# bwittmann/transoar

Hardware: AMD Instinct MI355X
Metric: training-step CT volumes/s, 160x160x256 Focused-Decoder (higher is better)
Workload: dtype bf16

## Files before the change

include/transoar_msda3d.h:

```cpp
#ifndef TRANSOAR_MSDA3D_H
#define TRANSOAR_MSDA3D_H

#include <stddef.h>
#include <stdint.h>

#ifdef __cplusplus
extern "C" {
#endif

enum {
  TRANSOAR_F32 = 0,
  TRANSOAR_F64 = 1,
  TRANSOAR_BF16 = 2,
  TRANSOAR_F16 = 3
};

enum {
  TRANSOAR_OK = 0,
  TRANSOAR_ERR_NULL = -1,
  TRANSOAR_ERR_DIM = -2,
  TRANSOAR_ERR_DTYPE = -3,
  TRANSOAR_ERR_ALIGN = -4,
  TRANSOAR_ERR_LEVELS = -5,
  TRANSOAR_ERR_WORKSPACE = -6,
  TRANSOAR_ERR_CONST = -7,
  TRANSOAR_ERR_MODE = -8
};

#define TRANSOAR_MSDA3D_MAX_LEVELS 8

#define TRANSOAR_MSDA3D_FORCE_GENERIC 1u
#define TRANSOAR_MSDA3D_NO_BRICK 4u
#define TRANSOAR_MSDA3D_FORK 8u
#define TRANSOAR_MSDA3D_NO_MMA 16u
#define TRANSOAR_MSDA3D_MMA_Q32 32u
#define TRANSOAR_MSDA3D_Q16 128u
#define TRANSOAR_MSDA3D_DETERMINISTIC 64u
#define TRANSOAR_MSDA3D_PULL_HEAD_MAJOR 2u

int transoar_msda3d_forward(const void* value, const int64_t* spatial_shapes,
                            const int64_t* level_start_index,
                            const void* sampling_loc, const void* attn_weight,
                            void* out, int N, int S, int M, int C, int L,
                            int Lq, int P, int value_dtype, int loc_dtype,
                            const int64_t* host_spatial_shapes, unsigned flags,
                            void* hip_stream);

int transoar_msda3d_forward_fused(const void* value, const void* proj,
                                  const float* ref, long ref_rows, void* out,
                                  int N, int S, int M, int C, int L, int P,
                                  int value_dtype,
                                  const int64_t* host_spatial_shapes,
                                  void* hip_stream);

int transoar_msda3d_backward(const void* value, const int64_t* spatial_shapes,
                             const int64_t* level_start_index,
                             const void* sampling_loc, const void* attn_weight,
                             const void* grad_out, void* grad_value,
                             void* grad_sampling_loc, void* grad_attn_weight,
                             void* workspace, size_t workspace_bytes,
                             int N, int S, int M, int C, int L, int Lq, int P,
                             int value_dtype, int loc_dtype,
                             const int64_t* host_spatial_shapes, unsigned flags,
                             void* hip_stream);

int transoar_msda3d_backward_proj(const void* value, const int64_t* spatial_shapes,
                                  const int64_t* level_start_index, const void* sampling_loc,
                                  const void* attn_weight, const void* grad_out,
                                  void* grad_value, void* grad_proj, void* workspace,
                                  size_t workspace_bytes, int N, int S, int M, int C, int L,
                                  int Lq, int P, int value_dtype, int loc_dtype,
                                  const int64_t* host_spatial_shapes, unsigned flags,
                                  void* hip_stream);

size_t transoar_msda3d_backward_workspace_bytes(int N, int S, int M, int C,
                                                int L, int Lq, int P,
                                                int value_dtype, int loc_dtype,
                                                unsigned flags);

enum {
  TRANSOAR_PROF_FWD = 0,
  TRANSOAR_PROF_BWD_QUERY = 1,
  TRANSOAR_PROF_CELL_COUNT = 2,
  TRANSOAR_PROF_SCAN = 3,
  TRANSOAR_PROF_CELL_FILL = 4,
  TRANSOAR_PROF_PULL = 5,
  TRANSOAR_PROF_FWD_GENERIC = 6,
  TRANSOAR_PROF_BWD_GENERIC = 7,
  TRANSOAR_PROF_VALUE_TILE = 8,
  TRANSOAR_PROF_VALUE_CELLS = 9,
  TRANSOAR_PROF_KINDS = 10
};
void transoar_msda3d_profile_enable(int on);
int transoar_msda3d_profile_read(double* total_ms, long* launches);

const char* transoar_msda3d_strerror(int code);

int transoar_msda3d_abi_version(void);

#ifdef __cplusplus
}
#endif
#endif
```

transoar_amd/backbone.py:

```python
import os

import torch
from torch import nn

from . import instnorm
from .conv3d import Conv3dK3, to_ncdhw
from .position_encoding import PositionEmbeddingLearned3D, PositionEmbeddingSine3D
from .swin_encoder import ConvPatchMerging, EncoderSwinBlock, PatchMerging
from .refine_block import DecoderDefAttnBlock
from .token_linear import token_linear


class EncoderCnnBlock(nn.Module):

    def __init__(self, in_channels, out_channels, kernel_size, stride, padding=1, bias=False,
                 affine=True, eps=1e-05):
        super().__init__()
        kernel_size, stride = tuple(kernel_size), tuple(stride)
        self._block = nn.Sequential(
            Conv3dK3(in_channels, out_channels, kernel_size, stride=stride, padding=padding, bias=bias),
            nn.InstanceNorm3d(out_channels, affine=affine, eps=eps),
            nn.ReLU(inplace=True),
            Conv3dK3(out_channels, out_channels, kernel_size, stride=1, padding=padding, bias=bias),
            nn.InstanceNorm3d(out_channels, affine=affine, eps=eps),
            nn.ReLU(inplace=True),
        )
        self._affine = affine

    fused_norm = True

    def _norm_relu(self, x, norm, part=None):
        if (EncoderCnnBlock.fused_norm and self._affine and x.dtype == torch.bfloat16
                and instnorm.supported(x, norm.num_features)):
            return instnorm.instance_norm_relu(x, norm.weight, norm.bias, norm.eps, relu=True, part=part)
        return torch.relu_(norm(x))

    def _conv_norm_relu(self, conv, norm, x):
        if (EncoderCnnBlock.fused_norm and self._affine and isinstance(conv, Conv3dK3) and norm.num_features <= 32):
            y, part = conv.forward_with_stats(x)
            if part is not None and not (y.dtype == torch.bfloat16 and instnorm.supported(y, norm.num_features)):
                part = None
            return self._norm_relu(y, norm, part)
        return self._norm_relu(conv(x), norm)

    def forward(self, x):
        if not x.is_cuda:
            return self._block(x)
        blk = self._block
        x = self._conv_norm_relu(blk[0], blk[1], x)
        return self._conv_norm_relu(blk[3], blk[4], x)


class Encoder(nn.Module):
    def __init__(self, config, debug=False):
        super().__init__()
        self._debug = debug
        self._stages = nn.ModuleList()
        cin, cout = config["in_channels"], config["start_channels"]
        swin = bool(config["use_encoder_attn"])
        depths = list(config["depths"])
        dpr = [float(v) for v in torch.linspace(0, config["drop_path_rate"], sum(depths))]
        merge = ConvPatchMerging if config["conv_merging"] else PatchMerging
        for stage_id, (kernel, stride) in enumerate(zip(config["conv_kernels"], config["strides"])):
            if swin and stage_id > 1:
                k = stage_id - 2
                stage = EncoderSwinBlock(
                    dim=cin, depth=depths[k], num_heads=config["num_heads"][k], window_size=config["window_size"],
                    mlp_ratio=config["mlp_ratio"], qkv_bias=config["qkv_bias"], qk_scale=config["qk_scale"],
                    drop=config["drop_rate"], attn_drop=config["attn_drop_rate"],
                    drop_path=dpr[sum(depths[:k]):sum(depths[:k + 1])], downsample=merge)
            else:
                stage = EncoderCnnBlock(cin, cout, kernel, stride)
            self._stages.append(stage)
            cin, cout = cout, cout * 2

    def forward(self, x):
        outputs = {}
        for i, stage in enumerate(self._stages):
            x = stage(x)
            outputs["C%d" % i] = x
        if self._debug:
            print("AttnFPN encoder shapes:", {k: list(v.shape) for k, v in outputs.items()})
            self._debug = False
        return outputs


def _gemm_conv_ok(f):
    return (f.is_cuda and f.dtype == torch.bfloat16 and f.dim() == 5 and f.shape[1] % 8 == 0
            and f.is_contiguous(memory_format=torch.channels_last_3d)
            and torch.is_autocast_enabled() and torch.get_autocast_gpu_dtype() == torch.bfloat16)


def _conv1_as_gemm(conv, f):
    n, c, d, h, w = f.shape
    tok = f.permute(0, 2, 3, 4, 1).reshape(n, d * h * w, c)
    y = token_linear(tok, conv.weight.view(conv.out_channels, c), conv.bias, force_hip=True, min_tokens=1024)
    return y.view(n, d, h, w, conv.out_channels).permute(0, 4, 1, 2, 3)


def _is_up2(up):
    return (tuple(up.kernel_size) == (2, 2, 2) and tuple(up.stride) == (2, 2, 2) and tuple(up.padding) == (0, 0, 0)
            and tuple(up.output_padding) == (0, 0, 0) and tuple(up.dilation) == (1, 1, 1) and up.groups == 1)


def _up2_as_gemm(up, f):
    n, c, d, h, w = f.shape
    co = up.out_channels
    tok = f.permute(0, 2, 3, 4, 1).reshape(n, d * h * w, c)
    w8 = up.weight.permute(2, 3, 4, 1, 0).reshape(8 * co, c)
    b8 = None if up.bias is None else up.bias.repeat(8)
    y = token_linear(tok, w8, b8, force_hip=True, min_tokens=1024)
    y = y.view(n, d, h, w, 2, 2, 2, co).permute(0, 1, 4, 2, 5, 3, 6, 7).reshape(n, 2 * d, 2 * h, 2 * w, co)
    return y.permute(0, 4, 1, 2, 3)


class Decoder(nn.Module):
    gemm_pointwise = os.environ.get("TRANSOAR_FPN_STOCK_POINTWISE") is None

    def __init__(self, config, debug=False):
        super().__init__()
        self._debug = debug
        n_stages = len(config["conv_kernels"])
        self._num_stages = n_stages
        self._refine_fmaps = config["use_decoder_attn"]
        self._refine_feature_levels = list(config["feature_levels"])
        self._seg_proxy = config["use_seg_proxy_loss"]
        fpn = int(config["fpn_channels"])
        enc_channels = [config["start_channels"] * 2 ** s for s in range(n_stages)]

        wanted = list(config["out_fmaps"]) + (list(config["feature_levels"]) if self._refine_fmaps else [])
        required = {int(name[-1]) for name in wanted}
        if self._seg_proxy:
            required.add(0)
        self._required_stages = sorted(required)
        first = 0 if self._seg_proxy else self._required_stages[0]
        self._first_stage = first

        lateral_in = enc_channels[first:]
        lateral_out = [min(c, fpn) for c in lateral_in]
        self._lateral = nn.ModuleList(nn.Conv3d(i, o, kernel_size=1) for i, o in zip(lateral_in, lateral_out))
        self._lateral_levels = len(self._lateral)

        self._out = nn.ModuleList()
        for n, stage in enumerate(self._required_stages):
            cout = enc_channels[0] if (self._seg_proxy and n == 0) else fpn
            self._out.append(Conv3dK3(lateral_out[stage - first], cout, kernel_size=3, padding=1))

        self._up = nn.ModuleList()
        coarse_to_fine = lateral_out[::-1]
        strides = [tuple(s) for s in config["strides"]][::-1]
        for lvl in range(len(coarse_to_fine) - 1):
            self._up.append(nn.ConvTranspose3d(coarse_to_fine[lvl], coarse_to_fine[lvl + 1],
                                               kernel_size=strides[lvl], stride=strides[lvl]))

        if self._refine_fmaps:
            if config["pos_encoding"] == "sine":
                self._pos_enc = PositionEmbeddingSine3D(channels=config["hidden_dim"])
            elif config["pos_encoding"] == "learned":
                self._pos_enc = PositionEmbeddingLearned3D(channels=config["hidden_dim"])
            else:
                raise ValueError("Please select a implemented pos. encoding.")
            self._refine = DecoderDefAttnBlock(
                d_model=config["hidden_dim"], nhead=config["nheads"], num_layers=config["layers"],
                dim_feedforward=config["dim_feedforward"], dropout=config["dropout"],
                feature_levels=config["feature_levels"], n_points=config["n_points"],
                use_cuda=config["use_cuda"])

    def forward(self, x):
        feats = list(x.values())[-self._lateral_levels:]
        if not Conv3dK3.ndhwc_everywhere:
            feats = [to_ncdhw(f) for f in feats]
        as_gemm = Decoder.gemm_pointwise and all(_gemm_conv_ok(f) for f in feats)
        laterals = [(_conv1_as_gemm(conv, f) if as_gemm else conv(f)) for conv, f in zip(self._lateral, feats)]
        merged = [None] * self._lateral_levels
        carry = None
        for k, lat in enumerate(reversed(laterals)):
            cur = lat if carry is None else lat + carry
            merged[self._lateral_levels - 1 - k] = cur
            if k < self._lateral_levels - 1:
                up = self._up[k]
                carry = _up2_as_gemm(up, cur) if (as_gemm and _is_up2(up)) else up(cur)
        outputs = {"P%d" % s: self._out[n](merged[s - self._first_stage])
                   for n, s in enumerate(self._required_stages)}

        if self._refine_fmaps:
            fmaps = [outputs[name] for name in self._refine_feature_levels]
            refined = self._refine(fmaps, [self._pos_enc(f) for f in fmaps])
            outputs.update(zip(self._refine_feature_levels, refined))
        if self._debug:
            print("AttnFPN decoder shapes:", {k: list(v.shape) for k, v in outputs.items()})
            self._debug = False
        return outputs


class AttnFPN(nn.Module):
    def __init__(self, fpn_config, debug=False):
        super().__init__()
        self._encoder = Encoder(fpn_config, debug)
        self._decoder = Decoder(fpn_config, debug)

    def forward(self, src):
        return self._decoder(self._encoder(src))

    def init_weights(self):
        pass
```

transoar_amd/csrc/msda3d.hip:

```cpp
#include <algorithm>
#include <cstring>

#include "../../include/transoar_msda3d.h"
#include "msda3d_common.hpp"
#include "msda3d_brick.hpp"
#include "msda3d_mma.hpp"
#include "msda3d_pcm.hpp"
#include "msda3d_q16.hpp"
#include "msda3d_tile.hpp"
#include "msda3d_cells_mma.hpp"
#include "msda3d_gather.hpp"
#include "msda3d_generic.hpp"
#include "msda3d_scatter.hpp"

#include <map>
#include <mutex>
#include <string>
#include <vector>

namespace transoar {

struct ProfPair { hipEvent_t beg, end; int kind; };
static std::mutex g_prof_mu;
static bool g_prof_on = false;
static std::vector<ProfPair> g_prof_live;
static std::vector<ProfPair> g_prof_free;

struct ProfScope {
  hipStream_t st;
  ProfPair pair;
  bool on;
  ProfScope(int kind, hipStream_t s) : st(s), on(false) {
    std::lock_guard<std::mutex> lk(g_prof_mu);
    if (!g_prof_on) return;
    if (!g_prof_free.empty()) {
      pair = g_prof_free.back();
      g_prof_free.pop_back();
    } else if (hipEventCreate(&pair.beg) != hipSuccess || hipEventCreate(&pair.end) != hipSuccess) {
      return;
    }
    pair.kind = kind;
    on = hipEventRecord(pair.beg, st) == hipSuccess;
  }
  ~ProfScope() {
    if (!on) return;
    (void)hipEventRecord(pair.end, st);
    std::lock_guard<std::mutex> lk(g_prof_mu);
    g_prof_live.push_back(pair);
  }
};

struct SideStream {
  hipStream_t stream = nullptr;
  hipEvent_t fork = nullptr, join = nullptr;
  bool ok = false;
};
static SideStream* side_stream() {
  static std::mutex mu;
  static SideStream per_device[16];
  int dev = 0;
  if (hipGetDevice(&dev) != hipSuccess || dev < 0 || dev >= 16) return nullptr;
  std::lock_guard<std::mutex> lk(mu);
  SideStream& s = per_device[dev];
  if (!s.ok && s.stream == nullptr) {
    if (hipStreamCreateWithFlags(&s.stream, hipStreamNonBlocking) == hipSuccess &&
        hipEventCreateWithFlags(&s.fork, hipEventDisableTiming) == hipSuccess &&
        hipEventCreateWithFlags(&s.join, hipEventDisableTiming) == hipSuccess)
      s.ok = true;
  }
  return s.ok ? &s : nullptr;
}

__global__ __launch_bounds__(256) void msda3d_zero16(u32x4* __restrict__ p, long n16) {
  const long i = static_cast<long>(blockIdx.x) * 256 + threadIdx.x;
  if (i < n16) p[i] = u32x4{0u, 0u, 0u, 0u};
}
static inline hipError_t zero_async(void* p, size_t bytes, hipStream_t st) {
  if (getenv("TRANSOAR_MSDA_MEMSET_NODE")) return hipMemsetAsync(p, 0, bytes, st);
  const long n16 = static_cast<long>((bytes + 15) / 16);
  hipLaunchKernelGGL(msda3d_zero16, dim3(static_cast<unsigned>((n16 + 255) / 256)), dim3(256), 0, st,
                     static_cast<u32x4*>(p), n16);
  return hipGetLastError();
}

struct Dims { int N, S, M, C, L, Lq, P; };

static inline int lpv_log2(int C, int elt) {
  const long bytes = static_cast<long>(C) * elt;
  if (bytes == 128) return 3;
  if (bytes == 256) return 4;
  if (bytes == 512) return 5;
  return -1;
}

static BrickOrder make_order(const int64_t* host_shapes, const Dims& d, int rows) {
  BrickOrder o{};
  if (!host_shapes || rows != d.S) return o;
  long start = 0, pad = 0;
  for (int l = 0; l < d.L; ++l) {
    const long D = host_shapes[3 * l], H = host_shapes[3 * l + 1], W = host_shapes[3 * l + 2];
    if (D <= 0 || H <= 0 || W <= 0) return BrickOrder{};
    o.D[l] = static_cast<int>(D); o.H[l] = static_cast<int>(H); o.W[l] = static_cast<int>(W);
    o.start[l] = static_cast<int>(start);
    o.nbh[l] = static_cast<int>((H + kBrickH - 1) / kBrickH);
    o.nbw[l] = static_cast<int>((W + kBrickW - 1) / kBrickW);
    o.pad_start[l] = static_cast<int>(pad);
    pad += ((D + kBrickD - 1) / kBrickD) * o.nbh[l] * o.nbw[l] * kBrickSlots;
    start += D * H * W;
  }
  if (start != d.S || pad * d.N * d.M >= (1L << 31)) return BrickOrder{};
  o.pad_start[d.L] = static_cast<int>(pad);
  o.L = d.L;
  o.enabled = 1;
  return o;
}
static inline long order_units(const BrickOrder& o, const Dims& d, int rows) {
  return static_cast<long>(d.N) * d.M * (o.enabled ? o.pad_start[o.L] : rows);
}

static inline size_t align16(size_t x) { return (x + 15) & ~static_cast<size_t>(15); }

static const void* device_const(const void* host, size_t bytes, hipStream_t st) {
  static std::mutex mu;
  static std::map<std::pair<int, std::string>, void*> cache;
  int dev = 0;
  if (hipGetDevice(&dev) != hipSuccess) return nullptr;
  std::pair<int, std::string> key(dev, std::string(static_cast<const char*>(host), bytes));
  std::lock_guard<std::mutex> lk(mu);
  auto it = cache.find(key);
  if (it != cache.end()) return it->second;
  hipStreamCaptureStatus cap = hipStreamCaptureStatusNone;
  if (hipStreamIsCapturing(st, &cap) != hipSuccess || cap != hipStreamCaptureStatusNone) return nullptr;
  if (cache.size() >= 256) return nullptr;
  void* p = nullptr;
  if (hipMalloc(&p, bytes) != hipSuccess) return nullptr;
  if (hipMemcpy(p, host, bytes, hipMemcpyHostToDevice) != hipSuccess) {
    (void)hipFree(p);
    return nullptr;
  }
  cache[key] = p;
  return p;
}
template <typename T> static const T* device_const(const T& v, hipStream_t st) {
  return static_cast<const T*>(device_const(&v, sizeof(T), st));
}

static inline int vec_lpv(const Dims& d, int elt, unsigned flags) {
  if (flags & TRANSOAR_MSDA3D_FORCE_GENERIC) return -1;
  const long value_bytes = static_cast<long>(d.N) * d.S * d.M * d.C * elt;
  const long n_points = static_cast<long>(d.N) * d.Lq * d.M * d.L * d.P;
  const long n_bins = static_cast<long>(d.N) * d.M * 8 * d.S;
  if (value_bytes >= 0xfffffff0L || n_points >= (1L << 31) - 1 || n_bins >= (1L << 31) - 1) return -1;
  if (static_cast<long>(d.N) * d.S >= (1L << 24) || static_cast<long>(d.M) * d.C * elt >= (1L << 24)) return -1;
  if (n_points * 32 >= 0xfffffff0L) return -1;
  if (static_cast<long>(d.N) * d.Lq * d.M >= (1L << 24) ||
      static_cast<long>(d.N) * d.Lq * d.M * d.C * elt >= 0x7ffffff0L) return -1;
  return lpv_log2(d.C, elt);
}

struct BwdWorkspace {
  size_t count, tile_sums, rank, rec_item, recs, coarse, det_keys, det_alt, det_temp, det_temp_bytes, total;
  long n_bins, n_points, n_scan, n_tiles;
};

int sort_keys64(unsigned long long* keys, unsigned long long* alt, long n, int end_bit, void* temp, size_t* temp_bytes,
                unsigned long long** sorted, hipStream_t st);

static BwdWorkspace bwd_workspace(const Dims& d, size_t acc_size, unsigned flags = 0u) {
  BwdWorkspace w;
  w.n_points = static_cast<long>(d.N) * d.Lq * d.M * d.L * d.P;
  w.n_bins = static_cast<long>(d.N) * d.M * 8 * d.S;
  w.n_scan = w.n_bins + 1;
  w.n_tiles = (w.n_scan + kScanTile - 1) / kScanTile;
  size_t off = 0;
  w.count = off;     off += align16(sizeof(int) * w.n_scan);
  w.tile_sums = off; off += align16(sizeof(int) * w.n_tiles);
  w.rank = off;      off += align16(sizeof(int) * w.n_points);
  w.rec_item = off;  off += align16(sizeof(int) * w.n_points);
  w.recs = off;      off += align16(8 * acc_size * w.n_points);
  w.coarse = off;    off += align16(sizeof(float) * static_cast<size_t>(d.N) * d.S * d.M * d.C);
  w.det_keys = w.det_alt = w.det_temp = off;
  w.det_temp_bytes = 0;
  if (flags & TRANSOAR_MSDA3D_DETERMINISTIC) {
    w.det_keys = off;  off += align16(sizeof(unsigned long long) * w.n_points);
    w.det_alt = off;   off += align16(sizeof(unsigned long long) * w.n_points);
    w.det_temp_bytes = align16((size_t(32) << 20) + static_cast<size_t>(w.n_points));
    w.det_temp = off;  off += w.det_temp_bytes;
  }
  w.total = off;
  return w;
}

static bool pcm_ok(const BrickOrder& order, const Dims& d) {
  if (!order.enabled || d.L > kPcmLevels || d.C != 64 || d.P != 4 || d.Lq != d.S) return false;
  for (int l = 0; l < d.L; ++l)
    if (order.D[l] > 1000 || order.H[l] > 1000 || order.W[l] > 1000) return false;
  const long n_pts = static_cast<long>(d.N) * d.Lq * d.M * d.L * d.P;
  const long n_wave = static_cast<long>(d.N) * (order.pad_start[order.L] >> 7) * d.M * 16;
  const long vbytes = static_cast<long>(d.N) * d.S * d.M * d.C * 2;
  return n_pts * 12 < 0xfffffff0L && n_wave < (1L << 31) - 8 && vbytes < 0xffffff00L;
}
static float host_bf16_round(float x) {
  unsigned u;
  memcpy(&u, &x, 4);
  u += 0x7fffu + ((u >> 16) & 1u);
  u &= 0xffff0000u;
  memcpy(&x, &u, 4);
  return x;
}
static PcmConst make_pcm_const(const BrickOrder& order) {
  PcmConst c;
  memset(&c, 0, sizeof(c));
  c.order = order;
  for (int l = 0; l < 4; ++l) {
    const int ls = l < order.L ? l : 0;
    c.fD[l] = static_cast<float>(order.D[ls]); c.fH[l] = static_cast<float>(order.H[ls]); c.fW[l] = static_cast<float>(order.W[ls]);
    c.dD[l] = host_bf16_round(c.fD[l]); c.dH[l] = host_bf16_round(c.fH[l]); c.dW[l] = host_bf16_round(c.fW[l]);
  }
  return c;
}

static Q16Const make_q16_const(const BrickOrder& order, int M) {
  Q16Const c;
  memset(&c, 0, sizeof(c));
  c.pc = make_pcm_const(order);
  auto mg = [](long d) -> unsigned long long { return (1ull << 40) / static_cast<unsigned long long>(d > 0 ? d : 1) + 1ull; };
  c.mg_M = mg(M);
  c.mg_bricks = mg(order.pad_start[order.L] >> 7);
  for (int l = 0; l < 4; ++l) {
    c.mg_nbw[l] = mg(l < order.L ? order.nbw[l] : 1);
    c.mg_nbh[l] = mg(l < order.L ? order.nbh[l] : 1);
  }
  return c;
}
static int env_int(const char* name, int dflt) {
  const char* v = getenv(name);
  return (v && *v) ? atoi(v) : dflt;
}

template <typename VT, typename LT>
static int launch_fwd(const void* value, const int64_t* shapes, const int64_t* lsi,
                      const void* loc, const void* attn, void* out, const Dims& d,
                      const int64_t* host_shapes, unsigned flags, hipStream_t st) {
  const long n_items = static_cast<long>(d.N) * d.Lq * d.M;
  const BrickOrder order = make_order(host_shapes, d, d.Lq);
  const long n_units = order_units(order, d, d.Lq);
  const long n_blocks = ((order.enabled ? n_units : n_items) + kWavesPerBlock - 1) / kWavesPerBlock;
  const int lg = vec_lpv(d, sizeof(VT), flags);
  const dim3 block(64 * kWavesPerBlock);
  auto v = static_cast<const VT*>(value);
  auto lo = static_cast<const LT*>(loc);
  auto at = static_cast<const LT*>(attn);
  auto o = static_cast<VT*>(out);
  if constexpr (sizeof(VT) == 2) {
    bool small = d.L <= kMmaLevels;
    for (int l = 0; small && l < d.L; ++l) small = order.D[l] <= 1000 && order.H[l] <= 1000 && order.W[l] <= 1000;
    if constexpr (sizeof(LT) == 4) {
      if (lg >= 0 && small && pcm_ok(order, d) && (flags & TRANSOAR_MSDA3D_Q16) &&
          !(flags & (TRANSOAR_MSDA3D_NO_BRICK | TRANSOAR_MSDA3D_NO_MMA | TRANSOAR_MSDA3D_MMA_Q32))) {
        ProfScope prof(TRANSOAR_PROF_FWD, st);
        static const int upw_env = env_int("TRANSOAR_MSDA3D_Q16_UPW", 4), probe = env_int("TRANSOAR_MSDA3D_Q16_PROBE", 0);
        const unsigned upw = static_cast<unsigned>(upw_env < 1 ? 1 : (upw_env > 64 ? 64 : upw_env));
        const long n_units = static_cast<long>(d.N) * (order.pad_start[order.L] >> 7) * d.M * 8;
        const long n_waves = (n_units + upw - 1) / upw;
        const unsigned vbytes = static_cast<unsigned>(static_cast<long>(d.N) * d.S * d.M * d.C * sizeof(VT));
        const long n_pts = static_cast<long>(d.N) * d.Lq * d.M * d.L * d.P;
        const Q16Const* cst = device_const(make_q16_const(order, d.M), st);
        if (cst == nullptr) return TRANSOAR_ERR_CONST;
        const dim3 grid(static_cast<unsigned>(((n_waves + 7) / 8) * 8));
#define TRANSOAR_Q16(PROBE)                                                                                             \
  hipLaunchKernelGGL((msda3d_fwd_q16<VT, PROBE>), grid, dim3(64), 0, st, v, lo, at, o, d.S, d.M, d.L, vbytes,               \
                     static_cast<unsigned>(n_pts * 12), static_cast<unsigned>(n_pts * 4), static_cast<unsigned>(n_units), upw, cst)
        if (probe == 1) TRANSOAR_Q16(1);
        else if (probe == 2) TRANSOAR_Q16(2);
        else if (probe == 3) TRANSOAR_Q16(3);
        else TRANSOAR_Q16(0);
#undef TRANSOAR_Q16
        return static_cast<int>(hipGetLastError());
      }
      if (lg >= 0 && small && pcm_ok(order, d) &&
          !(flags & (TRANSOAR_MSDA3D_NO_BRICK | TRANSOAR_MSDA3D_NO_MMA | TRANSOAR_MSDA3D_MMA_Q32))) {
        ProfScope prof(TRANSOAR_PROF_FWD, st);
        const long n_wave = static_cast<long>(d.N) * (order.pad_start[order.L] >> 7) * d.M * 16;
        const unsigned vbytes = static_cast<unsigned>(static_cast<long>(d.N) * d.S * d.M * d.C * sizeof(VT));
        const long n_pts = static_cast<long>(d.N) * d.Lq * d.M * d.L * d.P;
        const PcmConst* cst = device_const(make_pcm_const(order), st);
        if (cst == nullptr) return TRANSOAR_ERR_CONST;
        hipLaunchKernelGGL((msda3d_fwd_pcm<VT, false>), dim3(static_cast<unsigned>(((n_wave + 7) / 8) * 8)), dim3(64), 0, st,
                           v, lo, at, nullptr, nullptr, 0u, o, d.S, d.M, d.L, vbytes, static_cast<unsigned>(n_pts * 12),
                           static_cast<unsigned>(n_pts * 4), static_cast<unsigned>(n_wave), cst);
        return static_cast<int>(hipGetLastError());
      }
    }
    if (lg >= 0 && order.enabled && small && d.C == 64 && d.P == 4 &&
        !(flags & (TRANSOAR_MSDA3D_NO_BRICK | TRANSOAR_MSDA3D_NO_MMA))) {
      ProfScope prof(TRANSOAR_PROF_FWD, st);
      const long n_wave = static_cast<long>(d.N) * (order.pad_start[order.L] >> 7) * d.M * 4;
      const unsigned vbytes = static_cast<unsigned>(static_cast<long>(d.N) * d.S * d.M * d.C * sizeof(VT));
      const BrickOrder* order_d = device_const(order, st);
      if (order_d == nullptr) return TRANSOAR_ERR_CONST;
      hipLaunchKernelGGL((msda3d_fwd_mma<VT, LT>), dim3(static_cast<unsigned>(((n_wave + 7) / 8) * 8)), dim3(64), 0, st,
                         v, lo, at, o, d.S, d.M, d.L, vbytes, n_wave, order_d);
      return static_cast<int>(hipGetLastError());
    }
  }
  if (lg >= 0 && order.enabled && d.C == 64 && d.P == 4 && sizeof(VT) == 2 && !(flags & TRANSOAR_MSDA3D_NO_BRICK)) {
    ProfScope prof(TRANSOAR_PROF_FWD, st);
    const long n_wg = static_cast<long>(d.N) * (order.pad_start[order.L] >> 7) * d.M;
    const dim3 bgrid(((n_wg + 7) / 8) * 8);
    hipLaunchKernelGGL((msda3d_fwd_brick<VT, LT, 4, 64>), bgrid, dim3(kBrickThreads), kTileBytes, st, v, lo, at, o,
                       d.S, d.M, d.L, n_wg, order);
    return static_cast<int>(hipGetLastError());
  }
  if (lg < 0) {
    ProfScope prof(TRANSOAR_PROF_FWD_GENERIC, st);
    hipLaunchKernelGGL((msda3d_fwd_generic<VT, LT>), dim3((n_items + kWavesPerBlock - 1) / kWavesPerBlock),
                       block, 0, st, v, shapes, lsi, lo, at, o, d.S, d.M, d.C, d.L, d.Lq, d.P, n_items);
  } else {
    ProfScope prof(TRANSOAR_PROF_FWD, st);
    const dim3 grid(((n_blocks + 7) / 8) * 8);
    const unsigned vbytes = static_cast<unsigned>(static_cast<long>(d.N) * d.S * d.M * d.C * sizeof(VT));
#define TRANSOAR_FWD(LG)                                                                      \
  hipLaunchKernelGGL((msda3d_fwd_vec<VT, LT, LG>), grid, block, 0, st, v, shapes, lsi, lo, at, \
                     o, d.S, d.M, d.C, d.L, d.Lq, d.P, vbytes, n_units, n_blocks, order)
    if (lg == 3) TRANSOAR_FWD(3);
    else if (lg == 4) TRANSOAR_FWD(4);
    else TRANSOAR_FWD(5);
#undef TRANSOAR_FWD
  }
  return static_cast<int>(hipGetLastError());
}

template <typename VT>
static int launch_fwd_fused(const void* value, const void* proj, const float* ref, long ref_rows, void* out, const Dims& d,
                            const int64_t* host_shapes, hipStream_t st) {
  const BrickOrder order = make_order(host_shapes, d, d.Lq);
  if (vec_lpv(d, sizeof(VT), 0) < 0 || !pcm_ok(order, d)) return TRANSOAR_ERR_DIM;
  if (ref_rows != d.Lq && ref_rows != static_cast<long>(d.N) * d.Lq) return TRANSOAR_ERR_DIM;
  ProfScope prof(TRANSOAR_PROF_FWD, st);
  const long n_wave = static_cast<long>(d.N) * (order.pad_start[order.L] >> 7) * d.M * 16;
  const unsigned vbytes = static_cast<unsigned>(static_cast<long>(d.N) * d.S * d.M * d.C * sizeof(VT));
  const PcmConst* cst = device_const(make_pcm_const(order), st);
  if (cst == nullptr) return TRANSOAR_ERR_CONST;
  const unsigned ref_bstride = ref_rows == d.Lq ? 0u : static_cast<unsigned>(d.Lq) * d.L * 12u;
  const long proj_bytes = static_cast<long>(d.N) * d.S * 4 * d.M * d.L * d.P * 2;
  hipLaunchKernelGGL((msda3d_fwd_pcm<VT, true>), dim3(static_cast<unsigned>(((n_wave + 7) / 8) * 8)), dim3(64), 0, st,
                     static_cast<const VT*>(value), nullptr, nullptr, static_cast<const unsigned short*>(proj), ref, ref_bstride,
                     static_cast<VT*>(out), d.S, d.M, d.L, vbytes, static_cast<unsigned>(proj_bytes),
                     static_cast<unsigned>(ref_rows * d.L * 12), static_cast<unsigned>(n_wave), cst);
  return static_cast<int>(hipGetLastError());
}

__global__ __launch_bounds__(256) void msda3d_det_gather(const unsigned long long* __restrict__ sorted, const PointR16* __restrict__ slots,
                                                          PointR16* __restrict__ recs, long n) {
  const long j = static_cast<long>(blockIdx.x) * 256 + threadIdx.x;
  if (j >= n) return;
  const unsigned long long k = sorted[j];
  if (k == ~0ull) return;
  recs[j] = slots[static_cast<unsigned>(k)];
}

template <typename VT, typename LT>
static size_t bwd_workspace_bytes(const Dims& d, unsigned flags) {
  using A = typename Elem<VT>::acc;
  if (vec_lpv(d, sizeof(VT), flags) >= 0) return bwd_workspace(d, sizeof(A), flags).total;
  return sizeof(VT) == 2 ? align16(sizeof(float) * static_cast<size_t>(d.N) * d.S * d.M * d.C) : 0;
}

#define TRANSOAR_CHECK_HIP(expr)                         \
  do {                                                   \
    const hipError_t e_ = (expr);                        \
    if (e_ != hipSuccess) return static_cast<int>(e_);   \
  } while (0)

template <typename VT, typename LT>
static int launch_bwd(const void* value, const int64_t* shapes, const int64_t* lsi,
                      const void* loc, const void* attn, const void* grad_out, void* grad_value,
                      void* grad_loc, void* grad_attn, void* workspace, size_t workspace_bytes,
                      const Dims& d, const int64_t* host_shapes, unsigned flags, hipStream_t st, void* grad_proj = nullptr) {
  using A = typename Elem<VT>::acc;
  if (workspace_bytes < bwd_workspace_bytes<VT, LT>(d, flags)) return TRANSOAR_ERR_WORKSPACE;
  if (grad_proj != nullptr && (sizeof(VT) != 2 || sizeof(LT) != 4 || vec_lpv(d, sizeof(VT), flags) < 0)) return TRANSOAR_ERR_MODE;
  const long n_items = static_cast<long>(d.N) * d.Lq * d.M;
  const BrickOrder q_order = make_order(host_shapes, d, d.Lq);
  const long q_units = order_units(q_order, d, d.Lq);
  const long n_blocks = (q_units + kWavesPerBlock - 1) / kWavesPerBlock;
  const int lg = vec_lpv(d, sizeof(VT), flags);
  const dim3 block(64 * kWavesPerBlock);
  auto v = static_cast<const VT*>(value);
  auto lo = static_cast<const LT*>(loc);
  auto at = static_cast<const LT*>(attn);
  auto go = static_cast<const VT*>(grad_out);
  auto gl = static_cast<LT*>(grad_loc);
  auto ga = static_cast<LT*>(grad_attn);
  const size_t value_elems = static_cast<size_t>(d.N) * d.S * d.M * d.C;

  if (lg < 0) {
    ProfScope prof(TRANSOAR_PROF_BWD_GENERIC, st);
    A* gv = sizeof(VT) == 2 ? static_cast<A*>(workspace) : static_cast<A*>(grad_value);
    TRANSOAR_CHECK_HIP(hipMemsetAsync(gv, 0, sizeof(A) * value_elems, st));
    hipLaunchKernelGGL((msda3d_bwd_generic<VT, LT>), dim3((n_items + kWavesPerBlock - 1) / kWavesPerBlock),
                       block, 0, st, v, shapes, lsi, lo, at, go, gv, gl, ga, d.S, d.M, d.C, d.L, d.Lq, d.P,
                       n_items);
    if (sizeof(VT) == 2) {
      const int cast_blocks = static_cast<int>(std::min<size_t>((value_elems + 255) / 256, 1 << 16));
      hipLaunchKernelGGL((msda3d_cast_rows<VT>), dim3(cast_blocks), dim3(256), 0, st,
                         reinterpret_cast<const float*>(gv), static_cast<VT*>(grad_value),
                         static_cast<long>(value_elems));
    }
    return static_cast<int>(hipGetLastError());
  }

  const dim3 grid(((n_blocks + 7) / 8) * 8);
  const unsigned vbytes = static_cast<unsigned>(value_elems * sizeof(VT));
  const BwdWorkspace w = bwd_workspace(d, sizeof(A), flags);
  char* ws = static_cast<char*>(workspace);
  int* count = reinterpret_cast<int*>(ws + w.count);
  int* tile_sums = reinterpret_cast<int*>(ws + w.tile_sums);
  int* rank = reinterpret_cast<int*>(ws + w.rank);
  int* rec_item = reinterpret_cast<int*>(ws + w.rec_item);
  auto recs = reinterpret_cast<PointRec<A>*>(ws + w.recs);
  long cells_per_slab = 0;
  if (host_shapes)
    for (int l = 0; l < d.L; ++l)
      cells_per_slab += (host_shapes[3 * l] + 1) * (host_shapes[3 * l + 1] + 1) * (host_shapes[3 * l + 2] + 1);
  const bool fold_count = host_shapes != nullptr && cells_per_slab * d.N * d.M <= w.n_bins;
  const bool det_req = (flags & TRANSOAR_MSDA3D_DETERMINISTIC) != 0;
  const long n_scan = fold_count ? cells_per_slab * d.N * d.M + 1 + (det_req && cells_per_slab * d.N * d.M + 2 <= w.n_scan ? 1 : 0) : w.n_scan;
  const long n_tiles = (n_scan + kScanTile - 1) / kScanTile;
  TRANSOAR_CHECK_HIP(zero_async(count, sizeof(int) * n_scan, st));
  auto scan = [&]() {
    ProfScope prof(TRANSOAR_PROF_SCAN, st);
    hipLaunchKernelGGL(msda3d_scan_tiles, dim3(static_cast<unsigned>(n_tiles)), dim3(kScanThreads), 0,
                       st, count, tile_sums, static_cast<int>(n_scan));
    hipLaunchKernelGGL(msda3d_scan_tile_sums, dim3(1), dim3(kScanThreads), 0, st, tile_sums,
                       static_cast<int>(n_tiles));
    hipLaunchKernelGGL(msda3d_scan_add, dim3(static_cast<unsigned>(n_tiles)), dim3(kScanThreads), 0, st,
                       count, tile_sums, static_cast<int>(n_scan));
  };

#define TRANSOAR_BWDQ(LG)                                                                   \
  hipLaunchKernelGGL((msda3d_bwd_query_vec<VT, LT, LG>), grid, block, 0, st, v, shapes, lsi, lo, \
                     at, go, gl, ga, fold_count ? count : nullptr, rank, static_cast<int>(cells_per_slab), \
                     d.S, d.M, d.C, d.L, d.Lq, d.P, vbytes, q_units, n_blocks, q_order)
  bool brick_done = false, recs_done = false, det = false;
  if constexpr (sizeof(VT) == 2) {
    bool small = d.L <= kMmaLevels;
    for (int l = 0; small && l < d.L; ++l) small = q_order.D[l] <= 1000 && q_order.H[l] <= 1000 && q_order.W[l] <= 1000;
    if (q_order.enabled && fold_count && small && d.C == 64 && d.P == 4 &&
        !(flags & (TRANSOAR_MSDA3D_NO_BRICK | TRANSOAR_MSDA3D_NO_MMA))) {
      const long n_wave = static_cast<long>(d.N) * (q_order.pad_start[q_order.L] >> 7) * d.M * 4;
      const BrickOrder* order_d = device_const(q_order, st);
      if (order_d == nullptr) return TRANSOAR_ERR_CONST;
      const dim3 qgrid(static_cast<unsigned>(((n_wave + 7) / 8) * 8));
      {
        ProfScope prof(TRANSOAR_PROF_CELL_COUNT, st);
        hipLaunchKernelGGL((msda3d_cell_count_mma<LT>), qgrid, dim3(64), 0, st, lo, count + 1,
                           static_cast<int>(cells_per_slab), d.S, d.M, d.L, n_wave, order_d);
      }
      scan();
      det = det_req && cells_per_slab * d.N * d.M + 2 <= w.n_scan && w.n_points < (1L << 31);
      if (det_req && !det) return TRANSOAR_ERR_MODE;
      if (!det) {
        ProfScope prof(TRANSOAR_PROF_BWD_QUERY, st);
        hipLaunchKernelGGL((msda3d_bwd_query_mma<VT, LT>), qgrid, dim3(64), 0, st,
                           v, lo, at, go, gl, ga, count + 1, reinterpret_cast<PointR16*>(ws + w.recs), nullptr,
                           static_cast<int>(cells_per_slab), d.S, d.M, d.L, vbytes, n_wave, order_d,
                           static_cast<unsigned short*>(grad_proj));
      } else {
        auto keys = reinterpret_cast<unsigned long long*>(ws + w.det_keys);
        auto alt = reinterpret_cast<unsigned long long*>(ws + w.det_alt);
        PointR16* slots = reinterpret_cast<PointR16*>(ws + w.recs) + w.n_points;
        TRANSOAR_CHECK_HIP(hipMemsetAsync(keys, 0xff, sizeof(unsigned long long) * w.n_points, st));
        {
          ProfScope prof(TRANSOAR_PROF_BWD_QUERY, st);
          hipLaunchKernelGGL((msda3d_bwd_query_mma<VT, LT>), qgrid, dim3(64), 0, st,
                             v, lo, at, go, gl, ga, count + 1, slots, keys,
                             static_cast<int>(cells_per_slab), d.S, d.M, d.L, vbytes, n_wave, order_d,
                             static_cast<unsigned short*>(grad_proj));
        }
        ProfScope prof(TRANSOAR_PROF_CELL_FILL, st);
        int cell_bits = 1;
        while ((cells_per_slab * d.N * d.M) >> cell_bits) ++cell_bits;
        size_t need = 0;
        int rc = sort_keys64(keys, alt, w.n_points, 32 + cell_bits, nullptr, &need, nullptr, st);
        if (rc != 0) return rc;
        if (need > w.det_temp_bytes) return TRANSOAR_ERR_WORKSPACE;
        unsigned long long* sorted = nullptr;
        size_t temp_bytes = w.det_temp_bytes;
        rc = sort_keys64(keys, alt, w.n_points, 32 + cell_bits, ws + w.det_temp, &temp_bytes, &sorted, st);
        if (rc != 0) return rc;
        hipLaunchKernelGGL(msda3d_det_gather, dim3(static_cast<unsigned>((w.n_points + 255) / 256)), dim3(256), 0, st,
                           sorted, slots, reinterpret_cast<PointR16*>(ws + w.recs), w.n_points);
      }
      brick_done = recs_done = true;
    }
  }
  if (det_req && !det) return TRANSOAR_ERR_MODE;
  if (grad_proj != nullptr && !recs_done) return TRANSOAR_ERR_MODE;
  if constexpr (sizeof(VT) == 2) {
    if (!brick_done && q_order.enabled && fold_count && d.C == 64 && d.P == 4 && !(flags & TRANSOAR_MSDA3D_NO_BRICK)) {
      ProfScope prof(TRANSOAR_PROF_BWD_QUERY, st);
      const long n_wg = static_cast<long>(d.N) * (q_order.pad_start[q_order.L] >> 7) * d.M;
      hipLaunchKernelGGL((msda3d_bwd_query_brick<VT, LT, 4, 64>), dim3(((n_wg + 7) / 8) * 8), dim3(kBrickThreads),
                         kTileBytes, st, v, lo, at, go, gl, ga, count, rank, static_cast<int>(cells_per_slab), d.S, d.M,
                         d.L, n_wg, q_order);
      brick_done = true;
    }
  }
  if (!brick_done) {
    ProfScope prof(TRANSOAR_PROF_BWD_QUERY, st);
    if (lg == 3) TRANSOAR_BWDQ(3);
    else if (lg == 4) TRANSOAR_BWDQ(4);
    else TRANSOAR_BWDQ(5);
  }
#undef TRANSOAR_BWDQ

  const dim3 pgrid(static_cast<unsigned>((w.n_points + 255) / 256));
  if (!fold_count) {
    ProfScope prof(TRANSOAR_PROF_CELL_COUNT, st);
    hipLaunchKernelGGL((msda3d_cell_count<LT, A>), pgrid, dim3(256), 0, st, lo, at, shapes, lsi, count,
                       rank, d.M, d.L, d.Lq, d.P, w.n_points);
  }
  if (!recs_done) scan();
  BrickOrder r_order = make_order(host_shapes, d, d.S);
  if constexpr (sizeof(A) == 4) {
    if (r_order.enabled && fold_count && d.C == kTileC && !(flags & TRANSOAR_MSDA3D_NO_BRICK)) {
      auto recs8 = reinterpret_cast<PointW8<float>*>(ws + w.recs);
      auto recs4 = reinterpret_cast<PointR16*>(ws + w.recs);
      bool mma = false;
      if constexpr (sizeof(VT) == 2) mma = !(flags & TRANSOAR_MSDA3D_NO_MMA);
      if (!recs_done) {
        ProfScope prof(TRANSOAR_PROF_CELL_FILL, st);
        if (mma)
          hipLaunchKernelGGL((msda3d_cell_fill_r16<LT>), pgrid, dim3(256), 0, st, lo, at, shapes, lsi, count, rank, recs4,
                             d.M, d.L, d.Lq, d.P, w.n_points);
        else
          hipLaunchKernelGGL((msda3d_cell_fill_w8<LT, float>), pgrid, dim3(256), 0, st, lo, at, shapes, lsi, count,
                             rank, recs8, rec_item, d.M, d.L, d.Lq, d.P, w.n_points);
      }
      CoarseLevels cl{d.L, static_cast<int>(cells_per_slab), d.S, 0, 0};
      const int* offsets = det ? count + 1 : count;
      for (int l = d.L - 1; l >= 0 && !det; --l) {
        const long vox = host_shapes[3 * l] * host_shapes[3 * l + 1] * host_shapes[3 * l + 2];
        if (static_cast<long>(d.Lq) * d.P < kCoarsePointsPerVoxel * vox) break;
        cl.first = l;
        cl.cell_start -= static_cast<int>((host_shapes[3 * l] + 1) * (host_shapes[3 * l + 1] + 1) * (host_shapes[3 * l + 2] + 1));
        cl.row_start = r_order.start[l];
      }
      cl.rows = d.S - cl.row_start;
      const int coarse_levels = d.L - cl.first;
      const int cell_chunk = mma ? kCmCellChunk : kCellChunk;
      cl.chunks_per_slab = static_cast<int>((static_cast<long>(d.Lq) * d.P * coarse_levels + cell_chunk - 1) / cell_chunk) + 1;
      const int fine_bricks = r_order.pad_start[cl.first] >> 7;
      const BrickOrder* r_order_d = device_const(r_order, st);
      const CoarseLevels* cl_d = device_const(cl, st);
      if (r_order_d == nullptr || cl_d == nullptr) return TRANSOAR_ERR_CONST;
      float* scratch = reinterpret_cast<float*>(ws + w.coarse);
      const long scratch_elems = static_cast<long>(d.N) * cl.rows * d.M * kTileC;
      SideStream* side = (g_prof_on || !(flags & TRANSOAR_MSDA3D_FORK) || coarse_levels == 0 || fine_bricks == 0)
                             ? nullptr : side_stream();
      hipStream_t cst = st;
      if (side != nullptr) {
        TRANSOAR_CHECK_HIP(hipEventRecord(side->fork, st));
        TRANSOAR_CHECK_HIP(hipStreamWaitEvent(side->stream, side->fork, 0));
        cst = side->stream;
      }
      if (coarse_levels > 0) {
        ProfScope prof(TRANSOAR_PROF_VALUE_CELLS, cst);
        TRANSOAR_CHECK_HIP(zero_async(scratch, sizeof(float) * scratch_elems, cst));
        const long waves = static_cast<long>(d.N) * d.M * cl.chunks_per_slab;
        if (mma) {
          if constexpr (sizeof(VT) == 2)
            hipLaunchKernelGGL((msda3d_bwd_value_cells_mma<VT>), dim3(static_cast<unsigned>((waves + 3) / 4)), dim3(256), 0,
                               cst, go, offsets, recs4, scratch, static_cast<int>(cells_per_slab), d.N * d.M, d.M,
                               cl_d, r_order_d);
        } else {
          hipLaunchKernelGGL((msda3d_bwd_value_cells<VT>), dim3(static_cast<unsigned>((waves + 3) / 4)), dim3(256), 0, cst,
                             go, count, recs8, rec_item, scratch, static_cast<int>(cells_per_slab), d.N * d.M, d.M, cl_d,
                             r_order_d);
        }
      }
      if (side != nullptr) TRANSOAR_CHECK_HIP(hipEventRecord(side->join, side->stream));
      ProfScope prof(TRANSOAR_PROF_VALUE_TILE, st);
      if (fine_bricks > 0) {
        const long n_wg = static_cast<long>(d.N) * fine_bricks * d.M;
        if (mma) {
          if constexpr (sizeof(VT) == 2)
            hipLaunchKernelGGL((msda3d_bwd_value_tile_mma<VT>), dim3(static_cast<unsigned>(n_wg)), dim3(kBrickThreads), 0, st,
                               go, offsets, recs4, static_cast<VT*>(grad_value), static_cast<int>(cells_per_slab),
                               d.S, d.M, fine_bricks, n_wg, r_order_d);
        } else {
          hipLaunchKernelGGL((msda3d_bwd_value_tile<VT>), dim3(static_cast<unsigned>(n_wg)), dim3(kBrickThreads), 0, st, go,
                             count, recs8, rec_item, static_cast<VT*>(grad_value), static_cast<int>(cells_per_slab),
                             d.S, d.M, fine_bricks, n_wg, r_order_d);
        }
      }
      if (side != nullptr) TRANSOAR_CHECK_HIP(hipStreamWaitEvent(st, side->join, 0));
      if (coarse_levels > 0) {
        const long n4 = scratch_elems / 4;
        hipLaunchKernelGGL((msda3d_coarse_rows_store<VT>), dim3(static_cast<unsigned>((n4 + 255) / 256)), dim3(256), 0, st,
                           scratch, static_cast<VT*>(grad_value), d.S, d.M, cl.rows, cl.row_start, n4);
      }
      return static_cast<int>(hipGetLastError());
    }
  }
  {
    ProfScope prof(TRANSOAR_PROF_CELL_FILL, st);
    hipLaunchKernelGGL((msda3d_cell_fill<LT, A>), pgrid, dim3(256), 0, st, lo, at, shapes, lsi, count,
                       rank, recs, rec_item, d.M, d.L, d.Lq, d.P, w.n_points);
  }

  if (r_order.enabled && (flags & TRANSOAR_MSDA3D_PULL_HEAD_MAJOR)) r_order.enabled = 2;
  const long n_rows = order_units(r_order, d, d.S);
  const long r_blocks = (n_rows + kWavesPerBlock - 1) / kWavesPerBlock;
  const dim3 rgrid(((r_blocks + 7) / 8) * 8);
#define TRANSOAR_PULL(LG)                                                                        \
  hipLaunchKernelGGL((msda3d_bwd_value_pull<VT, A, LG>), rgrid, block, 0, st, go, shapes, lsi, count, \
                     recs, rec_item, static_cast<VT*>(grad_value), d.S, d.M, d.C, d.L, n_rows, r_blocks, r_order, \
                     static_cast<unsigned>(w.n_points * 4 * sizeof(A)))
  {
    ProfScope prof(TRANSOAR_PROF_PULL, st);
    if (lg == 3) TRANSOAR_PULL(3);
    else if (lg == 4) TRANSOAR_PULL(4);
    else TRANSOAR_PULL(5);
  }
#undef TRANSOAR_PULL
  return static_cast<int>(hipGetLastError());
}

static int check_common(const Dims& d, int value_dtype, int loc_dtype) {
  if (d.N <= 0 || d.S <= 0 || d.M <= 0 || d.C <= 0 || d.L <= 0 || d.Lq <= 0 || d.P <= 0)
    return TRANSOAR_ERR_DIM;
  if (d.L > TRANSOAR_MSDA3D_MAX_LEVELS) return TRANSOAR_ERR_LEVELS;
  if (static_cast<long>(d.N) * d.Lq * d.M >= (1L << 31) || static_cast<long>(d.N) * d.S >= (1L << 31))
    return TRANSOAR_ERR_DIM;
  const bool half = value_dtype == TRANSOAR_BF16 || value_dtype == TRANSOAR_F16;
  if (value_dtype < 0 || value_dtype > TRANSOAR_F16) return TRANSOAR_ERR_DTYPE;
  if (!(loc_dtype == value_dtype || (half && loc_dtype == TRANSOAR_F32))) return TRANSOAR_ERR_DTYPE;
  return TRANSOAR_OK;
}

static inline bool misaligned(const void* p) { return (reinterpret_cast<uintptr_t>(p) & 15u) != 0; }

}

using namespace transoar;

#define TRANSOAR_DISPATCH(VD, LD, CALL)                                            \
  do {                                                                             \
    if (VD == TRANSOAR_F32) { using VT = float; using LT = float; return CALL; }   \
    if (VD == TRANSOAR_F64) { using VT = double; using LT = double; return CALL; } \
    if (VD == TRANSOAR_BF16 && LD == TRANSOAR_BF16) { using VT = bf16_t; using LT = bf16_t; return CALL; } \
    if (VD == TRANSOAR_BF16) { using VT = bf16_t; using LT = float; return CALL; } \
    if (VD == TRANSOAR_F16 && LD == TRANSOAR_F16) { using VT = f16_t; using LT = f16_t; return CALL; }     \
    { using VT = f16_t; using LT = float; return CALL; }                           \
  } while (0)

extern "C" int transoar_msda3d_forward(const void* value, const int64_t* spatial_shapes,
                                       const int64_t* level_start_index, const void* sampling_loc,
                                       const void* attn_weight, void* out, int N, int S, int M,
                                       int C, int L, int Lq, int P, int value_dtype, int loc_dtype,
                                       const int64_t* host_spatial_shapes, unsigned flags,
                                       void* hip_stream) {
  if (!value || !spatial_shapes || !level_start_index || !sampling_loc || !attn_weight || !out)
    return TRANSOAR_ERR_NULL;
  const Dims d{N, S, M, C, L, Lq, P};
  const int rc = check_common(d, value_dtype, loc_dtype);
  if (rc != TRANSOAR_OK) return rc;
  if (misaligned(value) || misaligned(sampling_loc) || misaligned(attn_weight) || misaligned(out))
    return TRANSOAR_ERR_ALIGN;
  hipStream_t st = static_cast<hipStream_t>(hip_stream);
  TRANSOAR_DISPATCH(value_dtype, loc_dtype,
                    (launch_fwd<VT, LT>(value, spatial_shapes, level_start_index, sampling_loc,
                                        attn_weight, out, d, host_spatial_shapes, flags, st)));
}

extern "C" int transoar_msda3d_forward_fused(const void* value, const void* proj, const float* ref, long ref_rows,
                                             void* out, int N, int S, int M, int C, int L, int P, int value_dtype,
                                             const int64_t* host_spatial_shapes, void* hip_stream) {
  if (!value || !proj || !ref || !out || !host_spatial_shapes) return TRANSOAR_ERR_NULL;
  const Dims d{N, S, M, C, L, S, P};
  const int rc = check_common(d, value_dtype, TRANSOAR_F32);
  if (rc != TRANSOAR_OK) return rc;
  if (value_dtype != TRANSOAR_BF16 && value_dtype != TRANSOAR_F16) return TRANSOAR_ERR_DTYPE;
  if (misaligned(value) || misaligned(proj) || misaligned(ref) || misaligned(out)) return TRANSOAR_ERR_ALIGN;
  hipStream_t st = static_cast<hipStream_t>(hip_stream);
  if (value_dtype == TRANSOAR_BF16) return launch_fwd_fused<bf16_t>(value, proj, ref, ref_rows, out, d, host_spatial_shapes, st);
  return launch_fwd_fused<f16_t>(value, proj, ref, ref_rows, out, d, host_spatial_shapes, st);
}

extern "C" int transoar_msda3d_backward(const void* value, const int64_t* spatial_shapes,
                                        const int64_t* level_start_index, const void* sampling_loc,
                                        const void* attn_weight, const void* grad_out,
                                        void* grad_value, void* grad_sampling_loc,
                                        void* grad_attn_weight, void* workspace,
                                        size_t workspace_bytes, int N, int S, int M, int C, int L,
                                        int Lq, int P, int value_dtype, int loc_dtype,
                                        const int64_t* host_spatial_shapes, unsigned flags,
                                        void* hip_stream) {
  if (!value || !spatial_shapes || !level_start_index || !sampling_loc || !attn_weight ||
      !grad_out || !grad_value || !grad_sampling_loc || !grad_attn_weight)
    return TRANSOAR_ERR_NULL;
  const Dims d{N, S, M, C, L, Lq, P};
  const int rc = check_common(d, value_dtype, loc_dtype);
  if (rc != TRANSOAR_OK) return rc;
  if (misaligned(value) || misaligned(sampling_loc) || misaligned(attn_weight) ||
      misaligned(grad_out) || misaligned(grad_value) || misaligned(grad_sampling_loc) ||
      misaligned(grad_attn_weight) || misaligned(workspace))
    return TRANSOAR_ERR_ALIGN;
  if (!workspace && workspace_bytes != 0) return TRANSOAR_ERR_NULL;
  hipStream_t st = static_cast<hipStream_t>(hip_stream);
  TRANSOAR_DISPATCH(value_dtype, loc_dtype,
                    (launch_bwd<VT, LT>(value, spatial_shapes, level_start_index, sampling_loc,
                                        attn_weight, grad_out, grad_value, grad_sampling_loc,
                                        grad_attn_weight, workspace, workspace_bytes, d,
                                        host_spatial_shapes, flags, st)));
}

extern "C" int transoar_msda3d_backward_proj(const void* value, const int64_t* spatial_shapes,
                                             const int64_t* level_start_index, const void* sampling_loc,
                                             const void* attn_weight, const void* grad_out,
                                             void* grad_value, void* grad_proj, void* workspace,
                                             size_t workspace_bytes, int N, int S, int M, int C, int L,
                                             int Lq, int P, int value_dtype, int loc_dtype,
                                             const int64_t* host_spatial_shapes, unsigned flags,
                                             void* hip_stream) {
  if (!value || !spatial_shapes || !level_start_index || !sampling_loc || !attn_weight ||
      !grad_out || !grad_value || !grad_proj)
    return TRANSOAR_ERR_NULL;
  const Dims d{N, S, M, C, L, Lq, P};
  const int rc = check_common(d, value_dtype, loc_dtype);
  if (rc != TRANSOAR_OK) return rc;
  if (loc_dtype != TRANSOAR_F32 || (value_dtype != TRANSOAR_BF16 && value_dtype != TRANSOAR_F16) || L * P != 16) return TRANSOAR_ERR_MODE;
  if (misaligned(value) || misaligned(sampling_loc) || misaligned(attn_weight) ||
      misaligned(grad_out) || misaligned(grad_value) || misaligned(grad_proj) || misaligned(workspace))
    return TRANSOAR_ERR_ALIGN;
  if (!workspace && workspace_bytes != 0) return TRANSOAR_ERR_NULL;
  hipStream_t st = static_cast<hipStream_t>(hip_stream);
  TRANSOAR_DISPATCH(value_dtype, loc_dtype,
                    (launch_bwd<VT, LT>(value, spatial_shapes, level_start_index, sampling_loc,
                                        attn_weight, grad_out, grad_value, nullptr, nullptr, workspace, workspace_bytes, d,
                                        host_spatial_shapes, flags, st, grad_proj)));
}

extern "C" size_t transoar_msda3d_backward_workspace_bytes(int N, int S, int M, int C, int L, int Lq,
                                                           int P, int value_dtype, int loc_dtype,
                                                           unsigned flags) {
  const Dims d{N, S, M, C, L, Lq, P};
  if (check_common(d, value_dtype, loc_dtype) != TRANSOAR_OK) return 0;
  TRANSOAR_DISPATCH(value_dtype, loc_dtype, (bwd_workspace_bytes<VT, LT>(d, flags)));
}

extern "C" const char* transoar_msda3d_strerror(int code) {
  switch (code) {
    case TRANSOAR_OK: return "success";
    case TRANSOAR_ERR_NULL: return "a required pointer is NULL";
    case TRANSOAR_ERR_DIM: return "a dimension is non-positive or exceeds the 32-bit index range";
    case TRANSOAR_ERR_DTYPE: return "unsupported value/loc dtype combination";
    case TRANSOAR_ERR_ALIGN: return "a device buffer is not 16-byte aligned";
    case TRANSOAR_ERR_LEVELS: return "too many feature levels";
    case TRANSOAR_ERR_WORKSPACE: return "workspace is smaller than transoar_msda3d_backward_workspace_bytes()";
    case TRANSOAR_ERR_MODE: return "the deterministic backward does not cover this form (16-bit storage, C = 64, P = 4, <= 4 host-known levels, queries = pyramid voxels)";
    case TRANSOAR_ERR_CONST: return "could not place the launch constants in device memory (first call for a shape must not be inside a stream capture)";
    default: return code > 0 ? hipGetErrorString(static_cast<hipError_t>(code)) : "unknown error";
  }
}

extern "C" void transoar_msda3d_profile_enable(int on) {
  std::lock_guard<std::mutex> lk(g_prof_mu);
  g_prof_on = on != 0;
}

extern "C" int transoar_msda3d_profile_read(double* total_ms, long* launches) {
  std::vector<ProfPair> live;
  {
    std::lock_guard<std::mutex> lk(g_prof_mu);
    live.swap(g_prof_live);
  }
  for (int k = 0; k < TRANSOAR_PROF_KINDS; ++k) {
    total_ms[k] = 0.0;
    launches[k] = 0;
  }
  int rc = 0;
  for (const ProfPair& p : live) {
    float ms = 0.f;
    hipError_t e = hipEventSynchronize(p.end);
    if (e == hipSuccess) e = hipEventElapsedTime(&ms, p.beg, p.end);
    if (e != hipSuccess) { rc = static_cast<int>(e); continue; }
    total_ms[p.kind] += ms;
    launches[p.kind] += 1;
  }
  std::lock_guard<std::mutex> lk(g_prof_mu);
  g_prof_free.insert(g_prof_free.end(), live.begin(), live.end());
  return rc;
}

extern "C" int transoar_msda3d_abi_version(void) { return 6; }
```

transoar_amd/csrc/msda3d_common.hpp:

```cpp
#pragma once
#include <hip/hip_runtime.h>
#include <stdint.h>

namespace transoar {

constexpr int kWavesPerBlock = 4;
constexpr int kChunk = 16;

struct bf16_t { unsigned short bits; };
struct f16_t { _Float16 v; };

using u32x4 = __attribute__((ext_vector_type(4))) unsigned int;

__device__ __forceinline__ float bf16_to_f32(unsigned short b) {
  return __uint_as_float(static_cast<unsigned int>(b) << 16);
}
__device__ __forceinline__ unsigned short f32_to_bf16(float f) {
  unsigned int u = __float_as_uint(f);
  if ((u & 0x7fffffffu) > 0x7f800000u) return static_cast<unsigned short>((u >> 16) | 0x40u);
  u += 0x7fffu + ((u >> 16) & 1u);
  return static_cast<unsigned short>(u >> 16);
}

template <typename T> struct Elem;

template <> struct Elem<float> {
  using acc = float;
  static constexpr int VEC = 4;
  static __device__ __forceinline__ float ld(const float* p) { return *p; }
  static __device__ __forceinline__ void st(float* p, float v) { *p = v; }
  static __device__ __forceinline__ void unpack(const u32x4& r, float (&o)[4]) {
#pragma unroll
    for (int i = 0; i < 4; ++i) o[i] = __uint_as_float(r[i]);
  }
  static __device__ __forceinline__ u32x4 pack(const float (&o)[4]) {
    u32x4 r;
#pragma unroll
    for (int i = 0; i < 4; ++i) r[i] = __float_as_uint(o[i]);
    return r;
  }
};

template <> struct Elem<double> {
  using acc = double;
  static constexpr int VEC = 2;
  static __device__ __forceinline__ double ld(const double* p) { return *p; }
  static __device__ __forceinline__ void st(double* p, double v) { *p = v; }
  static __device__ __forceinline__ void unpack(const u32x4& r, double (&o)[2]) {
#pragma unroll
    for (int i = 0; i < 2; ++i)
      o[i] = __longlong_as_double((static_cast<long long>(r[2 * i + 1]) << 32) |
                                  static_cast<long long>(r[2 * i]));
  }
  static __device__ __forceinline__ u32x4 pack(const double (&o)[2]) {
    u32x4 r;
#pragma unroll
    for (int i = 0; i < 2; ++i) {
      const long long b = __double_as_longlong(o[i]);
      r[2 * i] = static_cast<unsigned int>(b);
      r[2 * i + 1] = static_cast<unsigned int>(b >> 32);
    }
    return r;
  }
};

template <> struct Elem<bf16_t> {
  using acc = float;
  static constexpr int VEC = 8;
  static __device__ __forceinline__ float ld(const bf16_t* p) { return bf16_to_f32(p->bits); }
  static __device__ __forceinline__ void st(bf16_t* p, float v) { p->bits = f32_to_bf16(v); }
  static __device__ __forceinline__ void unpack(const u32x4& r, float (&o)[8]) {
#pragma unroll
    for (int i = 0; i < 4; ++i) {
      o[2 * i] = __uint_as_float(r[i] << 16);
      o[2 * i + 1] = __uint_as_float(r[i] & 0xffff0000u);
    }
  }
  static __device__ __forceinline__ u32x4 pack(const float (&o)[8]) {
    u32x4 r;
#pragma unroll
    for (int i = 0; i < 4; ++i)
      r[i] = static_cast<unsigned int>(f32_to_bf16(o[2 * i])) |
             (static_cast<unsigned int>(f32_to_bf16(o[2 * i + 1])) << 16);
    return r;
  }
  static __device__ __forceinline__ float dot2(unsigned int a, unsigned int b, float acc) {
    typedef __bf16 bf16x2 __attribute__((ext_vector_type(2)));
    return __builtin_amdgcn_fdot2_f32_bf16(__builtin_bit_cast(bf16x2, a), __builtin_bit_cast(bf16x2, b), acc, false);
  }
};

template <> struct Elem<f16_t> {
  using acc = float;
  static constexpr int VEC = 8;
  static __device__ __forceinline__ float h2f(unsigned int bits16) {
    return static_cast<float>(__builtin_bit_cast(_Float16, static_cast<unsigned short>(bits16)));
  }
  static __device__ __forceinline__ unsigned int f2h(float f) {
    return __builtin_bit_cast(unsigned short, static_cast<_Float16>(f));
  }
  static __device__ __forceinline__ float ld(const f16_t* p) { return static_cast<float>(p->v); }
  static __device__ __forceinline__ void st(f16_t* p, float v) { p->v = static_cast<_Float16>(v); }
  static __device__ __forceinline__ void unpack(const u32x4& r, float (&o)[8]) {
#pragma unroll
    for (int i = 0; i < 4; ++i) {
      o[2 * i] = h2f(r[i] & 0xffffu);
      o[2 * i + 1] = h2f(r[i] >> 16);
    }
  }
  static __device__ __forceinline__ u32x4 pack(const float (&o)[8]) {
    u32x4 r;
#pragma unroll
    for (int i = 0; i < 4; ++i) r[i] = f2h(o[2 * i]) | (f2h(o[2 * i + 1]) << 16);
    return r;
  }
  static __device__ __forceinline__ float dot2(unsigned int a, unsigned int b, float acc) {
    typedef _Float16 f16x2 __attribute__((ext_vector_type(2)));
    return __builtin_amdgcn_fdot2(__builtin_bit_cast(f16x2, a), __builtin_bit_cast(f16x2, b), acc, false);
  }
};

__device__ __forceinline__ float pixel_coord(float loc, int size) {
#pragma clang fp contract(off)
  const float t = loc * static_cast<float>(size);
  return t - 0.5f;
}
__device__ __forceinline__ double pixel_coord(double loc, int size) {
#pragma clang fp contract(off)
  const double t = loc * static_cast<double>(size);
  return t - 0.5;
}

__device__ __forceinline__ float bcast(float v, int src) {
  return __int_as_float(__builtin_amdgcn_readlane(__float_as_int(v), src));
}
__device__ __forceinline__ double bcast(double v, int src) {
  const long long b = __double_as_longlong(v);
  const unsigned lo = __builtin_amdgcn_readlane(static_cast<int>(b), src);
  const unsigned hi = __builtin_amdgcn_readlane(static_cast<int>(b >> 32), src);
  return __longlong_as_double((static_cast<long long>(hi) << 32) | lo);
}

__device__ __forceinline__ float xor_lanes(float v, int mask) { return __shfl_xor(v, mask, 64); }
__device__ __forceinline__ double xor_lanes(double v, int mask) { return __shfl_xor(v, mask, 64); }

__device__ __forceinline__ float xor_free_shfl(float v, int src) { return __shfl(v, src, 64); }
__device__ __forceinline__ double xor_free_shfl(double v, int src) { return __shfl(v, src, 64); }

__device__ __forceinline__ void atomic_accum(float* p, float v) {
  __hip_atomic_fetch_add(p, v, __ATOMIC_RELAXED, __HIP_MEMORY_SCOPE_AGENT);
}
__device__ __forceinline__ void atomic_accum(double* p, double v) {
  __hip_atomic_fetch_add(p, v, __ATOMIC_RELAXED, __HIP_MEMORY_SCOPE_AGENT);
}

template <int HALF, typename A>
__device__ __forceinline__ void fold_lanes(const A (&in)[2 * HALF], A (&out)[HALF], int lane) {
  const bool up = (lane & HALF) != 0;
#pragma unroll
  for (int i = 0; i < HALF; ++i) {
    const A send = up ? in[i] : in[i + HALF];
    const A keep = up ? in[i + HALF] : in[i];
    out[i] = keep + xor_lanes(send, HALF);
  }
}
template <typename A>
__device__ __forceinline__ A sum_transpose64(const A (&v)[64], int lane) {
  A a32[32], a16[16], a8[8], a4[4], a2[2], a1[1];
  fold_lanes<32>(v, a32, lane);
  fold_lanes<16>(a32, a16, lane);
  fold_lanes<8>(a16, a8, lane);
  fold_lanes<4>(a8, a4, lane);
  fold_lanes<2>(a4, a2, lane);
  fold_lanes<1>(a2, a1, lane);
  return a1[0];
}

constexpr int kBrickD = 4, kBrickH = 4, kBrickW = 8, kBrickSlots = 128;
struct BrickOrder {
  int enabled, L;
  int D[8], H[8], W[8], start[8];
  int nbh[8], nbw[8];
  int pad_start[9];
};
__device__ __forceinline__ int brick_slot_to_row(const BrickOrder& o, int x) {
  int l = 0;
  for (int t = 1; t < o.L; ++t) l += (x >= o.pad_start[t]) ? 1 : 0;
  const int local = x - o.pad_start[l];
  const int brick = local >> 7, slot = local & 127;
  const int bw = brick % o.nbw[l];
  const int r = brick / o.nbw[l];
  const int bh = r % o.nbh[l], bd = r / o.nbh[l];
  const int d = bd * kBrickD + (slot >> 5), h = bh * kBrickH + ((slot >> 3) & 3), w = bw * kBrickW + (slot & 7);
  if (d >= o.D[l] || h >= o.H[l] || w >= o.W[l]) return -1;
  return o.start[l] + (d * o.H[l] + h) * o.W[l] + w;
}
__device__ __forceinline__ long ordered_unit(const BrickOrder& o, long u, int R, int M) {
  if (!o.enabled) return u;
  const int total = o.pad_start[o.L];
  int m, x;
  long b;
  if (o.enabled == 2) {
    const int slot = static_cast<int>(u & 127);
    const long t = u >> 7;
    m = static_cast<int>(t % M);
    const long t2 = t / M;
    const int bricks = total >> 7;
    x = static_cast<int>(t2 % bricks) * 128 + slot;
    b = t2 / bricks;
  } else {
    m = static_cast<int>(u % M);
    const long t = u / M;
    x = static_cast<int>(t % total);
    b = t / total;
  }
  const int r = brick_slot_to_row(o, x);
  return r < 0 ? -1 : (b * R + r) * M + m;
}

__device__ __forceinline__ long xcd_contiguous_block(long bid, long nblk) {
  const long per = (nblk + 7) >> 3;
  const long swz = (bid & 7) * per + (bid >> 3);
  return swz < nblk ? swz : -1;
}

struct alignas(16) PointR16 {
  float a;
  int item;
  unsigned lo, hi;
};
constexpr float kFracScale = 2097152.f;
__device__ __forceinline__ unsigned frac21(float f) {
  return min(static_cast<unsigned>(f * kFracScale + 0.5f), 0x1fffffu);
}
__device__ __forceinline__ PointR16 make_point_r16(float a, int item, float ld, float lh, float lw) {
  const unsigned qd = frac21(ld), qh = frac21(lh), qw = frac21(lw);
  return PointR16{a, item, qd | (qh << 21), (qh >> 11) | (qw << 10)};
}
__device__ __forceinline__ void point_r16_fracs(unsigned lo, unsigned hi, float& ld, float& lh, float& lw) {
  constexpr float inv = 1.f / kFracScale;
  ld = static_cast<float>(lo & 0x1fffffu) * inv;
  lh = static_cast<float>((lo >> 21) | ((hi & 0x3ffu) << 11)) * inv;
  lw = static_cast<float>(hi >> 10) * inv;
}

}
```

transoar_amd/csrc/msda3d_mma.hpp:

```cpp
#pragma once
#include "msda3d_common.hpp"

namespace transoar {

constexpr int kMmaKB = 64;
constexpr int kMmaVP = 144;
constexpr int kMmaWRows = kMmaKB + 1;
constexpr int kMmaDenseRows = 1024;
constexpr int kMmaLevels = 4;

typedef float f32x16 __attribute__((ext_vector_type(16)));
typedef short s16x4 __attribute__((ext_vector_type(4)));
typedef short s16x8 __attribute__((ext_vector_type(8)));
typedef __bf16 bf16x8_t __attribute__((ext_vector_type(8)));
typedef _Float16 f16x8_t __attribute__((ext_vector_type(8)));

template <typename VT> struct Mma;
template <> struct Mma<bf16_t> {
  static __device__ __forceinline__ f32x16 mfma(s16x8 a, s16x8 b, f32x16 c) {
    return __builtin_amdgcn_mfma_f32_32x32x16_bf16(__builtin_bit_cast(bf16x8_t, a), __builtin_bit_cast(bf16x8_t, b), c, 0, 0, 0);
  }
  static __device__ __forceinline__ void split(const float (&w)[8], s16x8& hi, s16x8& lo) {
    unsigned h[4], l[4];
#pragma unroll
    for (int i = 0; i < 4; ++i) {
      const unsigned u0 = __float_as_uint(w[2 * i]), u1 = __float_as_uint(w[2 * i + 1]);
      h[i] = __builtin_amdgcn_perm(u1, u0, 0x07060302u);
      const unsigned r0 = __float_as_uint(w[2 * i] - __uint_as_float(u0 & 0xffff0000u));
      const unsigned r1 = __float_as_uint(w[2 * i + 1] - __uint_as_float(u1 & 0xffff0000u));
      l[i] = __builtin_amdgcn_perm(r1, r0, 0x07060302u);
    }
    hi = __builtin_bit_cast(s16x8, u32x4{h[0], h[1], h[2], h[3]});
    lo = __builtin_bit_cast(s16x8, u32x4{l[0], l[1], l[2], l[3]});
  }
};
template <> struct Mma<f16_t> {
  static __device__ __forceinline__ f32x16 mfma(s16x8 a, s16x8 b, f32x16 c) {
    return __builtin_amdgcn_mfma_f32_32x32x16_f16(__builtin_bit_cast(f16x8_t, a), __builtin_bit_cast(f16x8_t, b), c, 0, 0, 0);
  }
  static __device__ __forceinline__ void split(const float (&w)[8], s16x8& hi, s16x8& lo) {
    f16x8_t h, l;
#pragma unroll
    for (int i = 0; i < 8; ++i) {
      h[i] = static_cast<_Float16>(w[i]);
      l[i] = static_cast<_Float16>(w[i] - static_cast<float>(h[i]));
    }
    hi = __builtin_bit_cast(s16x8, h);
    lo = __builtin_bit_cast(s16x8, l);
  }
};

typedef short s16x2 __attribute__((ext_vector_type(2)));
__device__ __forceinline__ int wave_min_pk16(int v) {
#define TRANSOAR_DPP_STEP(CTRL, ROWMASK)                                                        \
  {                                                                                             \
    const int o = __builtin_amdgcn_update_dpp(v, v, CTRL, ROWMASK, 0xf, false);                 \
    v = __builtin_bit_cast(int, __builtin_elementwise_min(__builtin_bit_cast(s16x2, v), __builtin_bit_cast(s16x2, o))); \
  }
  TRANSOAR_DPP_STEP(0xB1, 0xf)
  TRANSOAR_DPP_STEP(0x4E, 0xf)
  TRANSOAR_DPP_STEP(0x141, 0xf)
  TRANSOAR_DPP_STEP(0x140, 0xf)
  TRANSOAR_DPP_STEP(0x142, 0xa)
  TRANSOAR_DPP_STEP(0x143, 0xc)
#undef TRANSOAR_DPP_STEP
  return __builtin_amdgcn_readlane(v, 63);
}
__device__ __forceinline__ int pack16(int lo, int hi) { return (lo & 0xffff) | (hi << 16); }

template <int I> struct IntC { static constexpr int value = I; };
template <int I, int N, typename F>
__device__ __forceinline__ void static_for(F&& f) {
  if constexpr (I < N) {
    f(IntC<I>{});
    static_for<I + 1, N>(f);
  }
}

struct MmaPoint {
  int dhw;
  float ld, lh, lw, a;
};
struct MmaBox {
  int bd, bh, bw, TD, TH, TW;
};

template <typename VT, typename LT>
__global__ __launch_bounds__(64, 2) void msda3d_fwd_mma(
    const VT* __restrict__ value, const LT* __restrict__ loc, const LT* __restrict__ attn,
    VT* __restrict__ out, int S, int M, int L, unsigned value_bytes, long n_units, const BrickOrder* __restrict__ order_p) {
  const BrickOrder& order = *order_p;
  constexpr int P = 4, C = 64, KB = kMmaKB, VP = kMmaVP, WR = kMmaWRows;
  __shared__ __attribute__((aligned(16))) unsigned char vbuf[KB * VP];
  __shared__ __attribute__((aligned(16))) float wbuf[WR * 32];

  const long u = xcd_contiguous_block(blockIdx.x, n_units);
  if (u < 0) return;
  const int lane = threadIdx.x;
  const int j = lane & 31, kg = lane >> 5;
  const int sb = static_cast<int>(u & 3);
  const long t1 = u >> 2;
  const int m = static_cast<int>(t1 % M);
  const long t2 = t1 / M;
  const int bricks = order.pad_start[order.L] >> 7;
  const int brick = bricks - 1 - static_cast<int>(t2 % bricks);
  const long b = t2 / bricks;
  const int slot = (2 * (sb >> 1) + (j >> 4)) * 32 + ((j >> 2) & 3) * 8 + 4 * (sb & 1) + (j & 3);
  const int s = brick_slot_to_row(order, brick * kBrickSlots + slot);
  const bool live = s >= 0;
  const long item = live ? (b * S + s) * M + m : 0;
  const int LP = L * P;
  const unsigned row_bytes = static_cast<unsigned>(M) * C * sizeof(VT);
  const unsigned head_off = static_cast<unsigned>((b * S * M + m) * C * sizeof(VT));
  const __amdgpu_buffer_rsrc_t rsrc =
      __builtin_amdgcn_make_buffer_rsrc(const_cast<VT*>(value), 0, static_cast<int>(value_bytes), 0x00020000);

  MmaPoint pt[kMmaLevels][2];
  MmaBox box[kMmaLevels];
  static_for<0, kMmaLevels>([&](auto lc) {
    constexpr int l = decltype(lc)::value;
    box[l] = MmaBox{0, 0, 0, 0, 0, 0};
    if (l >= L) return;
    const int D = order.D[l], H = order.H[l], W = order.W[l];
    int lo_d = 32767, lo_h = 32767, lo_w = 32767, hi_d = -1, hi_h = -1, hi_w = -1;
    float lx[2] = {0.f, 0.f}, ly[2] = {0.f, 0.f}, lz[2] = {0.f, 0.f}, la[2] = {0.f, 0.f};
    if (live) {
      const long jx = item * LP + l * P + 2 * kg;
      if constexpr (sizeof(LT) == 4) {
        const float2 q0 = *reinterpret_cast<const float2*>(loc + 3 * jx), q1 = *reinterpret_cast<const float2*>(loc + 3 * jx + 2),
                     q2 = *reinterpret_cast<const float2*>(loc + 3 * jx + 4), qa = *reinterpret_cast<const float2*>(attn + jx);
        lx[0] = q0.x; ly[0] = q0.y; lz[0] = q1.x; lx[1] = q1.y; ly[1] = q2.x; lz[1] = q2.y;
        la[0] = qa.x; la[1] = qa.y;
      } else {
#pragma unroll
        for (int pi = 0; pi < 2; ++pi) {
          lx[pi] = static_cast<float>(Elem<LT>::ld(loc + 3 * (jx + pi)));
          ly[pi] = static_cast<float>(Elem<LT>::ld(loc + 3 * (jx + pi) + 1));
          lz[pi] = static_cast<float>(Elem<LT>::ld(loc + 3 * (jx + pi) + 2));
          la[pi] = static_cast<float>(Elem<LT>::ld(attn + jx + pi));
        }
      }
    }
#pragma unroll
    for (int pi = 0; pi < 2; ++pi) {
      MmaPoint g{0x3fffffff, 0.f, 0.f, 0.f, 0.f};
      const float w_im = pixel_coord(lx[pi], W), h_im = pixel_coord(ly[pi], H), d_im = pixel_coord(lz[pi], D);
      if (live && d_im > -1.f && h_im > -1.f && w_im > -1.f && d_im < D && h_im < H && w_im < W) {
        const float fd = floorf(d_im), fh = floorf(h_im), fw = floorf(w_im);
        const int d0 = static_cast<int>(fd), h0 = static_cast<int>(fh), w0 = static_cast<int>(fw);
        g.dhw = (d0 + 1) | ((h0 + 1) << 10) | ((w0 + 1) << 20);
        g.ld = d_im - fd; g.lh = h_im - fh; g.lw = w_im - fw; g.a = la[pi];
        lo_d = min(lo_d, max(d0, 0)); hi_d = max(hi_d, min(d0 + 1, D - 1));
        lo_h = min(lo_h, max(h0, 0)); hi_h = max(hi_h, min(h0 + 1, H - 1));
        lo_w = min(lo_w, max(w0, 0)); hi_w = max(hi_w, min(w0 + 1, W - 1));
      }
      pt[l][pi] = g;
    }
    const int r0 = wave_min_pk16(pack16(lo_d, lo_h)), r1 = wave_min_pk16(pack16(lo_w, -hi_d)), r2 = wave_min_pk16(pack16(-hi_h, -hi_w));
    hi_d = -(r1 >> 16);
    if (hi_d < 0) return;
    lo_d = static_cast<short>(r0); lo_h = r0 >> 16; lo_w = static_cast<short>(r1);
    hi_h = -static_cast<int>(static_cast<short>(r2)); hi_w = -(r2 >> 16);
    box[l] = MmaBox{lo_d, lo_h, lo_w, hi_d - lo_d + 1, hi_h - lo_h + 1, hi_w - lo_w + 1};
  });

  f32x16 acc0, acc1;
#pragma unroll
  for (int i = 0; i < 16; ++i) { acc0[i] = 0.f; acc1[i] = 0.f; }
  for (int i = lane; i < WR * 32 / 4; i += 64) reinterpret_cast<float4*>(wbuf)[i] = float4{0.f, 0.f, 0.f, 0.f};
  for (int i = lane; i < KB * VP / 16; i += 64) reinterpret_cast<float4*>(vbuf)[i] = float4{0.f, 0.f, 0.f, 0.f};

  const int st_row = lane >> 3, st_vec = lane & 7;
  auto load_block = [&](auto lc, int kb, u32x4 (&pre)[8]) {
    constexpr int l = decltype(lc)::value;
    const MmaBox bx = box[l];
    const int H = order.H[l], W = order.W[l], start = order.start[l];
    const int THW = bx.TH * bx.TW, R = bx.TD * THW;
    const float inv_thw = __builtin_amdgcn_rcpf(static_cast<float>(THW)), inv_tw = __builtin_amdgcn_rcpf(static_cast<float>(bx.TW));
    const int r = kb * KB + lane;
    const int rd = static_cast<int>((static_cast<float>(r) + 0.5f) * inv_thw), rr = r - __mul24(rd, THW);
    const int rh = static_cast<int>((static_cast<float>(rr) + 0.5f) * inv_tw), rw = rr - __mul24(rh, bx.TW);
    const int grow = start + __mul24(__mul24(bx.bd + rd, H) + (bx.bh + rh), W) + (bx.bw + rw);
    const unsigned past = static_cast<unsigned>((R - 1 - r) >> 31);
    const int row_off = static_cast<int>((head_off + __umul24(static_cast<unsigned>(grow), row_bytes)) | (past & 0xfffffff0u));
#pragma unroll
    for (int it = 0; it < 8; ++it) {
      const unsigned off = static_cast<unsigned>(__builtin_amdgcn_ds_bpermute((it * 8 + st_row) * 4, row_off)) + st_vec * 16u;
      pre[it] = __builtin_amdgcn_raw_buffer_load_b128(rsrc, off, 0, 0);
    }
  };

  u32x4 pre[8];
  bool have_pre = false;
  static_for<0, kMmaLevels>([&](auto lc) {
    constexpr int l = decltype(lc)::value;
    if (l >= L || box[l].TD == 0) return;
    const MmaBox bx = box[l];
    const int D = order.D[l], H = order.H[l], W = order.W[l];
    const int THW = bx.TH * bx.TW, R = bx.TD * THW;

    int ecol[16];
    float ewt[16];
    int near = 0;
#pragma unroll
    for (int pi = 0; pi < 2; ++pi) {
      const MmaPoint g = pt[l][pi];
      const int d0 = (g.dhw & 1023) - 1, h0 = ((g.dhw >> 10) & 1023) - 1, w0 = ((g.dhw >> 20) & 1023) - 1;
      const bool okp = g.dhw != 0x3fffffff;
      const int cb = (__mul24(__mul24(d0 - bx.bd, bx.TH) + (h0 - bx.bh), bx.TW) + (w0 - bx.bw)) * 32 + j;
      const bool vd[2] = {okp && static_cast<unsigned>(d0) < static_cast<unsigned>(D), okp && static_cast<unsigned>(d0 + 1) < static_cast<unsigned>(D)};
      const bool vh[2] = {static_cast<unsigned>(h0) < static_cast<unsigned>(H), static_cast<unsigned>(h0 + 1) < static_cast<unsigned>(H)};
      const bool vw[2] = {static_cast<unsigned>(w0) < static_cast<unsigned>(W), static_cast<unsigned>(w0 + 1) < static_cast<unsigned>(W)};
      const float wd[2] = {g.a * (1.f - g.ld), g.a * g.ld}, wh[2] = {1.f - g.lh, g.lh}, ww[2] = {1.f - g.lw, g.lw};
#pragma unroll
      for (int c = 0; c < 4; ++c) {
        const int dd = c >> 1, dh = c & 1;
        const float f = wd[dd] * wh[dh];
        const int col = cb + (dd ? THW * 32 : 0) + (dh ? bx.TW * 32 : 0);
#pragma unroll
        for (int dw = 0; dw < 2; ++dw) {
          ecol[pi * 8 + 2 * c + dw] = (vd[dd] && vh[dh] && vw[dw]) ? col + 32 * dw : -64;
          ewt[pi * 8 + 2 * c + dw] = f * ww[dw];
        }
      }
      const int odhw = __builtin_amdgcn_ds_bpermute((lane ^ 32) * 4, g.dhw);
      const int od = (odhw & 1023) - 1 - d0, oh = ((odhw >> 10) & 1023) - 1 - h0, ow = ((odhw >> 20) & 1023) - 1 - w0;
      near |= (okp && odhw != 0x3fffffff && abs(od) <= 1 && abs(oh) <= 1 && abs(ow) <= 1) ? 1 : 0;
    }
    const bool shared = __any(near);

    if (R > kMmaDenseRows) {
      float tacc[32];
#pragma unroll
      for (int i = 0; i < 32; ++i) tacc[i] = 0.f;
#pragma unroll 1
      for (int p4 = 0; p4 < 4; ++p4) {
        MmaPoint g = (p4 & 1) ? pt[l][1] : pt[l][0];
        MmaPoint o;
        o.dhw = __shfl_xor(g.dhw, 32, 64);
        o.ld = __shfl_xor(g.ld, 32, 64); o.lh = __shfl_xor(g.lh, 32, 64);
        o.lw = __shfl_xor(g.lw, 32, 64); o.a = __shfl_xor(g.a, 32, 64);
        if ((p4 >> 1) != kg) g = o;
        if (g.dhw == 0x3fffffff) continue;
        const int d0 = (g.dhw & 1023) - 1, h0 = ((g.dhw >> 10) & 1023) - 1, w0 = ((g.dhw >> 20) & 1023) - 1;
#pragma unroll 1
        for (int k = 0; k < 8; ++k) {
          const int dd = k >> 2, dh = (k >> 1) & 1, dw = k & 1;
          const int d = d0 + dd, h = h0 + dh, w = w0 + dw;
          if (static_cast<unsigned>(d) >= static_cast<unsigned>(D) || static_cast<unsigned>(h) >= static_cast<unsigned>(H) ||
              static_cast<unsigned>(w) >= static_cast<unsigned>(W))
            continue;
          const float wv = g.a * ((dd ? g.ld : 1.f - g.ld) * (dh ? g.lh : 1.f - g.lh)) * (dw ? g.lw : 1.f - g.lw);
          const long grow = order.start[l] + (static_cast<long>(d) * H + h) * W + w;
          const VT* src = value + ((b * S + grow) * M + m) * C + 32 * kg;
#pragma unroll
          for (int i = 0; i < 4; ++i) {
            float vv[8];
            Elem<VT>::unpack(reinterpret_cast<const u32x4*>(src)[i], vv);
#pragma unroll
            for (int e = 0; e < 8; ++e) tacc[8 * i + e] += wv * vv[e];
          }
        }
      }
#pragma unroll
      for (int bq = 0; bq < 4; ++bq) {
#pragma unroll
        for (int t = 0; t < 4; ++t) {
          const float keep = kg == 0 ? tacc[8 * bq + t] : tacc[8 * bq + 4 + t];
          const float give = kg == 0 ? tacc[8 * bq + 4 + t] : tacc[8 * bq + t];
          const float got = __shfl_xor(give, 32, 64);
          acc0[4 * bq + t] += kg == 0 ? keep : got;
          acc1[4 * bq + t] += kg == 0 ? got : keep;
        }
      }
      have_pre = false;
      return;
    }

    const int nblk = (R + KB - 1) / KB;
    if (!have_pre) load_block(lc, 0, pre);
    for (int kb = 0; kb < nblk; ++kb) {
      const int k0 = kb * KB;
      const int nch = (min(KB, R - k0) + 15) >> 4;
#pragma unroll
      for (int it = 0; it < 4; ++it) *reinterpret_cast<u32x4*>(vbuf + (it * 8 + st_row) * VP + st_vec * 16) = pre[it];
      if (nch > 2) {
#pragma unroll
        for (int it = 4; it < 8; ++it) *reinterpret_cast<u32x4*>(vbuf + (it * 8 + st_row) * VP + st_vec * 16) = pre[it];
      }
      have_pre = false;
      if (kb + 1 < nblk) {
        load_block(lc, kb + 1, pre);
        have_pre = true;
      } else if constexpr (l + 1 < kMmaLevels) {
        if (l + 1 < L && box[l + 1].TD != 0) {
          const MmaBox nb = box[l + 1];
          if (nb.TD * nb.TH * nb.TW <= kMmaDenseRows) {
            load_block(IntC<l + 1>{}, 0, pre);
            have_pre = true;
          }
        }
      }
      int wad[16];
#pragma unroll
      for (int e = 0; e < 16; ++e)
        wad[e] = static_cast<int>(min(static_cast<unsigned>(ecol[e] - k0 * 32), static_cast<unsigned>(KB * 32 + j)));
      auto add_round = [&](auto pic, int turn) {
        constexpr int pi = decltype(pic)::value;
        int ad[8];
        float prev[8];
#pragma unroll
        for (int q = 0; q < 8; ++q) ad[q] = (turn < 0 || kg == turn) ? wad[pi * 8 + q] : KB * 32 + j;
#pragma unroll
        for (int q = 0; q < 8; ++q) prev[q] = wbuf[ad[q]];
#pragma unroll
        for (int q = 0; q < 8; ++q) wbuf[ad[q]] = prev[q] + ewt[pi * 8 + q];
      };
      if (!shared) {
        add_round(IntC<0>{}, -1);
        add_round(IntC<1>{}, -1);
      } else {
        add_round(IntC<0>{}, 0);
        add_round(IntC<1>{}, 0);
        add_round(IntC<0>{}, 1);
        add_round(IntC<1>{}, 1);
      }
      for (int kc = 0; kc < nch; kc += 2) {
        s16x8 bhi[2], blo[2], a0[2], a1[2];
#pragma unroll
        for (int h = 0; h < 2; ++h) {
          const float* wcol = wbuf + ((kc + h) * 16 + 8 * kg) * 32 + j;
          float wv[8];
#pragma unroll
          for (int t = 0; t < 8; ++t) wv[t] = wcol[32 * t];
          Mma<VT>::split(wv, bhi[h], blo[h]);
          const unsigned char* abase = vbuf + ((kc + h) * 16 + 8 * kg + ((lane & 15) >> 2)) * VP + (16 * ((lane >> 4) & 1) + 4 * (lane & 3)) * 2;
          typedef __attribute__((address_space(3))) s16x4 lds_s16x4;
          const s16x4 a00 = __builtin_amdgcn_ds_read_tr16_b64_v4i16((lds_s16x4*)(abase));
          const s16x4 a01 = __builtin_amdgcn_ds_read_tr16_b64_v4i16((lds_s16x4*)(abase + 4 * VP));
          const s16x4 a10 = __builtin_amdgcn_ds_read_tr16_b64_v4i16((lds_s16x4*)(abase + 64));
          const s16x4 a11 = __builtin_amdgcn_ds_read_tr16_b64_v4i16((lds_s16x4*)(abase + 4 * VP + 64));
          a0[h] = __builtin_shufflevector(a00, a01, 0, 1, 2, 3, 4, 5, 6, 7);
          a1[h] = __builtin_shufflevector(a10, a11, 0, 1, 2, 3, 4, 5, 6, 7);
        }
#pragma unroll
        for (int h = 0; h < 2; ++h) {
          acc0 = Mma<VT>::mfma(a0[h], bhi[h], acc0);
          acc1 = Mma<VT>::mfma(a1[h], bhi[h], acc1);
          acc0 = Mma<VT>::mfma(a0[h], blo[h], acc0);
          acc1 = Mma<VT>::mfma(a1[h], blo[h], acc1);
        }
      }
#pragma unroll
      for (int e = 0; e < 16; ++e) wbuf[wad[e]] = 0.f;
    }
  });

  if (live) {
    VT* dst = out + item * C + 4 * kg;
#pragma unroll
    for (int tile = 0; tile < 2; ++tile) {
#pragma unroll
      for (int bq = 0; bq < 4; ++bq) {
        float v[8];
#pragma unroll
        for (int t = 0; t < 4; ++t) {
          v[t] = tile == 0 ? acc0[4 * bq + t] : acc1[4 * bq + t];
          v[4 + t] = 0.f;
        }
        const u32x4 pk = Elem<VT>::pack(v);
        *reinterpret_cast<uint2*>(dst + tile * 32 + 8 * bq) = uint2{pk[0], pk[1]};
      }
    }
  }
}


template <typename LT>
__device__ __forceinline__ bool mma_level_points(const BrickOrder& order, int l, bool live, long item, int LP, int kg,
                                                 const LT* __restrict__ loc, const LT* __restrict__ attn,
                                                 MmaPoint (&pt)[2], MmaBox& box, float (&a_raw)[2]) {
  constexpr int P = 4;
  box = MmaBox{0, 0, 0, 0, 0, 0};
  a_raw[0] = a_raw[1] = 0.f;
  const int D = order.D[l], H = order.H[l], W = order.W[l];
  int lo_d = 32767, lo_h = 32767, lo_w = 32767, hi_d = -1, hi_h = -1, hi_w = -1;
  float lx[2] = {0.f, 0.f}, ly[2] = {0.f, 0.f}, lz[2] = {0.f, 0.f}, la[2] = {0.f, 0.f};
  if (live) {
    const long jx = item * LP + l * P + 2 * kg;
    if constexpr (sizeof(LT) == 4) {
      const float2 q0 = *reinterpret_cast<const float2*>(loc + 3 * jx), q1 = *reinterpret_cast<const float2*>(loc + 3 * jx + 2),
                   q2 = *reinterpret_cast<const float2*>(loc + 3 * jx + 4), qa = attn ? *reinterpret_cast<const float2*>(attn + jx) : float2{0.f, 0.f};
      lx[0] = q0.x; ly[0] = q0.y; lz[0] = q1.x; lx[1] = q1.y; ly[1] = q2.x; lz[1] = q2.y;
      la[0] = qa.x; la[1] = qa.y;
    } else {
#pragma unroll
      for (int pi = 0; pi < 2; ++pi) {
        lx[pi] = static_cast<float>(Elem<LT>::ld(loc + 3 * (jx + pi)));
        ly[pi] = static_cast<float>(Elem<LT>::ld(loc + 3 * (jx + pi) + 1));
        lz[pi] = static_cast<float>(Elem<LT>::ld(loc + 3 * (jx + pi) + 2));
        la[pi] = attn ? static_cast<float>(Elem<LT>::ld(attn + jx + pi)) : 0.f;
      }
    }
  }
  a_raw[0] = la[0]; a_raw[1] = la[1];
#pragma unroll
  for (int pi = 0; pi < 2; ++pi) {
    MmaPoint g{0x3fffffff, 0.f, 0.f, 0.f, 0.f};
    const float w_im = pixel_coord(lx[pi], W), h_im = pixel_coord(ly[pi], H), d_im = pixel_coord(lz[pi], D);
    if (live && d_im > -1.f && h_im > -1.f && w_im > -1.f && d_im < D && h_im < H && w_im < W) {
      const float fd = floorf(d_im), fh = floorf(h_im), fw = floorf(w_im);
      const int d0 = static_cast<int>(fd), h0 = static_cast<int>(fh), w0 = static_cast<int>(fw);
      g.dhw = (d0 + 1) | ((h0 + 1) << 10) | ((w0 + 1) << 20);
      g.ld = d_im - fd; g.lh = h_im - fh; g.lw = w_im - fw; g.a = la[pi];
      lo_d = min(lo_d, max(d0, 0)); hi_d = max(hi_d, min(d0 + 1, D - 1));
      lo_h = min(lo_h, max(h0, 0)); hi_h = max(hi_h, min(h0 + 1, H - 1));
      lo_w = min(lo_w, max(w0, 0)); hi_w = max(hi_w, min(w0 + 1, W - 1));
    }
    pt[pi] = g;
  }
  const int r0 = wave_min_pk16(pack16(lo_d, lo_h)), r1 = wave_min_pk16(pack16(lo_w, -hi_d)), r2 = wave_min_pk16(pack16(-hi_h, -hi_w));
  hi_d = -(r1 >> 16);
  if (hi_d < 0) return false;
  lo_d = static_cast<short>(r0); lo_h = r0 >> 16; lo_w = static_cast<short>(r1);
  hi_h = -static_cast<int>(static_cast<short>(r2)); hi_w = -(r2 >> 16);
  box = MmaBox{lo_d, lo_h, lo_w, hi_d - lo_d + 1, hi_h - lo_h + 1, hi_w - lo_w + 1};
  return true;
}

template <typename VT, typename LT>
__global__ __launch_bounds__(64, 2) void msda3d_bwd_query_mma(
    const VT* __restrict__ value, const LT* __restrict__ loc, const LT* __restrict__ attn,
    const VT* __restrict__ grad_out, LT* __restrict__ grad_loc, LT* __restrict__ grad_attn,
    int* __restrict__ cursor, PointR16* __restrict__ recs, unsigned long long* __restrict__ det_keys, int cells_per_slab,
    int S, int M, int L, unsigned value_bytes, long n_units, const BrickOrder* __restrict__ order_p,
    unsigned short* __restrict__ grad_proj = nullptr) {
  const BrickOrder& order = *order_p;
  constexpr int P = 4, C = 64, KB = kMmaKB, VP = kMmaVP, WR = kMmaWRows;
  __shared__ __attribute__((aligned(16))) unsigned char vbuf[KB * VP];
  __shared__ __attribute__((aligned(16))) float gbuf[WR * 32];

  const long u = xcd_contiguous_block(blockIdx.x, n_units);
  if (u < 0) return;
  const int lane = threadIdx.x;
  const int j = lane & 31, kg = lane >> 5;
  const int sb = static_cast<int>(u & 3);
  const long t1 = u >> 2;
  const int m = static_cast<int>(t1 % M);
  const long t2 = t1 / M;
  const int bricks = order.pad_start[order.L] >> 7;
  const int brick = bricks - 1 - static_cast<int>(t2 % bricks);
  const long b = t2 / bricks;
  const int slot = (2 * (sb >> 1) + (j >> 4)) * 32 + ((j >> 2) & 3) * 8 + 4 * (sb & 1) + (j & 3);
  const int s = brick_slot_to_row(order, brick * kBrickSlots + slot);
  const bool live = s >= 0;
  const long item = live ? (b * S + s) * M + m : 0;
  const int LP = L * P;
  const unsigned row_bytes = static_cast<unsigned>(M) * C * sizeof(VT);
  const unsigned head_off = static_cast<unsigned>((b * S * M + m) * C * sizeof(VT));
  const __amdgpu_buffer_rsrc_t rsrc =
      __builtin_amdgcn_make_buffer_rsrc(const_cast<VT*>(value), 0, static_cast<int>(value_bytes), 0x00020000);

  s16x8 gof[4];
#pragma unroll
  for (int sk = 0; sk < 4; ++sk) {
    u32x4 raw{0u, 0u, 0u, 0u};
    if (live) raw = *reinterpret_cast<const u32x4*>(grad_out + item * C + 16 * sk + 8 * kg);
    gof[sk] = __builtin_bit_cast(s16x8, raw);
  }

  MmaPoint pt[kMmaLevels][2];
  MmaBox box[kMmaLevels];
  float a_in[kMmaLevels][2];
  static_for<0, kMmaLevels>([&](auto lc) {
    constexpr int l = decltype(lc)::value;
    box[l] = MmaBox{0, 0, 0, 0, 0, 0};
    a_in[l][0] = a_in[l][1] = 0.f;
    if (l >= L) return;
    mma_level_points<LT>(order, l, live, item, LP, kg, loc, attn, pt[l], box[l], a_in[l]);
  });

  for (int i = lane; i < WR * 32 / 4; i += 64) reinterpret_cast<float4*>(gbuf)[i] = float4{0.f, 0.f, 0.f, 0.f};
  for (int i = lane; i < KB * VP / 16; i += 64) reinterpret_cast<float4*>(vbuf)[i] = float4{0.f, 0.f, 0.f, 0.f};

  const int st_row = lane >> 3, st_vec = lane & 7;
  auto load_block = [&](auto lc, int kb, u32x4 (&pre)[8]) {
    constexpr int l = decltype(lc)::value;
    const MmaBox bx = box[l];
    const int H = order.H[l], W = order.W[l], start = order.start[l];
    const int THW = bx.TH * bx.TW, R = bx.TD * THW;
    const float inv_thw = __builtin_amdgcn_rcpf(static_cast<float>(THW)), inv_tw = __builtin_amdgcn_rcpf(static_cast<float>(bx.TW));
    const int r = kb * KB + lane;
    const int rd = static_cast<int>((static_cast<float>(r) + 0.5f) * inv_thw), rr = r - __mul24(rd, THW);
    const int rh = static_cast<int>((static_cast<float>(rr) + 0.5f) * inv_tw), rw = rr - __mul24(rh, bx.TW);
    const int grow = start + __mul24(__mul24(bx.bd + rd, H) + (bx.bh + rh), W) + (bx.bw + rw);
    const unsigned past = static_cast<unsigned>((R - 1 - r) >> 31);
    const int row_off = static_cast<int>((head_off + __umul24(static_cast<unsigned>(grow), row_bytes)) | (past & 0xfffffff0u));
#pragma unroll
    for (int it = 0; it < 8; ++it) {
      const unsigned off = static_cast<unsigned>(__builtin_amdgcn_ds_bpermute((it * 8 + st_row) * 4, row_off)) + st_vec * 16u;
      pre[it] = __builtin_amdgcn_raw_buffer_load_b128(rsrc, off, 0, 0);
    }
  };

  u32x4 pre[8];
  bool have_pre = false;
  int cell_start = 0;
  float res_a[kMmaLevels][2], res_l[kMmaLevels][2][3];
  static_for<0, kMmaLevels>([&](auto lc) {
    constexpr int l = decltype(lc)::value;
#pragma unroll
    for (int pi = 0; pi < 2; ++pi) {
      res_a[l][pi] = 0.f;
      res_l[l][pi][0] = 0.f; res_l[l][pi][1] = 0.f; res_l[l][pi][2] = 0.f;
    }
  });
  static_for<0, kMmaLevels>([&](auto lc) {
    constexpr int l = decltype(lc)::value;
    if (l >= L) return;
    const int D = order.D[l], H = order.H[l], W = order.W[l];
    const int level_cells = (D + 1) * (H + 1) * (W + 1);
    const int my_cell_start = cell_start;
    cell_start += level_cells;
    if (box[l].TD == 0) return;
    const MmaBox bx = box[l];
    const int THW = bx.TH * bx.TW, R = bx.TD * THW;

    if (det_keys != nullptr) {
      const long slab_cell = static_cast<long>(b * M + m) * cells_per_slab + my_cell_start;
#pragma unroll
      for (int pi = 0; pi < 2; ++pi) {
        const MmaPoint g = pt[l][pi];
        if (g.dhw == 0x3fffffff) continue;
        const int c1d = g.dhw & 1023, c1h = (g.dhw >> 10) & 1023, c1w = (g.dhw >> 20) & 1023;
        const unsigned long long cell = static_cast<unsigned long long>(slab_cell + (c1d * (H + 1) + c1h) * (W + 1) + c1w);
        const unsigned slot = static_cast<unsigned>(item) * static_cast<unsigned>(LP) + static_cast<unsigned>(l * P + 2 * kg + pi);
        recs[slot] = make_point_r16(g.a, static_cast<int>(item), g.ld, g.lh, g.lw);
        det_keys[slot] = (cell << 32) | slot;
      }
    } else if (cursor != nullptr) {
      int* slab_cursor = cursor + static_cast<int>(b * M + m) * cells_per_slab + my_cell_start;
      int* hist = reinterpret_cast<int*>(gbuf);
      const int CH = bx.TH + 1, CW = bx.TW + 1;
      const int ncells = (bx.TD + 1) * CH * CW;
      const bool use_hist = ncells <= KB * 32;
      int rank[2] = {-1, -1}, lcell[2] = {0, 0};
      if (use_hist) {
        for (int c = lane; c < ncells; c += 64) hist[c] = 0;
      }
#pragma unroll
      for (int pi = 0; pi < 2; ++pi) {
        const int dhw = pt[l][pi].dhw;
        if (dhw == 0x3fffffff) continue;
        const int c1d = dhw & 1023, c1h = (dhw >> 10) & 1023, c1w = (dhw >> 20) & 1023;
        if (use_hist) {
          lcell[pi] = ((c1d - bx.bd) * CH + (c1h - bx.bh)) * CW + (c1w - bx.bw);
          rank[pi] = atomicAdd(&hist[lcell[pi]], 1);
        } else {
          rank[pi] = atomicAdd(slab_cursor + (c1d * (H + 1) + c1h) * (W + 1) + c1w, 1);
        }
      }
      if (use_hist) {
        const float inv_chw = __builtin_amdgcn_rcpf(static_cast<float>(CH * CW)), inv_cw = __builtin_amdgcn_rcpf(static_cast<float>(CW));
        for (int c0 = 0; c0 < ncells; c0 += 512) {
          int base[8];
#pragma unroll
          for (int k = 0; k < 8; ++k) {
            const int c = c0 + 64 * k + lane;
            const int n = c < ncells ? hist[c] : 0;
            base[k] = -1;
            if (n > 0) {
              const int cd = static_cast<int>((static_cast<float>(c) + 0.5f) * inv_chw), cr = c - cd * (CH * CW);
              const int ch = static_cast<int>((static_cast<float>(cr) + 0.5f) * inv_cw), cw = cr - ch * CW;
              base[k] = atomicAdd(slab_cursor + ((bx.bd + cd) * (H + 1) + (bx.bh + ch)) * (W + 1) + (bx.bw + cw), n);
            }
          }
#pragma unroll
          for (int k = 0; k < 8; ++k)
            if (base[k] >= 0) hist[c0 + 64 * k + lane] = base[k];
        }
#pragma unroll
        for (int pi = 0; pi < 2; ++pi)
          if (rank[pi] >= 0) rank[pi] += hist[lcell[pi]];
      }
#pragma unroll
      for (int pi = 0; pi < 2; ++pi) {
        const MmaPoint g = pt[l][pi];
        if (rank[pi] >= 0) recs[rank[pi]] = make_point_r16(g.a, static_cast<int>(item), g.ld, g.lh, g.lw);
      }
    }

    int ecol[16];
    float dots[16];
#pragma unroll
    for (int pi = 0; pi < 2; ++pi) {
      const MmaPoint g = pt[l][pi];
      const int d0 = (g.dhw & 1023) - 1, h0 = ((g.dhw >> 10) & 1023) - 1, w0 = ((g.dhw >> 20) & 1023) - 1;
      const bool okp = g.dhw != 0x3fffffff;
      const int cb = (__mul24(__mul24(d0 - bx.bd, bx.TH) + (h0 - bx.bh), bx.TW) + (w0 - bx.bw)) * 32 + j;
      const bool vd[2] = {okp && static_cast<unsigned>(d0) < static_cast<unsigned>(D), okp && static_cast<unsigned>(d0 + 1) < static_cast<unsigned>(D)};
      const bool vh[2] = {static_cast<unsigned>(h0) < static_cast<unsigned>(H), static_cast<unsigned>(h0 + 1) < static_cast<unsigned>(H)};
      const bool vw[2] = {static_cast<unsigned>(w0) < static_cast<unsigned>(W), static_cast<unsigned>(w0 + 1) < static_cast<unsigned>(W)};
#pragma unroll
      for (int c = 0; c < 4; ++c) {
        const int dd = c >> 1, dh = c & 1;
        const int col = cb + (dd ? THW * 32 : 0) + (dh ? bx.TW * 32 : 0);
#pragma unroll
        for (int dw = 0; dw < 2; ++dw) {
          ecol[pi * 8 + 2 * c + dw] = (vd[dd] && vh[dh] && vw[dw]) ? col + 32 * dw : -64;
          dots[pi * 8 + 2 * c + dw] = 0.f;
        }
      }
    }

    if (R > kMmaDenseRows) {
#pragma unroll 1
      for (int p4 = 0; p4 < 4; ++p4) {
        MmaPoint g = (p4 & 1) ? pt[l][1] : pt[l][0];
        MmaPoint o;
        o.dhw = __shfl_xor(g.dhw, 32, 64);
        const bool mine = (p4 >> 1) == kg;
        const int dhw = mine ? g.dhw : o.dhw;
        float part[8];
#pragma unroll
        for (int k = 0; k < 8; ++k) part[k] = 0.f;
        if (dhw != 0x3fffffff) {
          const int d0 = (dhw & 1023) - 1, h0 = ((dhw >> 10) & 1023) - 1, w0 = ((dhw >> 20) & 1023) - 1;
#pragma unroll 1
          for (int k = 0; k < 8; ++k) {
            const int dd = k >> 2, dh = (k >> 1) & 1, dw = k & 1;
            const int d = d0 + dd, h = h0 + dh, w = w0 + dw;
            float acc = 0.f;
            if (static_cast<unsigned>(d) < static_cast<unsigned>(D) && static_cast<unsigned>(h) < static_cast<unsigned>(H) &&
                static_cast<unsigned>(w) < static_cast<unsigned>(W)) {
              const long grow = order.start[l] + (static_cast<long>(d) * H + h) * W + w;
              const VT* src = value + ((b * S + grow) * M + m) * C + 8 * kg;
#pragma unroll
              for (int sk = 0; sk < 4; ++sk) {
                const u32x4 v = *reinterpret_cast<const u32x4*>(src + 16 * sk);
                const u32x4 gq = __builtin_bit_cast(u32x4, gof[sk]);
#pragma unroll
                for (int t = 0; t < 4; ++t) acc = Elem<VT>::dot2(v[t], gq[t], acc);
              }
            }
#pragma unroll
            for (int kk = 0; kk < 8; ++kk) part[kk] = kk == k ? acc : part[kk];
          }
        }
#pragma unroll
        for (int k = 0; k < 8; ++k) {
          const float full = part[k] + __shfl_xor(part[k], 32, 64);
          if (mine) {
            if (p4 & 1) dots[8 + k] = full;
            else dots[k] = full;
          }
        }
      }
      have_pre = false;
    } else {
      const int nblk = (R + KB - 1) / KB;
      if (!have_pre) load_block(lc, 0, pre);
      for (int kb = 0; kb < nblk; ++kb) {
        const int k0 = kb * KB;
        const int rows_here = min(KB, R - k0);
#pragma unroll
        for (int it = 0; it < 4; ++it) *reinterpret_cast<u32x4*>(vbuf + (it * 8 + st_row) * VP + st_vec * 16) = pre[it];
        if (rows_here > 32) {
#pragma unroll
          for (int it = 4; it < 8; ++it) *reinterpret_cast<u32x4*>(vbuf + (it * 8 + st_row) * VP + st_vec * 16) = pre[it];
        }
        have_pre = false;
        if (kb + 1 < nblk) {
          load_block(lc, kb + 1, pre);
          have_pre = true;
        } else if constexpr (l + 1 < kMmaLevels) {
          if (l + 1 < L && box[l + 1].TD != 0) {
            const MmaBox nb = box[l + 1];
            if (nb.TD * nb.TH * nb.TW <= kMmaDenseRows) {
              load_block(IntC<l + 1>{}, 0, pre);
              have_pre = true;
            }
          }
        }
        for (int tile = 0; tile * 32 < rows_here; ++tile) {
          f32x16 acc;
#pragma unroll
          for (int i = 0; i < 16; ++i) acc[i] = 0.f;
          const unsigned char* arow = vbuf + (tile * 32 + j) * VP + 16 * kg;
#pragma unroll
          for (int sk = 0; sk < 4; ++sk) {
            const s16x8 a = __builtin_bit_cast(s16x8, *reinterpret_cast<const u32x4*>(arow + 32 * sk));
            acc = Mma<VT>::mfma(a, gof[sk], acc);
          }
#pragma unroll
          for (int r = 0; r < 16; ++r) gbuf[(tile * 32 + (r & 3) + 8 * (r >> 2) + 4 * kg) * 32 + j] = acc[r];
        }
#pragma unroll
        for (int e = 0; e < 16; ++e)
          dots[e] += gbuf[min(static_cast<unsigned>(ecol[e] - k0 * 32), static_cast<unsigned>(KB * 32 + j))];
      }
    }

    if (live) {
#pragma unroll
      for (int pi = 0; pi < 2; ++pi) {
        const MmaPoint g = pt[l][pi];
        float pa = 0.f, px = 0.f, py = 0.f, pz = 0.f;
#pragma unroll
        for (int k = 0; k < 8; ++k) {
          const int dd = k >> 2, dh = (k >> 1) & 1, dw = k & 1;
          const float dot = dots[pi * 8 + k];
          const float wd = dd ? g.ld : 1.f - g.ld, wh = dh ? g.lh : 1.f - g.lh, ww = dw ? g.lw : 1.f - g.lw;
          pa += (wd * wh * ww) * dot;
          px += (dw ? dot : -dot) * (wd * wh);
          py += (dh ? dot : -dot) * (wd * ww);
          pz += (dd ? dot : -dot) * (wh * ww);
        }
        res_a[l][pi] = pa;
        res_l[l][pi][0] = px * g.a * static_cast<float>(W);
        res_l[l][pi][1] = py * g.a * static_cast<float>(H);
        res_l[l][pi][2] = pz * g.a * static_cast<float>(D);
      }
    }
  });

  if constexpr (sizeof(LT) == 4) {
    if (grad_proj != nullptr) {
      float part = 0.f;
      static_for<0, kMmaLevels>([&](auto lc) {
        constexpr int l = decltype(lc)::value;
        if (l >= L) return;
        part = fmaf(a_in[l][0], res_a[l][0], part);
        part = fmaf(a_in[l][1], res_a[l][1], part);
      });
      const float dot = part + __shfl_xor(part, 32, 64);
      unsigned* stage = reinterpret_cast<unsigned*>(vbuf);
      int* tok = reinterpret_cast<int*>(vbuf + 32 * 128);
      auto bf = [](float x) -> unsigned { return static_cast<unsigned>(f32_to_bf16(x)); };
      auto rnd = [](float x) -> float { return bf16_to_f32(f32_to_bf16(x)); };
      static_for<0, kMmaLevels>([&](auto lc) {
        constexpr int l = decltype(lc)::value;
        if (l >= L) return;
        const float sz[3] = {rnd(static_cast<float>(order.W[l])), rnd(static_cast<float>(order.H[l])), rnd(static_cast<float>(order.D[l]))};
        const float rc[3] = {__builtin_amdgcn_rcpf(sz[0]), __builtin_amdgcn_rcpf(sz[1]), __builtin_amdgcn_rcpf(sz[2])};
        unsigned o[6];
#pragma unroll
        for (int pi = 0; pi < 2; ++pi)
#pragma unroll
          for (int k = 0; k < 3; ++k) {
            const float x = rnd(res_l[l][pi][k]);
            const float q0 = x * rc[k];
            o[3 * pi + k] = bf(__builtin_fmaf(__builtin_fmaf(-q0, sz[k], x), rc[k], q0));
          }
        unsigned* dst = stage + j * 32 + l * 6 + kg * 3;
        dst[0] = o[0] | (o[1] << 16);
        dst[1] = o[2] | (o[3] << 16);
        dst[2] = o[4] | (o[5] << 16);
        stage[j * 32 + 24 + l * 2 + kg] = bf(a_in[l][0] * (res_a[l][0] - dot)) | (bf(a_in[l][1] * (res_a[l][1] - dot)) << 16);
      });
      if (kg == 0) tok[j] = live ? static_cast<int>(b * S + s) : -1;
      __syncthreads();
      const unsigned row_pieces = static_cast<unsigned>(M) * 8u;
#pragma unroll
      for (int it = 0; it < 4; ++it) {
        const int e = it * 64 + lane, q = e >> 3, pc = e & 7;
        const int t = tok[q];
        if (t < 0) continue;
        const u32x4 v = *reinterpret_cast<const u32x4*>(vbuf + q * 128 + pc * 16);
        const unsigned piece = pc < 6 ? static_cast<unsigned>(m) * 6u + pc : static_cast<unsigned>(M) * 6u + static_cast<unsigned>(m) * 2u + (pc - 6);
        *reinterpret_cast<u32x4*>(grad_proj + (static_cast<long>(t) * row_pieces + piece) * 8) = v;
      }
      return;
    }
  }
  if (live) {
    static_for<0, kMmaLevels>([&](auto lc) {
      constexpr int l = decltype(lc)::value;
      if (l >= L) return;
      const long jx = item * LP + l * P + 2 * kg;
      if constexpr (sizeof(LT) == 4) {
        *reinterpret_cast<float2*>(grad_attn + jx) = float2{res_a[l][0], res_a[l][1]};
        float2* gl = reinterpret_cast<float2*>(grad_loc + 3 * jx);
        gl[0] = float2{res_l[l][0][0], res_l[l][0][1]};
        gl[1] = float2{res_l[l][0][2], res_l[l][1][0]};
        gl[2] = float2{res_l[l][1][1], res_l[l][1][2]};
      } else {
#pragma unroll
        for (int pi = 0; pi < 2; ++pi) {
          Elem<LT>::st(grad_attn + jx + pi, res_a[l][pi]);
#pragma unroll
          for (int k = 0; k < 3; ++k) Elem<LT>::st(grad_loc + 3 * (jx + pi) + k, res_l[l][pi][k]);
        }
      }
    });
  }
}

template <typename LT>
__global__ __launch_bounds__(64) void msda3d_cell_count_mma(
    const LT* __restrict__ loc, int* __restrict__ count, int cells_per_slab, int S, int M, int L, long n_units,
    const BrickOrder* __restrict__ order_p) {
  const BrickOrder& order = *order_p;
  constexpr int P = 4, KB = kMmaKB;
  __shared__ int hist[KB * 32];

  const long u = xcd_contiguous_block(blockIdx.x, n_units);
  if (u < 0) return;
  const int lane = threadIdx.x;
  const int j = lane & 31, kg = lane >> 5;
  const int sb = static_cast<int>(u & 3);
  const long t1 = u >> 2;
  const int m = static_cast<int>(t1 % M);
  const long t2 = t1 / M;
  const int bricks = order.pad_start[order.L] >> 7;
  const int brick = bricks - 1 - static_cast<int>(t2 % bricks);
  const long b = t2 / bricks;
  const int slot = (2 * (sb >> 1) + (j >> 4)) * 32 + ((j >> 2) & 3) * 8 + 4 * (sb & 1) + (j & 3);
  const int s = brick_slot_to_row(order, brick * kBrickSlots + slot);
  const bool live = s >= 0;
  const long item = live ? (b * S + s) * M + m : 0;
  const int LP = L * P;

  int cell_start = 0;
  static_for<0, kMmaLevels>([&](auto lc) {
    constexpr int l = decltype(lc)::value;
    if (l >= L) return;
    const int D = order.D[l], H = order.H[l], W = order.W[l];
    const int my_cell_start = cell_start;
    cell_start += (D + 1) * (H + 1) * (W + 1);
    MmaPoint pt[2];
    MmaBox bx;
    float a_unused[2];
    if (!mma_level_points<LT>(order, l, live, item, LP, kg, loc, static_cast<const LT*>(nullptr), pt, bx, a_unused)) return;
    int* slab_count = count + static_cast<int>(b * M + m) * cells_per_slab + my_cell_start;
    const int CH = bx.TH + 1, CW = bx.TW + 1;
    const int ncells = (bx.TD + 1) * CH * CW;
    const bool use_hist = ncells <= KB * 32;
    if (use_hist) {
      for (int c = lane; c < ncells; c += 64) hist[c] = 0;
    }
#pragma unroll
    for (int pi = 0; pi < 2; ++pi) {
      const int dhw = pt[pi].dhw;
      if (dhw == 0x3fffffff) continue;
      const int c1d = dhw & 1023, c1h = (dhw >> 10) & 1023, c1w = (dhw >> 20) & 1023;
      if (use_hist) atomicAdd(&hist[((c1d - bx.bd) * CH + (c1h - bx.bh)) * CW + (c1w - bx.bw)], 1);
      else atomicAdd(slab_count + (c1d * (H + 1) + c1h) * (W + 1) + c1w, 1);
    }
    if (use_hist) {
      const float inv_chw = __builtin_amdgcn_rcpf(static_cast<float>(CH * CW)), inv_cw = __builtin_amdgcn_rcpf(static_cast<float>(CW));
      for (int c = lane; c < ncells; c += 64) {
        const int n = hist[c];
        if (n > 0) {
          const int cd = static_cast<int>((static_cast<float>(c) + 0.5f) * inv_chw), cr = c - cd * (CH * CW);
          const int ch = static_cast<int>((static_cast<float>(cr) + 0.5f) * inv_cw), cw = cr - ch * CW;
          atomicAdd(slab_count + ((bx.bd + cd) * (H + 1) + (bx.bh + ch)) * (W + 1) + (bx.bw + cw), n);
        }
      }
    }
  });
}

}
```

transoar_amd/csrc/msda3d_pcm.hpp:

```cpp
#pragma once
#include "msda3d_common.hpp"
#include "msda3d_mma.hpp"

namespace transoar {

constexpr int kPcmKB = 32;
constexpr int kPcmVP = 128;
constexpr int kPcmKW = 32;
constexpr int kPcmWP = kPcmKW + 4;
constexpr int kPcmBoxRows = 256;
constexpr int kPcmLevels = 4;
constexpr int kPcmPU = 272, kPcmPF = 136;
constexpr int kPcmSkip = 0x3fffffff;

template <typename VT> struct PcmW;
template <> struct PcmW<bf16_t> {
  static __device__ __forceinline__ unsigned split(float w) {
    const unsigned u = __float_as_uint(w);
    const float lo = w - __uint_as_float(u & 0xffff0000u);
    return __builtin_amdgcn_perm(u, __float_as_uint(lo), 0x07060302u);
  }
  static __device__ __forceinline__ unsigned pack2(float a, float b) {
    typedef float f32x2_t __attribute__((ext_vector_type(2)));
    typedef __bf16 bf16x2_t __attribute__((ext_vector_type(2)));
    return __builtin_bit_cast(unsigned, __builtin_convertvector(f32x2_t{a, b}, bf16x2_t));
  }
};
template <> struct PcmW<f16_t> {
  static __device__ __forceinline__ unsigned split(float w) {
    const _Float16 hi = static_cast<_Float16>(w);
    const _Float16 lo = static_cast<_Float16>(w - static_cast<float>(hi));
    return (static_cast<unsigned>(__builtin_bit_cast(unsigned short, hi)) << 16) | __builtin_bit_cast(unsigned short, lo);
  }
  static __device__ __forceinline__ unsigned pack2(float a, float b) {
    return (static_cast<unsigned>(__builtin_bit_cast(unsigned short, static_cast<_Float16>(b))) << 16) |
           __builtin_bit_cast(unsigned short, static_cast<_Float16>(a));
  }
};

__device__ __forceinline__ unsigned opaque_copy(unsigned v) {
  asm volatile("" : "+v"(v));
  return v;
}

__device__ __forceinline__ int half_min_pk16(int v) {
#define TRANSOAR_PCM_STEP(CTRL)                                                                  \
  {                                                                                              \
    const int o = __builtin_amdgcn_mov_dpp(v, CTRL, 0xf, 0xf, true);                             \
    v = __builtin_bit_cast(int, __builtin_elementwise_min(__builtin_bit_cast(s16x2, v), __builtin_bit_cast(s16x2, o))); \
  }
  TRANSOAR_PCM_STEP(0xB1)
  TRANSOAR_PCM_STEP(0x4E)
  TRANSOAR_PCM_STEP(0x141)
  TRANSOAR_PCM_STEP(0x140)
#undef TRANSOAR_PCM_STEP
  const int o = __builtin_amdgcn_update_dpp(v, v, 0x142, 0xa, 0xf, false);
  return __builtin_bit_cast(int, __builtin_elementwise_min(__builtin_bit_cast(s16x2, v), __builtin_bit_cast(s16x2, o)));
}
template <int CTRL>
__device__ __forceinline__ float quad_perm_f(float v) {
  return __int_as_float(__builtin_amdgcn_mov_dpp(__float_as_int(v), CTRL, 0xf, 0xf, true));
}
__device__ __forceinline__ void both_halves_f(float v, float& lo, float& hi) {
  const auto sw = __builtin_amdgcn_permlane32_swap(__float_as_uint(v), opaque_copy(__float_as_uint(v)), false, false);
  lo = __uint_as_float(sw[0]);
  hi = __uint_as_float(sw[1]);
}

__device__ __forceinline__ float bf16_round_f(float x) {
  unsigned u = __float_as_uint(x);
  u += 0x7fffu + ((u >> 16) & 1u);
  return __uint_as_float(u & 0xffff0000u);
}
__device__ __forceinline__ int sgpr(int v) { return __builtin_amdgcn_readfirstlane(v); }

__device__ __forceinline__ float pixel_coord_f(float loc, float size) {
#pragma clang fp contract(off)
  const float t = loc * size;
  return t - 0.5f;
}

struct PcmBox {
  int bd, bh, bw, TD, TH, TW;
};

struct PcmConst {
  BrickOrder order;
  float fD[4], fH[4], fW[4];
  float dD[4], dH[4], dW[4];
};

template <typename VT, bool FUSED>
__global__ __launch_bounds__(64, kPcmKW == 32 ? 4 : 3) void msda3d_fwd_pcm(
    const VT* __restrict__ value, const float* __restrict__ loc, const float* __restrict__ attn,
    const unsigned short* __restrict__ proj, const float* __restrict__ ref, unsigned ref_bstride,
    VT* __restrict__ out, int S, int M, int L, unsigned value_bytes, unsigned param_bytes, unsigned aux_bytes,
    unsigned n_units, const PcmConst* __restrict__ cst) {
  const BrickOrder& order = cst->order;
  constexpr int C = 64, KB = kPcmKB, KW = kPcmKW, VP = kPcmVP, WP = kPcmWP;
  __shared__ __attribute__((aligned(128))) unsigned char vbuf[KB * VP];
  __shared__ __attribute__((aligned(16))) unsigned wbuf[32 * WP];

  const unsigned per_xcd = (n_units + 7u) >> 3;
  const unsigned u = (blockIdx.x & 7u) * per_xcd + (blockIdx.x >> 3);
  if (u >= n_units) return;
  const int lane = threadIdx.x;
  const int kh = lane >> 5, n = lane & 31, q = n >> 2, p = n & 3;
  const unsigned sub = u & 15u;
  const unsigned t1 = u >> 4;
  const unsigned m = t1 % static_cast<unsigned>(M);
  const unsigned t2 = t1 / static_cast<unsigned>(M);
  const unsigned bricks = static_cast<unsigned>(order.pad_start[order.L]) >> 7;
  const int brick = static_cast<int>(bricks - 1u - t2 % bricks);
  const unsigned b = t2 / bricks;

  int lq = 0;
#pragma unroll
  for (int t = 1; t < kPcmLevels; ++t) lq += (t < order.L && brick * kBrickSlots >= order.pad_start[t]) ? 1 : 0;
  const int qD = order.D[lq], qH = order.H[lq], qW = order.W[lq];
  const unsigned lbrick = static_cast<unsigned>(brick - (order.pad_start[lq] >> 7));
  const unsigned nbw = static_cast<unsigned>(order.nbw[lq]), nbh = static_cast<unsigned>(order.nbh[lq]);
  const unsigned bwi = lbrick % nbw, brest = lbrick / nbw;
  const unsigned bhi = brest % nbh, bdi = brest / nbh;
  const int od = static_cast<int>(bdi * kBrickD + 2 * (sub >> 3)), oh = static_cast<int>(bhi * kBrickH + 2 * ((sub >> 2) & 1)),
            ow = static_cast<int>(bwi * kBrickW + 2 * (sub & 3));
  if (od >= qD || oh >= qH || ow >= qW) return;
  const int qbase = order.start[lq] + static_cast<int>(b) * S;
  auto row_of = [&](int qq) -> int {
    const int d = od + (qq >> 2), h = oh + ((qq >> 1) & 1), w = ow + (qq & 1);
    const int r = qbase + __mul24(__mul24(d, qH) + h, qW) + w;
    return (d < qD && h < qH && w < qW) ? r : -1;
  };
  const int s = row_of(q);
  const bool live = s >= 0;
  const unsigned row_bytes = static_cast<unsigned>(M) * C * sizeof(VT);
  const unsigned head_off = (b * static_cast<unsigned>(S) * M + m) * (C * sizeof(VT));
  const __amdgpu_buffer_rsrc_t rsrc =
      __builtin_amdgcn_make_buffer_rsrc(const_cast<VT*>(value), 0, static_cast<int>(value_bytes), 0x00020000);

  {
    const int r = lane & 15;
    const bool loc_piece = r < 12;
    const int lv = loc_piece ? r : 3 * (r - 12);
    const bool on = lv < 3 * L;
    if constexpr (FUSED) {
      const __amdgpu_buffer_rsrc_t prs = __builtin_amdgcn_make_buffer_rsrc(const_cast<unsigned short*>(proj), 0, static_cast<int>(param_bytes), 0x00020000);
      const unsigned cols2 = 8u * M * L * 4;
      const unsigned in_row = loc_piece ? (m * L * 12 + r * 4) * 2u : (3u * M * L * 4 + m * L * 4 + (r - 12) * 4) * 2u;
#pragma unroll
      for (int it = 0; it < 2; ++it) {
        const int qq = (lane >> 4) + 4 * it;
        const int sq = row_of(qq);
        const unsigned off = (on && sq >= 0) ? __umul24(static_cast<unsigned>(sq), cols2) + in_row : 0xfffffff0u;
        typedef unsigned u32x2_t __attribute__((ext_vector_type(2)));
        const u32x2_t v = __builtin_bit_cast(u32x2_t, __builtin_amdgcn_raw_buffer_load_b64(prs, off, 0, 0));
        *reinterpret_cast<u32x2_t*>(vbuf + qq * kPcmPF + r * 8) = v;
      }
    } else {
      const __amdgpu_buffer_rsrc_t lrs = __builtin_amdgcn_make_buffer_rsrc(const_cast<float*>(loc), 0, static_cast<int>(param_bytes), 0x00020000);
      const __amdgpu_buffer_rsrc_t ars = __builtin_amdgcn_make_buffer_rsrc(const_cast<float*>(attn), 0, static_cast<int>(aux_bytes), 0x00020000);
      const unsigned item_loc = static_cast<unsigned>(L) * 48u, item_attn = static_cast<unsigned>(L) * 16u;
#pragma unroll
      for (int it = 0; it < 2; ++it) {
        const int qq = (lane >> 4) + 4 * it;
        const int sq = row_of(qq);
        const unsigned item = __umul24(static_cast<unsigned>(sq), static_cast<unsigned>(M)) + m;
        const bool ok = on && sq >= 0;
        const unsigned loff = (ok && loc_piece) ? item * item_loc + r * 16 : 0xfffffff0u;
        const unsigned aoff = (ok && !loc_piece) ? item * item_attn + (r - 12) * 16 : 0xfffffff0u;
        const u32x4 vl = __builtin_amdgcn_raw_buffer_load_b128(lrs, loff, 0, 2);
        const u32x4 va = __builtin_amdgcn_raw_buffer_load_b128(ars, aoff, 0, 2);
        *reinterpret_cast<u32x4*>(vbuf + qq * kPcmPU + r * 16) = loc_piece ? vl : va;
      }
    }
  }

  float fl[2][3], fa[2];
  int dhw[2];
  int mn[3], mx[3];
  {
    float px[2][3];
    float fs[2][3];
    bool okl[2];
#pragma unroll
    for (int pi = 0; pi < 2; ++pi) {
      okl[pi] = live && 2 * kh + pi < L;
      fs[pi][0] = kh ? cst->fW[2 + pi] : cst->fW[pi];
      fs[pi][1] = kh ? cst->fH[2 + pi] : cst->fH[pi];
      fs[pi][2] = kh ? cst->fD[2 + pi] : cst->fD[pi];
    }
    if constexpr (FUSED) {
      const __amdgpu_buffer_rsrc_t rrs = __builtin_amdgcn_make_buffer_rsrc(const_cast<float*>(ref), 0, static_cast<int>(aux_bytes), 0x00020000);
      const unsigned short* pb = reinterpret_cast<const unsigned short*>(vbuf + q * kPcmPF);
      const unsigned rrow = live ? (static_cast<unsigned>(s) - b * static_cast<unsigned>(S)) * L * 12u + b * ref_bstride : 0xfffffff0u;
#pragma unroll
      for (int pi = 0; pi < 2; ++pi) {
        const int l = 2 * kh + pi;
        typedef float f32x3_t __attribute__((ext_vector_type(3)));
        const f32x3_t rp = __builtin_bit_cast(f32x3_t, __builtin_amdgcn_raw_buffer_load_b96(rrs, okl[pi] ? rrow + l * 12u : 0xfffffff0u, 0, 0));
        const float dv[3] = {kh ? cst->dW[2 + pi] : cst->dW[pi], kh ? cst->dH[2 + pi] : cst->dH[pi], kh ? cst->dD[2 + pi] : cst->dD[pi]};
        fa[pi] = okl[pi] ? bf16_to_f32(pb[48 + l * 4 + p]) : -3.0e38f;
#pragma unroll
        for (int k = 0; k < 3; ++k) {
          const float off = bf16_to_f32(pb[(l * 4 + p) * 3 + k]);
          const float rc = __builtin_amdgcn_rcpf(dv[k]);
          const float q0 = off * rc;
          const float qv = __builtin_fmaf(__builtin_fmaf(-q0, dv[k], off), rc, q0);
          px[pi][k] = rp[k] + bf16_round_f(qv);
        }
      }
      float mxl = fmaxf(fa[0], fa[1]);
      mxl = fmaxf(mxl, quad_perm_f<0xB1>(mxl));
      mxl = fmaxf(mxl, quad_perm_f<0x4E>(mxl));
      {
        float a0, a1;
        both_halves_f(mxl, a0, a1);
        mxl = fmaxf(a0, a1);
      }
      const float e0 = __expf(fa[0] - mxl), e1 = __expf(fa[1] - mxl);
      float sum = e0 + e1;
      sum += quad_perm_f<0xB1>(sum);
      sum += quad_perm_f<0x4E>(sum);
      {
        float a0, a1;
        both_halves_f(sum, a0, a1);
        sum = a0 + a1;
      }
      fa[0] = e0 / sum; fa[1] = e1 / sum;
    } else {
      const float* pb = reinterpret_cast<const float*>(vbuf + q * kPcmPU);
#pragma unroll
      for (int pi = 0; pi < 2; ++pi) {
        const int l = 2 * kh + pi;
        px[pi][0] = pb[(l * 4 + p) * 3]; px[pi][1] = pb[(l * 4 + p) * 3 + 1]; px[pi][2] = pb[(l * 4 + p) * 3 + 2];
        fa[pi] = pb[48 + l * 4 + p];
      }
    }
    int i0[2][3];
    unsigned okmask = 0u;
#pragma unroll
    for (int pi = 0; pi < 2; ++pi) {
      const float w_im = pixel_coord_f(px[pi][0], fs[pi][0]), h_im = pixel_coord_f(px[pi][1], fs[pi][1]), d_im = pixel_coord_f(px[pi][2], fs[pi][2]);
      const bool ok = okl[pi] && d_im > -1.f && h_im > -1.f && w_im > -1.f && d_im < fs[pi][2] && h_im < fs[pi][1] && w_im < fs[pi][0];
      const float fd = floorf(d_im), fh = floorf(h_im), fw = floorf(w_im);
      i0[pi][0] = static_cast<int>(fd); i0[pi][1] = static_cast<int>(fh); i0[pi][2] = static_cast<int>(fw);
      fl[pi][0] = d_im - fd; fl[pi][1] = h_im - fh; fl[pi][2] = w_im - fw;
      fa[pi] = ok ? fa[pi] : 0.f;
      dhw[pi] = ok ? (i0[pi][0] + 1) | ((i0[pi][1] + 1) << 10) | ((i0[pi][2] + 1) << 20) : kPcmSkip;
      okmask |= ok ? (pi ? 0xffff0000u : 0x0000ffffu) : 0u;
    }
#pragma unroll
    for (int k = 0; k < 3; ++k) {
      const unsigned pk = __builtin_amdgcn_perm(static_cast<unsigned>(i0[1][k]), static_cast<unsigned>(i0[0][k]), 0x05040100u);
      const int t0 = i0[0][k] + (fl[0][k == 0 ? 0 : k == 1 ? 1 : 2] > 0.f ? 1 : 0), t1 = i0[1][k] + (fl[1][k == 0 ? 0 : k == 1 ? 1 : 2] > 0.f ? 1 : 0);
      const unsigned tp = __builtin_amdgcn_perm(static_cast<unsigned>(t1), static_cast<unsigned>(t0), 0x05040100u);
      const unsigned ng = __builtin_bit_cast(unsigned, -__builtin_bit_cast(s16x2, tp));
      mn[k] = half_min_pk16(static_cast<int>((pk & okmask) | (0x7fff7fffu & ~okmask)));
      mx[k] = half_min_pk16(static_cast<int>((ng & okmask) | (0x7fff7fffu & ~okmask)));
    }
  }

  PcmBox box[kPcmLevels];
  int mode[kPcmLevels];
#pragma unroll
  for (int l = 0; l < kPcmLevels; ++l) {
    const int src = (l >> 1) * 32 + 31;
    int lo3[3], hi3[3];
#pragma unroll
    for (int k = 0; k < 3; ++k) {
      const int a = __builtin_amdgcn_readlane(mn[k], src), c = __builtin_amdgcn_readlane(mx[k], src);
      lo3[k] = (l & 1) ? (a >> 16) : static_cast<short>(a);
      hi3[k] = -((l & 1) ? (c >> 16) : static_cast<int>(static_cast<short>(c)));
    }
    box[l] = PcmBox{lo3[0], lo3[1], lo3[2], hi3[0] - lo3[0] + 1, hi3[1] - lo3[1] + 1, hi3[2] - lo3[2] + 1};
    mode[l] = (l >= L || lo3[0] == 32767) ? 0 : (box[l].TD * box[l].TH * box[l].TW <= kPcmBoxRows ? 1 : 2);
  }

  unsigned wq[kPcmLevels][4];
  int pdhw[kPcmLevels];
  {
    unsigned X[2][4], Y[2][4];
#pragma unroll
    for (int pi = 0; pi < 2; ++pi) {
      const float ld = fl[pi][0], lh = fl[pi][1], lw = fl[pi][2];
      const float wd[2] = {fa[pi] * (1.f - ld), fa[pi] * ld}, wh[2] = {1.f - lh, lh}, ww[2] = {1.f - lw, lw};
#pragma unroll
      for (int c = 0; c < 4; ++c) {
        const float f0 = wd[0] * wh[c >> 1], f1 = wd[1] * wh[c >> 1];
        X[pi][c] = PcmW<VT>::split(f0 * ww[c & 1]);
        Y[pi][c] = PcmW<VT>::split(f1 * ww[c & 1]);
      }
    }
#pragma unroll
    for (int pi = 0; pi < 2; ++pi) {
#pragma unroll
      for (int c = 0; c < 4; ++c) {
        const auto sw = __builtin_amdgcn_permlane32_swap(X[pi][c], Y[pi][c], false, false);
        wq[pi][c] = sw[0];
        wq[2 + pi][c] = sw[1];
      }
      const auto sd = __builtin_amdgcn_permlane32_swap(static_cast<unsigned>(dhw[pi]), opaque_copy(static_cast<unsigned>(dhw[pi])), false, false);
      pdhw[pi] = static_cast<int>(sd[0]);
      pdhw[2 + pi] = static_cast<int>(sd[1]);
    }
  }

  f32x16 acc0, acc1;
#pragma unroll
  for (int i = 0; i < 16; ++i) { acc0[i] = 0.f; acc1[i] = 0.f; }
  for (int i = lane; i < 32 * WP / 2; i += 64) reinterpret_cast<uint2*>(wbuf)[i] = uint2{0u, 0u};

  auto row_offsets = [&](auto lc, int k0) -> int {
    constexpr int l = decltype(lc)::value;
    const PcmBox bx = box[l];
    const int D = order.D[l], H = order.H[l], W = order.W[l], start = order.start[l];
    const int r = k0 + lane;
    int d, h, w;
    bool ok;
    if (mode[l] == 1) {
      const int THW = bx.TH * bx.TW, R = bx.TD * THW;
      const float inv_thw = __builtin_amdgcn_rcpf(static_cast<float>(THW)), inv_tw = __builtin_amdgcn_rcpf(static_cast<float>(bx.TW));
      const int rd = static_cast<int>((static_cast<float>(r) + 0.5f) * inv_thw), rr = r - __mul24(rd, THW);
      const int rh = static_cast<int>((static_cast<float>(rr) + 0.5f) * inv_tw), rw = rr - __mul24(rh, bx.TW);
      d = bx.bd + rd; h = bx.bh + rh; w = bx.bw + rw;
      ok = r < R;
    } else {
      const int pd = __builtin_amdgcn_ds_bpermute((r >> 3) * 4, pdhw[l]);
      d = (pd & 1023) - 1 + ((r >> 2) & 1); h = ((pd >> 10) & 1023) - 1 + ((r >> 1) & 1); w = ((pd >> 20) & 1023) - 1 + (r & 1);
      ok = pd != kPcmSkip;
    }
    ok = ok && static_cast<unsigned>(d) < static_cast<unsigned>(D) && static_cast<unsigned>(h) < static_cast<unsigned>(H) &&
         static_cast<unsigned>(w) < static_cast<unsigned>(W);
    const int grow = start + __mul24(__mul24(d, H) + h, W) + w;
    return ok ? static_cast<int>(head_off + __umul24(static_cast<unsigned>(grow), row_bytes)) : static_cast<int>(0xffffff00u);
  };
  const int st_row = lane >> 3, st_vec = lane & 7;
  const int st_swz = (st_vec ^ ((st_row & 2) << 1)) * 16;
  auto issue_loads = [&](int row_off, int half, u32x4 (&pre)[4]) {
#pragma unroll
    for (int it = 0; it < 4; ++it) {
      const unsigned off = static_cast<unsigned>(__builtin_amdgcn_ds_bpermute((half * 32 + it * 8 + st_row) * 4, row_off)) + st_vec * 16u;
      pre[it] = __builtin_amdgcn_raw_buffer_load_b128(rsrc, off, 0, 0);
    }
  };

  u32x4 pre[4];
  bool have_pre = false;
  int row_off = 0;
  const int tr_off0 = ((16 * ((lane >> 4) & 1) + 4 * (lane & 3)) * 2) ^ ((((lane & 15) >> 2) & 2) << 5), tr_off1 = tr_off0 ^ 64;
  unsigned* const wcol = wbuf + n * WP;
  const int spare = KW + (n >> 3);
  static_for<0, kPcmLevels>([&](auto lc) {
    constexpr int l = decltype(lc)::value;
    if (mode[l] == 0) return;
    const PcmBox bx = box[l];
    const int THW = bx.TH * bx.TW;
    const int R = mode[l] == 1 ? bx.TD * THW : 256;
    int col[4];
    if (mode[l] == 1) {
      const int pd = pdhw[l];
      const int d1 = pd & 1023, h1 = (pd >> 10) & 1023, w1 = pd >> 20;
      const int base = __mul24(__mul24(bx.bd + 1, bx.TH) + (bx.bh + 1), bx.TW) + (bx.bw + 1);
      const int c0 = pd == kPcmSkip ? 0 : __mul24(__mul24(d1 + kh, bx.TH) + h1, bx.TW) + w1 - base;
      col[0] = c0; col[1] = c0 + 1; col[2] = c0 + bx.TW; col[3] = c0 + bx.TW + 1;
    } else {
#pragma unroll
      for (int c = 0; c < 4; ++c) col[c] = n * 8 + kh * 4 + c;
    }
    const int nh = (R + KB - 1) / KB;
    if (!have_pre) {
      row_off = row_offsets(lc, 0);
      issue_loads(row_off, 0, pre);
    }
    int wad[4];
    for (int hb = 0; hb < nh; ++hb) {
      const int half = hb & 1;
      const int sub = hb & (KW / KB - 1);
      const int nch = (min(KB, R - hb * KB) + 15) >> 4;
#pragma unroll
      for (int it = 0; it < 2; ++it) *reinterpret_cast<u32x4*>(vbuf + (it * 8 + st_row) * VP + st_swz) = pre[it];
      if (nch > 1) {
#pragma unroll
        for (int it = 2; it < 4; ++it) *reinterpret_cast<u32x4*>(vbuf + (it * 8 + st_row) * VP + st_swz) = pre[it];
      }
      if (sub == 0) {
        const int k0 = hb * KB;
#pragma unroll
        for (int c = 0; c < 4; ++c) {
          const unsigned t = static_cast<unsigned>(col[c] - k0);
          wad[c] = (t < static_cast<unsigned>(KW) && wq[l][c] != 0u) ? static_cast<int>(t) : spare;
          wcol[wad[c]] = wq[l][c];
        }
      }
      have_pre = false;
      if (hb + 1 < nh) {
        if (half == 1) row_off = row_offsets(lc, (hb + 1) * KB);
        issue_loads(row_off, half ^ 1, pre);
        have_pre = true;
      } else if constexpr (l + 1 < kPcmLevels) {
        if (mode[l + 1] != 0) {
          row_off = row_offsets(IntC<l + 1>{}, 0);
          issue_loads(row_off, 0, pre);
          have_pre = true;
        }
      }
#pragma unroll
      for (int kc = 0; kc < 2; ++kc) {
        if (kc >= nch) break;
        const unsigned* wp = wcol + sub * KB + kc * 16 + 8 * kh;
        const u32x4 p0 = *reinterpret_cast<const u32x4*>(wp);
        const u32x4 p1 = *reinterpret_cast<const u32x4*>(wp + 4);
        const u32x4 ahi{__builtin_amdgcn_perm(p0[1], p0[0], 0x07060302u), __builtin_amdgcn_perm(p0[3], p0[2], 0x07060302u),
                        __builtin_amdgcn_perm(p1[1], p1[0], 0x07060302u), __builtin_amdgcn_perm(p1[3], p1[2], 0x07060302u)};
        const u32x4 alo{__builtin_amdgcn_perm(p0[1], p0[0], 0x05040100u), __builtin_amdgcn_perm(p0[3], p0[2], 0x05040100u),
                        __builtin_amdgcn_perm(p1[1], p1[0], 0x05040100u), __builtin_amdgcn_perm(p1[3], p1[2], 0x05040100u)};
        const unsigned char* vrow = vbuf + (kc * 16 + 8 * kh + ((lane & 15) >> 2)) * VP;
        typedef __attribute__((address_space(3))) s16x4 lds_s16x4;
        const s16x4 b00 = __builtin_amdgcn_ds_read_tr16_b64_v4i16((lds_s16x4*)(vrow + tr_off0));
        const s16x4 b01 = __builtin_amdgcn_ds_read_tr16_b64_v4i16((lds_s16x4*)(vrow + 4 * VP + tr_off0));
        const s16x4 b10 = __builtin_amdgcn_ds_read_tr16_b64_v4i16((lds_s16x4*)(vrow + tr_off1));
        const s16x4 b11 = __builtin_amdgcn_ds_read_tr16_b64_v4i16((lds_s16x4*)(vrow + 4 * VP + tr_off1));
        const s16x8 v0 = __builtin_shufflevector(b00, b01, 0, 1, 2, 3, 4, 5, 6, 7);
        const s16x8 v1 = __builtin_shufflevector(b10, b11, 0, 1, 2, 3, 4, 5, 6, 7);
        const s16x8 whi = __builtin_bit_cast(s16x8, ahi), wlo = __builtin_bit_cast(s16x8, alo);
        acc0 = Mma<VT>::mfma(whi, v0, acc0);
        acc1 = Mma<VT>::mfma(whi, v1, acc1);
        acc0 = Mma<VT>::mfma(wlo, v0, acc0);
        acc1 = Mma<VT>::mfma(wlo, v1, acc1);
      }
      if (sub == KW / KB - 1 || hb + 1 == nh) {
#pragma unroll
        for (int c = 0; c < 4; ++c) wcol[wad[c]] = 0u;
      }
    }
  });

  {
    unsigned short* ob = reinterpret_cast<unsigned short*>(vbuf);
#pragma unroll
    for (int g = 0; g < 4; ++g) {
      const float v0 = (acc0[4 * g] + acc0[4 * g + 1]) + (acc0[4 * g + 2] + acc0[4 * g + 3]);
      const float v1 = (acc1[4 * g] + acc1[4 * g + 1]) + (acc1[4 * g + 2] + acc1[4 * g + 3]);
      const unsigned pk = PcmW<VT>::pack2(v0, v1);
      ob[(2 * g + kh) * C + n] = static_cast<unsigned short>(pk);
      ob[(2 * g + kh) * C + 32 + n] = static_cast<unsigned short>(pk >> 16);
    }
    const int sq = row_of(lane >> 3);
    const u32x4 line = *reinterpret_cast<const u32x4*>(vbuf + (lane >> 3) * 128 + (lane & 7) * 16);
    const __amdgpu_buffer_rsrc_t ors = __builtin_amdgcn_make_buffer_rsrc(out, 0, static_cast<int>(value_bytes), 0x00020000);
    const unsigned ooff = sq >= 0 ? (__umul24(static_cast<unsigned>(sq), static_cast<unsigned>(M)) + m) * (C * sizeof(VT)) + (lane & 7) * 16u : 0xfffffff0u;
    __builtin_amdgcn_raw_buffer_store_b128(line, ors, ooff, 0, 2);
  }
}

}
```

transoar_amd/ms_deform_attn.py:

```python
import itertools
import math
import warnings

import torch
import torch.nn.functional as F
from torch import nn
from torch.autograd import Function
from torch.autograd.function import once_differentiable

from . import msda as MSDA
from .token_linear import token_linear
from .tokens import (sampling_head as _sampling_head, sampling_head_backward_raw as _head_bwd_raw,
                     sampling_head_raw as _head_raw, sampling_head_usable as _sampling_head_usable)

_debug_core = None


def _fused_usable(value, proj, reference_points, shapes, m, lv, pt, lq, s):
    if torch.is_grad_enabled() and (value.requires_grad or proj.requires_grad):
        return False
    return (MSDA.locality_hint and not (MSDA.flags & 0x35) and lq == s and pt == 4 and lv <= 4
            and value.dtype in (torch.bfloat16, torch.float16) and value.shape[-1] == 64 and value.is_contiguous()
            and _sampling_head_usable(proj, reference_points, shapes, m, lv, pt))


def register_debug_core(fn):
    global _debug_core
    prev, _debug_core = _debug_core, fn
    return prev


class MSDeformAttnFunction(Function):

    @staticmethod
    def forward(ctx, value, value_spatial_shapes, value_level_start_index,
                sampling_locations, attention_weights, im2col_step):
        ctx.im2col_step = im2col_step
        out = MSDA.ms_deform_attn_forward(value, value_spatial_shapes, value_level_start_index,
                                          sampling_locations, attention_weights, im2col_step)
        ctx.save_for_backward(value, value_spatial_shapes, value_level_start_index,
                              sampling_locations, attention_weights)
        return out

    @staticmethod
    @once_differentiable
    def backward(ctx, grad_output):
        value, shapes, starts, loc, attn = ctx.saved_tensors
        g_value, g_loc, g_attn = MSDA.ms_deform_attn_backward(
            value, shapes, starts, loc, attn, grad_output.contiguous(), ctx.im2col_step)
        return g_value, None, None, g_loc, g_attn, None


class _HeadGather(Function):

    @staticmethod
    def forward(ctx, value, proj, reference_points, shapes, level_start, m, lv, pt, im2col_step):
        loc, attn = _head_raw(proj, reference_points, shapes, m, lv, pt)
        out = MSDA.ms_deform_attn_forward(value, shapes, level_start, loc, attn, im2col_step)
        ctx.save_for_backward(value, shapes, level_start, loc, attn)
        ctx.head = (m, lv, pt, tuple(proj.shape), im2col_step)
        return out

    @staticmethod
    @once_differentiable
    def backward(ctx, grad_output):
        value, shapes, starts, loc, attn = ctx.saved_tensors
        m, lv, pt, proj_shape, step = ctx.head
        grad_output = grad_output.contiguous()
        res = MSDA.ms_deform_attn_backward_proj(value, shapes, starts, loc, attn, grad_output, step)
        if res is None:
            g_value, g_loc, g_attn = MSDA.ms_deform_attn_backward(value, shapes, starts, loc, attn, grad_output, step)
            g_proj = _head_bwd_raw(g_loc.contiguous(), g_attn.contiguous(), attn, shapes, m, lv, pt, proj_shape)
        else:
            g_value, g_proj = res
        return g_value, g_proj, None, None, None, None, None, None, None


HEAD_GATHER = __import__("os").environ.get("TRANSOAR_HEAD_GATHER", "1") != "0"


def _axis_directions(n_heads):
    lattice = [v for v in itertools.product((-1.0, 0.0, 1.0), repeat=3)]
    if n_heads == 6:
        keep = [v for v in lattice if sum(abs(c) for c in v) == 1]
    elif n_heads == 26:
        keep = [v for v in lattice if any(c != 0 for c in v)]
    else:
        raise ValueError("Only nheads of value 26 or 6 are supported.")
    return torch.tensor(keep, dtype=torch.float32)


class MSDeformAttn(nn.Module):
    def __init__(self, d_model=256, n_levels=4, n_heads=8, n_points=4, use_cuda=True):
        super().__init__()
        if d_model % n_heads:
            raise ValueError("d_model must be divisible by n_heads, but got %d and %d" % (d_model, n_heads))
        head_dim = d_model // n_heads
        if head_dim & (head_dim - 1):
            warnings.warn("MSDeformAttn: a power-of-two head dimension keeps the gfx950 kernels on "
                          "their vectorised path (C*elt in {128,256,512} bytes).")
        self.im2col_step = 64
        self.d_model, self.n_levels, self.n_heads, self.n_points = d_model, n_levels, n_heads, n_points
        self.use_cuda = use_cuda

        self.sampling_offsets = nn.Linear(d_model, n_heads * n_levels * n_points * 3)
        self.attention_weights = nn.Linear(d_model, n_heads * n_levels * n_points)
        self.value_proj = nn.Linear(d_model, d_model)
        self.output_proj = nn.Linear(d_model, d_model)
        self._reset_parameters()

    def _reset_parameters(self):
        step = torch.arange(1, self.n_points + 1, dtype=torch.float32)
        bias = _axis_directions(self.n_heads)[:, None, None, :] * step[None, None, :, None]
        bias = bias.expand(self.n_heads, self.n_levels, self.n_points, 3)
        with torch.no_grad():
            self.sampling_offsets.weight.zero_()
            self.sampling_offsets.bias.copy_(bias.reshape(-1))
            self.attention_weights.weight.zero_()
            self.attention_weights.bias.zero_()
            nn.init.xavier_uniform_(self.value_proj.weight)
            self.value_proj.bias.zero_()
            nn.init.xavier_uniform_(self.output_proj.weight)
            self.output_proj.bias.zero_()

    def forward(self, query, reference_points, input_flatten, input_spatial_shapes,
                input_level_start_index, input_padding_mask=None):
        n, lq, _ = query.shape
        s = input_flatten.shape[1]
        if reference_points.shape[-1] != 3:
            raise ValueError("Last dim of reference_points must be 3 (x, y, z), got %d"
                             % reference_points.shape[-1])
        m, lv, pt = self.n_heads, self.n_levels, self.n_points

        value = token_linear(input_flatten, self.value_proj.weight, self.value_proj.bias)
        if input_padding_mask is not None:
            value = value.masked_fill(input_padding_mask[..., None], 0.0)
        value = value.view(n, s, m, self.d_model // m)

        n_off = self.sampling_offsets.out_features
        proj = token_linear(query, self.sampling_offsets.weight,
                            torch.cat((self.sampling_offsets.bias, self.attention_weights.bias)),
                            weight2=self.attention_weights.weight)
        if self.use_cuda and _fused_usable(value, proj, reference_points, input_spatial_shapes, m, lv, pt, lq, s):
            sampled = MSDA.ms_deform_attn_forward_fused(value, input_spatial_shapes, proj, reference_points, strict=False)
            if sampled is not None:
                return token_linear(sampled, self.output_proj.weight, self.output_proj.bias)
        if (self.use_cuda and HEAD_GATHER and lv == 4 and pt == 4 and torch.is_grad_enabled()
                and value.dtype in (torch.bfloat16, torch.float16)
                and _sampling_head_usable(proj, reference_points, input_spatial_shapes, m, lv, pt)):
            sampled = _HeadGather.apply(value, proj, reference_points, input_spatial_shapes, input_level_start_index,
                                        m, lv, pt, self.im2col_step)
            return token_linear(sampled, self.output_proj.weight, self.output_proj.bias)
        if self.use_cuda and _sampling_head_usable(proj, reference_points, input_spatial_shapes, m, lv, pt):
            locations, weights = _sampling_head(proj, reference_points, input_spatial_shapes, m, lv, pt)
        else:
            offsets = proj[..., :n_off].unflatten(-1, (m, lv, pt, 3))
            weights = F.softmax(proj[..., n_off:].unflatten(-1, (m, lv * pt)), dim=-1)
            weights = weights.view(n, lq, m, lv, pt)
            whd = input_spatial_shapes.flip(-1).to(offsets.dtype)
            locations = reference_points[:, :, None, :, None, :] + offsets / whd[None, None, None, :, None, :]

        if self.use_cuda:
            sampled = MSDeformAttnFunction.apply(value, input_spatial_shapes, input_level_start_index,
                                                 locations, weights, self.im2col_step)
        else:
            if _debug_core is None:
                raise RuntimeError(
                    "MSDeformAttn(use_cuda=False): this package has no CPU path. The reference's "
                    "debug core lives in oracle/torch_ref.py; a test harness may inject it with "
                    "transoar_amd.ms_deform_attn.register_debug_core().")
            sampled = _debug_core(value, input_spatial_shapes, locations, weights)
        return token_linear(sampled, self.output_proj.weight, self.output_proj.bias)
```

transoar_amd/msda.py:

```python
import ctypes
import os

import torch

from . import _native

_DT = {torch.float32: _native.F32, torch.float64: _native.F64,
       torch.bfloat16: _native.BF16, torch.float16: _native.F16}

flags = int(os.environ.get("TRANSOAR_MSDA_FLAGS", "0"))
DETERMINISTIC = 64
ERR_MODE = -8
deterministic = os.environ.get("TRANSOAR_MSDA_DETERMINISTIC", "0") == "1"


locality_hint = True


def _shapes_on_host(spatial_shapes):
    if not locality_hint:
        return None, None
    hit = getattr(spatial_shapes, "_transoar_host_shapes", None)
    if hit is None or hit[0] != spatial_shapes._version:
        vals = [int(v) for v in spatial_shapes.flatten().tolist()]
        hit = (spatial_shapes._version, (ctypes.c_int64 * len(vals))(*vals))
        spatial_shapes._transoar_host_shapes = hit
    return hit[1], ctypes.addressof(hit[1])


def _require(cond, msg):
    if not cond:
        raise RuntimeError(msg)


def _check_inputs(named):
    for name, t in named:
        _require(t.is_contiguous(), "%s tensor has to be contiguous" % name)
    if not named[0][1].is_cuda:
        raise RuntimeError("Not implemented on the CPU")
    dev = named[0][1].device
    for name, t in named:
        _require(t.is_cuda and t.device == dev, "%s must be a CUDA tensor on %s" % (name, dev))


def _dims(value, spatial_shapes, level_start_index, sampling_loc, attn_weight, im2col_step):
    _require(value.dim() == 4, "value must be (N, S, M, C)")
    _require(sampling_loc.dim() == 6 and sampling_loc.size(-1) == 3,
             "sampling_loc must be (N, Lq, M, L, P, 3)")
    N, S, M, C = value.shape
    L = spatial_shapes.size(0)
    Lq, P = sampling_loc.size(1), sampling_loc.size(4)
    _require(spatial_shapes.dtype == torch.int64 and tuple(spatial_shapes.shape) == (L, 3),
             "spatial_shapes must be int64 (L, 3)")
    _require(level_start_index.dtype == torch.int64 and tuple(level_start_index.shape) == (L,),
             "level_start_index must be int64 (L,)")
    _require(tuple(sampling_loc.shape) == (N, Lq, M, L, P, 3), "sampling_loc shape mismatch")
    _require(tuple(attn_weight.shape) == (N, Lq, M, L, P), "attn_weight shape mismatch")
    step = min(N, int(im2col_step))
    _require(step > 0 and N % step == 0,
             "batch(%d) must divide im2col_step(%d)" % (N, step))
    _require(value.dtype in _DT, "unsupported value dtype %s" % value.dtype)
    return N, S, M, C, L, Lq, P


def _coerce_loc(value, sampling_loc, attn_weight):
    half = value.dtype in (torch.bfloat16, torch.float16)
    if sampling_loc.dtype != attn_weight.dtype or not (
            sampling_loc.dtype == value.dtype or (half and sampling_loc.dtype == torch.float32)):
        want = torch.float32 if half else value.dtype
        sampling_loc = sampling_loc.to(want).contiguous()
        attn_weight = attn_weight.to(want).contiguous()
    return sampling_loc, attn_weight


def ms_deform_attn_forward(value, spatial_shapes, level_start_index, sampling_loc, attn_weight,
                           im2col_step):
    _check_inputs([("value", value), ("spatial_shapes", spatial_shapes),
                   ("level_start_index", level_start_index), ("sampling_loc", sampling_loc),
                   ("attn_weight", attn_weight)])
    N, S, M, C, L, Lq, P = _dims(value, spatial_shapes, level_start_index, sampling_loc,
                                 attn_weight, im2col_step)
    sampling_loc, attn_weight = _coerce_loc(value, sampling_loc, attn_weight)
    out = torch.empty((N, Lq, M * C), dtype=value.dtype, device=value.device)
    _keep, host_ptr = _shapes_on_host(spatial_shapes)
    _native.launch(_native.lib.transoar_msda3d_forward, value,
                   value.data_ptr(), spatial_shapes.data_ptr(), level_start_index.data_ptr(),
                   sampling_loc.data_ptr(), attn_weight.data_ptr(), out.data_ptr(),
                   N, S, M, C, L, Lq, P, _DT[value.dtype], _DT[sampling_loc.dtype], host_ptr, flags)
    return out


def ms_deform_attn_forward_fused(value, spatial_shapes, proj, reference_points, strict=True):
    _check_inputs([("value", value), ("spatial_shapes", spatial_shapes), ("proj", proj),
                   ("reference_points", reference_points)])
    _require(value.dim() == 4 and value.dtype in (torch.bfloat16, torch.float16), "value must be 16-bit (N, S, M, C)")
    N, S, M, C = value.shape
    L = spatial_shapes.size(0)
    P = proj.size(-1) // (4 * M * L)
    _require(proj.dtype == torch.bfloat16 and tuple(proj.shape) == (N, S, 4 * M * L * P), "proj must be bf16 (N, S, 4*M*L*P)")
    _require(reference_points.dtype == torch.float32 and reference_points.dim() == 4 and
             tuple(reference_points.shape[1:]) == (S, L, 3) and reference_points.size(0) in (1, N),
             "reference_points must be fp32 (1 or N, S, L, 3)")
    out = torch.empty((N, S, M * C), dtype=value.dtype, device=value.device)
    _keep, host_ptr = _shapes_on_host(spatial_shapes)
    _require(host_ptr is not None, "the fused gather needs the level shapes on the host (locality_hint)")
    rc = _native.launch(_native.lib.transoar_msda3d_forward_fused, value,
                        value.data_ptr(), proj.data_ptr(), reference_points.data_ptr(), reference_points.size(0) * S,
                        out.data_ptr(), N, S, M, C, L, P, _DT[value.dtype], host_ptr, ok=() if strict else (-2,))
    return None if rc else out


def ms_deform_attn_backward(value, spatial_shapes, level_start_index, sampling_loc, attn_weight,
                            grad_output, im2col_step):
    _check_inputs([("value", value), ("spatial_shapes", spatial_shapes),
                   ("level_start_index", level_start_index), ("sampling_loc", sampling_loc),
                   ("attn_weight", attn_weight), ("grad_output", grad_output)])
    N, S, M, C, L, Lq, P = _dims(value, spatial_shapes, level_start_index, sampling_loc,
                                 attn_weight, im2col_step)
    _require(tuple(grad_output.shape) == (N, Lq, M * C) and grad_output.dtype == value.dtype,
             "grad_output must be (N, Lq, M*C) with value's dtype")
    loc_in_dtype, attn_in_dtype = sampling_loc.dtype, attn_weight.dtype
    sampling_loc, attn_weight = _coerce_loc(value, sampling_loc, attn_weight)
    grad_value = torch.empty_like(value)
    grad_loc = torch.empty_like(sampling_loc)
    grad_attn = torch.empty_like(attn_weight)
    dims = (N, S, M, C, L, Lq, P, _DT[value.dtype], _DT[sampling_loc.dtype])
    _keep, host_ptr = _shapes_on_host(spatial_shapes)
    torch_det = torch.are_deterministic_algorithms_enabled()

    def run(call_flags, ok=()):
        ws_bytes = _native.lib.transoar_msda3d_backward_workspace_bytes(*dims, call_flags)
        workspace = torch.empty(max(ws_bytes, 16), dtype=torch.uint8, device=value.device)
        return _native.launch(_native.lib.transoar_msda3d_backward, value,
                              value.data_ptr(), spatial_shapes.data_ptr(), level_start_index.data_ptr(),
                              sampling_loc.data_ptr(), attn_weight.data_ptr(), grad_output.data_ptr(),
                              grad_value.data_ptr(), grad_loc.data_ptr(), grad_attn.data_ptr(),
                              workspace.data_ptr(), ws_bytes, *dims, host_ptr, call_flags, ok=ok)

    strict = deterministic or bool(flags & DETERMINISTIC)
    if strict or torch_det:
        if run(flags | DETERMINISTIC, ok=() if strict else (ERR_MODE,)) == ERR_MODE:
            if not torch.is_deterministic_algorithms_warn_only_enabled():
                raise RuntimeError("ms_deform_attn_backward does not have a deterministic implementation for this form (16-bit "
                                   "storage, 64 channels, 4 points, <= 4 levels with queries = the pyramid's voxels are covered), "
                                   "but torch.use_deterministic_algorithms(True) is set; use warn_only=True to run the default order")
            import warnings
            warnings.warn("ms_deform_attn_backward: no deterministic implementation for this form; running the default "
                          "(atomic-order dependent) accumulation")
            run(flags)
    else:
        run(flags)
    return [grad_value, grad_loc.to(loc_in_dtype), grad_attn.to(attn_in_dtype)]


def ms_deform_attn_backward_proj(value, spatial_shapes, level_start_index, sampling_loc, attn_weight, grad_output, im2col_step):
    _check_inputs([("value", value), ("spatial_shapes", spatial_shapes), ("level_start_index", level_start_index),
                   ("sampling_loc", sampling_loc), ("attn_weight", attn_weight), ("grad_output", grad_output)])
    N, S, M, C, L, Lq, P = _dims(value, spatial_shapes, level_start_index, sampling_loc, attn_weight, im2col_step)
    _require(tuple(grad_output.shape) == (N, Lq, M * C) and grad_output.dtype == value.dtype,
             "grad_output must be (N, Lq, M*C) with value's dtype")
    if sampling_loc.dtype != torch.float32 or attn_weight.dtype != torch.float32 or value.dtype not in (torch.bfloat16, torch.float16):
        return None
    call_flags = flags | (DETERMINISTIC if (deterministic or torch.are_deterministic_algorithms_enabled()) else 0)
    grad_value = torch.empty_like(value)
    grad_proj = torch.empty((N, Lq, 4 * M * L * P), dtype=torch.bfloat16, device=value.device)
    dims = (N, S, M, C, L, Lq, P, _DT[value.dtype], _DT[sampling_loc.dtype])
    _keep, host_ptr = _shapes_on_host(spatial_shapes)
    ws_bytes = _native.lib.transoar_msda3d_backward_workspace_bytes(*dims, call_flags)
    workspace = torch.empty(max(ws_bytes, 16), dtype=torch.uint8, device=value.device)
    rc = _native.launch(_native.lib.transoar_msda3d_backward_proj, value,
                        value.data_ptr(), spatial_shapes.data_ptr(), level_start_index.data_ptr(), sampling_loc.data_ptr(),
                        attn_weight.data_ptr(), grad_output.data_ptr(), grad_value.data_ptr(), grad_proj.data_ptr(),
                        workspace.data_ptr(), ws_bytes, *dims, host_ptr, call_flags, ok=(ERR_MODE,))
    return None if rc else [grad_value, grad_proj]
```

transoar_amd/refine_block.py:

```python
import copy
import os

import torch
import torch.nn.functional as F
from torch import nn

from .ms_deform_attn import MSDeformAttn
from .token_linear import fused_ffn, fused_ffn_usable, linear_relu_dropout, linear_relu_dropout_usable, token_linear

FUSED_FFN1 = os.environ.get("TRANSOAR_FUSED_FFN1", "1") != "0"
from . import tokens as fused_tokens
from .position_encoding import is_constant


class _MapToTokens(torch.autograd.Function):

    @staticmethod
    def forward(ctx, fmap):
        from .conv3d import to_ndhwc
        ctx.shape = fmap.shape
        n, c = fmap.shape[:2]
        return to_ndhwc(fmap).permute(0, 2, 3, 4, 1).reshape(n, -1, c)

    @staticmethod
    def backward(ctx, g):
        from .conv3d import Conv3dK3, to_ncdhw
        n, c, d, h, w = ctx.shape
        g = g.contiguous().view(n, d, h, w, c).permute(0, 4, 1, 2, 3)
        if Conv3dK3.ndhwc_everywhere and g.dtype == torch.bfloat16:
            return g
        return to_ncdhw(g) if g.dtype == torch.bfloat16 else g.contiguous()


def map_to_tokens(fmap):
    if fmap.is_cuda and fmap.dtype == torch.bfloat16 and fmap.shape[1] % 8 == 0:
        return _MapToTokens.apply(fmap)
    return fmap.flatten(2).transpose(1, 2)


def tokens_to_map(tokens, shape):
    n, _, c = tokens.shape
    if tokens.stride(2) == 1 and tokens.stride(1) == c:
        return tokens.view(n, *shape, c).permute(0, 4, 1, 2, 3)
    return tokens.transpose(1, 2).reshape(n, c, *shape)


def _activation(name):
    try:
        return {"relu": F.relu, "gelu": F.gelu, "glu": F.glu}[name]
    except KeyError:
        raise RuntimeError("activation should be relu/gelu, not %s." % name)


class DefAttnLayer(nn.Module):

    def __init__(self, d_model, d_ffn, dropout, activation, n_levels, n_heads, n_points, use_cuda):
        super().__init__()
        self.self_attn = MSDeformAttn(d_model, n_levels, n_heads, n_points, use_cuda)
        self.dropout1 = nn.Dropout(dropout)
        self.norm1 = nn.LayerNorm(d_model)
        self.linear1 = nn.Linear(d_model, d_ffn)
        self.activation = _activation(activation)
        self.dropout2 = nn.Dropout(dropout)
        self.linear2 = nn.Linear(d_ffn, d_model)
        self.dropout3 = nn.Dropout(dropout)
        self.norm2 = nn.LayerNorm(d_model)

    def forward(self, src, pos, reference_points, spatial_shapes, level_start_index, padding_mask=None):
        query = src if pos is None else src + pos
        attn = self.self_attn(query, reference_points, src, spatial_shapes, level_start_index, padding_mask)
        src = self.norm1(src + self.dropout1(attn))
        hidden = self.dropout2(self.activation(token_linear(src, self.linear1.weight, self.linear1.bias)))
        ffn = token_linear(hidden, self.linear2.weight, self.linear2.bias)
        return self.norm2(src + self.dropout3(ffn))

    def forward_fused(self, x, x16, q16, reference_points, spatial_shapes, level_start_index, pos_pack=()):
        attn = self.self_attn(q16, reference_points, x16, spatial_shapes, level_start_index)
        y32, y16, _ = fused_tokens.add_layernorm(x, attn.contiguous(), self.norm1, dropout=self.dropout1)
        if (self.activation is F.relu and fused_tokens.SEEDED_DROPOUT and FUSED_FFN1
                and fused_ffn_usable(y16, self.linear1.weight, self.linear2.weight)):
            ffn = fused_ffn(y16, self.linear1, self.linear2, self.dropout2)
            return fused_tokens.add_layernorm(y32, ffn.contiguous(), self.norm2, *pos_pack, dropout=self.dropout3)
        if (self.activation is F.relu and fused_tokens.SEEDED_DROPOUT and FUSED_FFN1
                and linear_relu_dropout_usable(y16, self.linear1.weight)):
            hidden = linear_relu_dropout(y16, self.linear1.weight, self.linear1.bias, self.dropout2)
        else:
            hidden = token_linear(y16, self.linear1.weight, self.linear1.bias)
            if self.activation is F.relu and hidden.dtype == torch.bfloat16 and hidden.numel() % 8 == 0:
                hidden = fused_tokens.relu_dropout(hidden, self.dropout2)
            else:
                hidden = self.dropout2(self.activation(hidden))
        ffn = token_linear(hidden, self.linear2.weight, self.linear2.bias)
        return fused_tokens.add_layernorm(y32, ffn.contiguous(), self.norm2, *pos_pack, dropout=self.dropout3)


class DefAttnTransformer(nn.Module):
    def __init__(self, layer, num_layers):
        super().__init__()
        self.layers = nn.ModuleList(copy.deepcopy(layer) for _ in range(num_layers))
        self.num_layers = num_layers

    @staticmethod
    def get_reference_points(spatial_shapes, device):
        per_level = []
        for d, h, w in spatial_shapes.tolist():
            z = (torch.arange(d, dtype=torch.float32, device=device) + 0.5) / d
            y = (torch.arange(h, dtype=torch.float32, device=device) + 0.5) / h
            x = (torch.arange(w, dtype=torch.float32, device=device) + 0.5) / w
            grid = torch.stack((x[None, None, :].expand(d, h, w), y[None, :, None].expand(d, h, w),
                                z[:, None, None].expand(d, h, w)), dim=-1)
            per_level.append(grid.reshape(-1, 3))
        pts = torch.cat(per_level, 0)
        return pts[None, :, None, :].expand(1, -1, spatial_shapes.shape[0], -1).contiguous()

    def forward(self, src, spatial_shapes, level_start_index, pos=None, reference_points=None):
        if reference_points is None:
            reference_points = self.get_reference_points(spatial_shapes, src.device)
        out = src
        for layer in self.layers:
            out = layer(out, pos, reference_points, spatial_shapes, level_start_index)
        return out


class DecoderDefAttnBlock(nn.Module):
    def __init__(self, d_model, nhead, num_layers, dim_feedforward, dropout, feature_levels,
                 n_points, use_cuda=True, activation="relu"):
        super().__init__()
        self.d_model, self.nhead, self.feature_levels = d_model, nhead, feature_levels
        n_levels = len(feature_levels)
        layer = DefAttnLayer(d_model, dim_feedforward, dropout, activation, n_levels, nhead, n_points, use_cuda)
        self.refine_def_attn = DefAttnTransformer(layer, num_layers)
        self.level_embed = nn.Parameter(torch.empty(n_levels, d_model))
        self._geometry = {}
        self._reset_parameters()

    def _reset_parameters(self):
        for p in self.parameters():
            if p.dim() > 1:
                nn.init.xavier_uniform_(p)
        for m in self.modules():
            if isinstance(m, MSDeformAttn):
                m._reset_parameters()
        nn.init.normal_(self.level_embed)

    def _level_geometry(self, shapes, device):
        key = (shapes, device)
        geo = self._geometry.get(key)
        if geo is None:
            spatial = torch.as_tensor(shapes, dtype=torch.long, device=device)
            sizes = [d * h * w for d, h, w in shapes]
            starts = torch.as_tensor([sum(sizes[:i]) for i in range(len(sizes))], dtype=torch.long, device=device)
            ref = DefAttnTransformer.get_reference_points(spatial, device)
            geo = (spatial, starts, sizes, ref)
            self._geometry[key] = geo
        return geo

    def forward(self, fmaps, pos_embeds):
        shapes = tuple(tuple(f.shape[2:]) for f in fmaps)
        spatial, starts, sizes, ref = self._level_geometry(shapes, fmaps[0].device)
        tokens = torch.cat([map_to_tokens(f) for f in fmaps], dim=1)
        if self._fused_ok(tokens, pos_embeds):
            memory = self._forward_fused(tokens, pos_embeds, shapes, spatial, starts, sizes, ref)
        else:
            pos = torch.cat([self._pos_tokens(p, lvl) + self.level_embed[lvl].view(1, 1, -1).to(p.dtype)
                             for lvl, p in enumerate(pos_embeds)], dim=1)
            memory = self.refine_def_attn(tokens, spatial, starts, pos, ref)
        return [tokens_to_map(m, shape) for m, shape in zip(memory.split(sizes, dim=1), shapes)]

    bf16_out = os.environ.get("TRANSOAR_REFINE_FP32_OUT", "0") != "1"

    def _fused_ok(self, tokens, pos_embeds):
        return (tokens.is_cuda and tokens.dtype == torch.bfloat16 and tokens.is_contiguous()
                and torch.is_autocast_enabled() and torch.get_autocast_gpu_dtype() == torch.bfloat16
                and all(is_constant(p) for p in pos_embeds)
                and fused_tokens.usable(tokens, None, self.d_model))

    def _forward_fused(self, tokens, pos_embeds, shapes, spatial, starts, sizes, ref):
        key = ("pos_sine", shapes, tokens.device)
        const = self._geometry.get(key)
        if const is None:
            sine = torch.cat([self._pos_tokens(p, lvl)[0] for lvl, p in enumerate(pos_embeds)], dim=0)
            const = self._geometry[key] = (sine.float().contiguous(), starts.int().contiguous())
        pos_sine, starts32 = const
        pos_pack = (pos_sine, self.level_embed, starts32)
        layers = self.refine_def_attn.layers
        q16 = fused_tokens.pos_query(tokens, pos_sine, self.level_embed, starts32)
        x, x16 = tokens, tokens
        for i, layer in enumerate(layers):
            last = i == len(layers) - 1
            x, x16, q16 = layer.forward_fused(x, x16, q16, ref, spatial, starts, () if last else pos_pack)
        return x16 if DecoderDefAttnBlock.bf16_out else x

    def _pos_tokens(self, pos_map, lvl):
        key = ("pos", lvl, tuple(pos_map.shape), pos_map.device)
        if not is_constant(pos_map):
            return pos_map.flatten(2).transpose(1, 2)
        hit = self._geometry.get(key)
        if hit is None:
            hit = self._geometry[key] = pos_map.flatten(2).transpose(1, 2).contiguous()
        return hit
```

transoar_amd/transoarnet.py:

```python
import itertools

import torch
import torch.nn.functional as F
from torch import nn

from . import seg_proxy, shadow
from .backbone import AttnFPN
from .criterion import TransoarCriterion
from .focused_decoder import FocusedDecoder
from .matcher import Matcher
from .position_encoding import PositionEmbeddingLearned3D, PositionEmbeddingSine3D


def build_backbone(config):
    return AttnFPN(config)


def build_neck(config, bbox_props):
    return FocusedDecoder(d_model=config["hidden_dim"], nhead=config["nheads"],
                          num_decoder_layers=config["dec_layers"], dim_feedforward=config["dim_feedforward"],
                          dropout=config["dropout"], activation="relu", return_intermediate_dec=True,
                          bbox_props=bbox_props, config=config)


def build_pos_enc(config):
    if config["pos_encoding"] == "sine":
        return PositionEmbeddingSine3D(channels=config["hidden_dim"])
    if config["pos_encoding"] == "learned":
        return PositionEmbeddingLearned3D(channels=config["hidden_dim"])
    raise ValueError("Please select a implemented pos. encoding.")


def build_criterion(config):
    matcher = Matcher(cost_class=config["set_cost_class"], cost_bbox=config["set_cost_bbox"],
                      cost_giou=config["set_cost_giou"], anchor_matching=config["anchor_matching"],
                      num_organs=config["neck"]["num_organs"])
    return TransoarCriterion(num_classes=config["num_classes"], matcher=matcher,
                             seg_proxy=config["backbone"]["use_seg_proxy_loss"],
                             seg_fg_bg=config["backbone"]["fg_bg"])


class MLP(nn.Module):
    def __init__(self, input_dim, hidden_dim, output_dim, num_layers):
        super().__init__()
        self.num_layers = num_layers
        dims = [input_dim] + [hidden_dim] * (num_layers - 1) + [output_dim]
        self.layers = nn.ModuleList(nn.Linear(a, b) for a, b in zip(dims[:-1], dims[1:]))

    def forward(self, x):
        for layer in self.layers[:-1]:
            x = F.relu(shadow.linear(x, layer.weight, layer.bias))
        return shadow.linear(x, self.layers[-1].weight, self.layers[-1].bias)


def generate_anchors(neck_config, bbox_props):
    n_q, n_org = neck_config["num_queries"], neck_config["num_organs"]
    qpo = int(n_q / n_org)
    dynamic = neck_config["anchor_gen_dynamic_offset"]
    anchors, pos_limits = [], []
    for props in bbox_props.values():
        median = torch.tensor(props["median"], dtype=torch.float32)
        vol = torch.tensor(props["attn_area"], dtype=torch.float32)
        centre, extent = (vol[:3] + vol[3:]) / 2, vol[3:] - vol[:3]
        if dynamic:
            o = (extent - median[3:]) / 3
            per_axis = [torch.stack((o[a], -o[a], torch.zeros(()))) for a in range(3)]
        else:
            fixed = float(neck_config["anchor_gen_offset"])
            per_axis = [torch.tensor([0.0, fixed, -fixed])] * 3
        if qpo == 1:
            shifts = torch.zeros(1, 3)
        else:
            shifts = torch.tensor(list(itertools.product(*[ax.tolist() for ax in per_axis])), dtype=torch.float32)
            if qpo == 7:
                shifts = shifts[(shifts != 0).sum(-1) <= 1]
        anchors.append(torch.cat((shifts + centre, median[3:].expand(shifts.shape[0], 3)), dim=-1))
        pos_limits.append(shifts.max(dim=0).values)
    med = torch.tensor([p["median"] for p in bbox_props.values()], dtype=torch.float32)[:, 3:]
    lo = torch.tensor([p["min"] for p in bbox_props.values()], dtype=torch.float32)[:, 3:]
    hi = torch.tensor([p["max"] for p in bbox_props.values()], dtype=torch.float32)[:, 3:]
    size_limits = torch.max(med - lo, hi - med)
    restriction = torch.cat((torch.stack(pos_limits), size_limits), dim=-1).repeat_interleave(qpo, dim=0)
    return torch.cat(anchors).clamp(min=0, max=1), restriction


class TransoarNet(nn.Module):
    def __init__(self, config):
        super().__init__()
        neck = config["neck"]
        hidden = neck["hidden_dim"]
        self._input_levels = neck["input_levels"]
        self._anchor_offset = neck["anchor_offset_pred"]
        self._aux_loss = neck["aux_loss"]

        self._backbone = build_backbone(config["backbone"])

        anchors, restrictions = generate_anchors(neck, config["bbox_properties"])
        if not neck["anchor_gen_dynamic_offset"]:
            restrictions = torch.full_like(restrictions, float(neck["max_anchor_pred_offset"]))
        restrictions[:, :3] /= 2
        self.register_buffer("_anchors", anchors, persistent=False)
        self.register_buffer("_restrictions", restrictions, persistent=False)

        self._neck = build_neck(neck, config["bbox_properties"])
        self._cls_head = nn.Linear(hidden, 1)
        self._reg_head = MLP(hidden, hidden, 6, 3)

        self._seg_proxy = config["backbone"]["use_seg_proxy_loss"]
        if self._seg_proxy:
            n_out = 2 if config["backbone"]["fg_bg"] else neck["num_organs"] + 1
            self._seg_head = nn.Conv3d(config["backbone"]["start_channels"], n_out, kernel_size=1, stride=1)

        self._query_embed = nn.Embedding(neck["num_queries"], hidden * 2)
        self._pos_enc = build_pos_enc(neck)
        if self._anchor_offset:
            for t in (self._cls_head.weight, self._cls_head.bias,
                      self._reg_head.layers[-1].weight, self._reg_head.layers[-1].bias):
                nn.init.zeros_(t)

    def forward(self, x):
        feats = self._backbone(x)
        det_src = feats[self._input_levels]
        hs = self._neck(det_src, self._query_embed.weight, self._pos_enc(det_src))
        logits = shadow.linear(hs, self._cls_head.weight, self._cls_head.bias)
        boxes = self._reg_head(hs)
        if self._anchor_offset:
            boxes = (boxes.tanh() * self._restrictions + self._anchors).clamp(min=0, max=1)
        else:
            boxes = boxes.sigmoid()
        pred_seg = 0
        if self._seg_proxy:
            p0 = feats["P0"]
            pred_seg = seg_proxy.seg_head(p0, self._seg_head) if seg_proxy.head_usable(p0, self._seg_head) else self._seg_head(p0)
        out = {"pred_logits": logits[-1], "pred_boxes": boxes[-1], "pred_seg": pred_seg}
        if self._aux_loss:
            out["aux_outputs"] = [{"pred_logits": a, "pred_boxes": b} for a, b in zip(logits[:-1], boxes[:-1])]
        return out
```

Baseline: 64.37.

## Compute last refine layer's deformable attention only for query levels read downstream

In the final decoder deformable-attention layer, queries are computed only for the leading feature levels the network actually consumes (the detection input level and P0 when the seg proxy is on). Only those query bricks are launched, and the outputs and gradients for the remaining rows are zeroed. A deterministic backward still walks all bricks but writes only the live ones. This removes forward and backward sampling work for unused query rows, at the cost of extra dispatch paths, fallback checks and dropping the unused refined outputs.

Measured after the change: 64.32. Within noise of the previous version (-0.1%).

```diff
diff --git a/include/transoar_msda3d.h b/include/transoar_msda3d.h
--- a/include/transoar_msda3d.h
+++ b/include/transoar_msda3d.h
@@ -37,6 +37,8 @@
 #define TRANSOAR_MSDA3D_Q16 128u
 #define TRANSOAR_MSDA3D_DETERMINISTIC 64u
 #define TRANSOAR_MSDA3D_PULL_HEAD_MAJOR 2u
+#define TRANSOAR_MSDA3D_QUERY_LEVELS_SHIFT 8
+#define TRANSOAR_MSDA3D_QUERY_LEVELS(k) (((unsigned)(k) & 15u) << TRANSOAR_MSDA3D_QUERY_LEVELS_SHIFT)
 
 int transoar_msda3d_forward(const void* value, const int64_t* spatial_shapes,
                             const int64_t* level_start_index,
diff --git a/transoar_amd/backbone.py b/transoar_amd/backbone.py
--- a/transoar_amd/backbone.py
+++ b/transoar_amd/backbone.py
@@ -124,6 +124,7 @@
         self._num_stages = n_stages
         self._refine_fmaps = config["use_decoder_attn"]
         self._refine_feature_levels = list(config["feature_levels"])
+        self.read_levels = None
         self._seg_proxy = config["use_seg_proxy_loss"]
         fpn = int(config["fpn_channels"])
         enc_channels = [config["start_channels"] * 2 ** s for s in range(n_stages)]
@@ -185,13 +186,23 @@
 
         if self._refine_fmaps:
             fmaps = [outputs[name] for name in self._refine_feature_levels]
-            refined = self._refine(fmaps, [self._pos_enc(f) for f in fmaps])
+            k = self._read_refine_levels()
+            refined = self._refine(fmaps, [self._pos_enc(f) for f in fmaps], read_levels=k)
             outputs.update(zip(self._refine_feature_levels, refined))
+            for name in self._refine_feature_levels[len(refined):]:
+                del outputs[name]
         if self._debug:
             print("AttnFPN decoder shapes:", {k: list(v.shape) for k, v in outputs.items()})
             self._debug = False
         return outputs
 
+    def _read_refine_levels(self):
+        if self.read_levels is None:
+            return None
+        read = [name in self.read_levels for name in self._refine_feature_levels]
+        k = sum(read)
+        return k if 0 < k < len(read) and all(read[:k]) else None
+
 
 class AttnFPN(nn.Module):
     def __init__(self, fpn_config, debug=False):
diff --git a/transoar_amd/csrc/msda3d.hip b/transoar_amd/csrc/msda3d.hip
--- a/transoar_amd/csrc/msda3d.hip
+++ b/transoar_amd/csrc/msda3d.hip
@@ -93,7 +93,7 @@
   return -1;
 }
 
-static BrickOrder make_order(const int64_t* host_shapes, const Dims& d, int rows) {
+static BrickOrder make_order(const int64_t* host_shapes, const Dims& d, int rows, int q_levels = 0, bool walk_all = false) {
   BrickOrder o{};
   if (!host_shapes || rows != d.S) return o;
   long start = 0, pad = 0;
@@ -110,6 +110,8 @@
   }
   if (start != d.S || pad * d.N * d.M >= (1L << 31)) return BrickOrder{};
   o.pad_start[d.L] = static_cast<int>(pad);
+  o.q_write_bricks = o.pad_start[q_levels > 0 && q_levels < d.L ? q_levels : d.L] >> 7;
+  o.q_bricks = walk_all ? o.pad_start[d.L] >> 7 : o.q_write_bricks;
   o.L = d.L;
   o.enabled = 1;
   return o;
@@ -233,6 +235,11 @@
   }
   return c;
 }
+static inline int query_levels(unsigned flags, int L) {
+  const int k = static_cast<int>((flags >> TRANSOAR_MSDA3D_QUERY_LEVELS_SHIFT) & 15u);
+  if (k > L) return -1;
+  return k == L ? 0 : k;
+}
 static int env_int(const char* name, int dflt) {
   const char* v = getenv(name);
   return (v && *v) ? atoi(v) : dflt;
@@ -243,10 +250,17 @@
                       const void* loc, const void* attn, void* out, const Dims& d,
                       const int64_t* host_shapes, unsigned flags, hipStream_t st) {
   const long n_items = static_cast<long>(d.N) * d.Lq * d.M;
-  const BrickOrder order = make_order(host_shapes, d, d.Lq);
+  const int ql = query_levels(flags, d.L);
+  if (ql < 0) return TRANSOAR_ERR_LEVELS;
+  const BrickOrder order = make_order(host_shapes, d, d.Lq, ql);
   const long n_units = order_units(order, d, d.Lq);
   const long n_blocks = ((order.enabled ? n_units : n_items) + kWavesPerBlock - 1) / kWavesPerBlock;
   const int lg = vec_lpv(d, sizeof(VT), flags);
+  if (ql > 0) {
+    bool covered = sizeof(VT) == 2 && sizeof(LT) == 4 && lg >= 0 && d.L <= kMmaLevels && pcm_ok(order, d) &&
+                   !(flags & (TRANSOAR_MSDA3D_NO_BRICK | TRANSOAR_MSDA3D_NO_MMA | TRANSOAR_MSDA3D_MMA_Q32 | TRANSOAR_MSDA3D_Q16));
+    if (!covered) return TRANSOAR_ERR_MODE;
+  }
   const dim3 block(64 * kWavesPerBlock);
   auto v = static_cast<const VT*>(value);
   auto lo = static_cast<const LT*>(loc);
@@ -281,7 +295,7 @@
       if (lg >= 0 && small && pcm_ok(order, d) &&
           !(flags & (TRANSOAR_MSDA3D_NO_BRICK | TRANSOAR_MSDA3D_NO_MMA | TRANSOAR_MSDA3D_MMA_Q32))) {
         ProfScope prof(TRANSOAR_PROF_FWD, st);
-        const long n_wave = static_cast<long>(d.N) * (order.pad_start[order.L] >> 7) * d.M * 16;
+        const long n_wave = static_cast<long>(d.N) * order.q_bricks * d.M * 16;
         const unsigned vbytes = static_cast<unsigned>(static_cast<long>(d.N) * d.S * d.M * d.C * sizeof(VT));
         const long n_pts = static_cast<long>(d.N) * d.Lq * d.M * d.L * d.P;
         const PcmConst* cst = device_const(make_pcm_const(order), st);
@@ -338,7 +352,7 @@
   if (vec_lpv(d, sizeof(VT), 0) < 0 || !pcm_ok(order, d)) return TRANSOAR_ERR_DIM;
   if (ref_rows != d.Lq && ref_rows != static_cast<long>(d.N) * d.Lq) return TRANSOAR_ERR_DIM;
   ProfScope prof(TRANSOAR_PROF_FWD, st);
-  const long n_wave = static_cast<long>(d.N) * (order.pad_start[order.L] >> 7) * d.M * 16;
+  const long n_wave = static_cast<long>(d.N) * order.q_bricks * d.M * 16;
   const unsigned vbytes = static_cast<unsigned>(static_cast<long>(d.N) * d.S * d.M * d.C * sizeof(VT));
   const PcmConst* cst = device_const(make_pcm_const(order), st);
   if (cst == nullptr) return TRANSOAR_ERR_CONST;
@@ -382,10 +396,13 @@
   if (workspace_bytes < bwd_workspace_bytes<VT, LT>(d, flags)) return TRANSOAR_ERR_WORKSPACE;
   if (grad_proj != nullptr && (sizeof(VT) != 2 || sizeof(LT) != 4 || vec_lpv(d, sizeof(VT), flags) < 0)) return TRANSOAR_ERR_MODE;
   const long n_items = static_cast<long>(d.N) * d.Lq * d.M;
-  const BrickOrder q_order = make_order(host_shapes, d, d.Lq);
+  const int ql = query_levels(flags, d.L);
+  if (ql < 0) return TRANSOAR_ERR_LEVELS;
+  const BrickOrder q_order = make_order(host_shapes, d, d.Lq, ql, (flags & TRANSOAR_MSDA3D_DETERMINISTIC) != 0);
   const long q_units = order_units(q_order, d, d.Lq);
   const long n_blocks = (q_units + kWavesPerBlock - 1) / kWavesPerBlock;
   const int lg = vec_lpv(d, sizeof(VT), flags);
+  if (ql > 0 && lg < 0) return TRANSOAR_ERR_MODE;
   const dim3 block(64 * kWavesPerBlock);
   auto v = static_cast<const VT*>(value);
   auto lo = static_cast<const LT*>(loc);
@@ -449,7 +466,7 @@
     for (int l = 0; small && l < d.L; ++l) small = q_order.D[l] <= 1000 && q_order.H[l] <= 1000 && q_order.W[l] <= 1000;
     if (q_order.enabled && fold_count && small && d.C == 64 && d.P == 4 &&
         !(flags & (TRANSOAR_MSDA3D_NO_BRICK | TRANSOAR_MSDA3D_NO_MMA))) {
-      const long n_wave = static_cast<long>(d.N) * (q_order.pad_start[q_order.L] >> 7) * d.M * 4;
+      const long n_wave = static_cast<long>(d.N) * q_order.q_bricks * d.M * 4;
       const BrickOrder* order_d = device_const(q_order, st);
       if (order_d == nullptr) return TRANSOAR_ERR_CONST;
       const dim3 qgrid(static_cast<unsigned>(((n_wave + 7) / 8) * 8));
@@ -498,6 +515,7 @@
   }
   if (det_req && !det) return TRANSOAR_ERR_MODE;
   if (grad_proj != nullptr && !recs_done) return TRANSOAR_ERR_MODE;
+  if (ql > 0 && !recs_done) return TRANSOAR_ERR_MODE;
   if constexpr (sizeof(VT) == 2) {
     if (!brick_done && q_order.enabled && fold_count && d.C == 64 && d.P == 4 && !(flags & TRANSOAR_MSDA3D_NO_BRICK)) {
       ProfScope prof(TRANSOAR_PROF_BWD_QUERY, st);
diff --git a/transoar_amd/csrc/msda3d_common.hpp b/transoar_amd/csrc/msda3d_common.hpp
--- a/transoar_amd/csrc/msda3d_common.hpp
+++ b/transoar_amd/csrc/msda3d_common.hpp
@@ -182,6 +182,8 @@
   int D[8], H[8], W[8], start[8];
   int nbh[8], nbw[8];
   int pad_start[9];
+  int q_bricks;
+  int q_write_bricks;
 };
 __device__ __forceinline__ int brick_slot_to_row(const BrickOrder& o, int x) {
   int l = 0;
diff --git a/transoar_amd/csrc/msda3d_mma.hpp b/transoar_amd/csrc/msda3d_mma.hpp
--- a/transoar_amd/csrc/msda3d_mma.hpp
+++ b/transoar_amd/csrc/msda3d_mma.hpp
@@ -448,12 +448,13 @@
   const long t1 = u >> 2;
   const int m = static_cast<int>(t1 % M);
   const long t2 = t1 / M;
-  const int bricks = order.pad_start[order.L] >> 7;
+  const int bricks = order.q_bricks;
   const int brick = bricks - 1 - static_cast<int>(t2 % bricks);
   const long b = t2 / bricks;
   const int slot = (2 * (sb >> 1) + (j >> 4)) * 32 + ((j >> 2) & 3) * 8 + 4 * (sb & 1) + (j & 3);
   const int s = brick_slot_to_row(order, brick * kBrickSlots + slot);
   const bool live = s >= 0;
+  const bool writes = live && brick < order.q_write_bricks;
   const long item = live ? (b * S + s) * M + m : 0;
   const int LP = L * P;
   const unsigned row_bytes = static_cast<unsigned>(M) * C * sizeof(VT);
@@ -465,7 +466,7 @@
 #pragma unroll
   for (int sk = 0; sk < 4; ++sk) {
     u32x4 raw{0u, 0u, 0u, 0u};
-    if (live) raw = *reinterpret_cast<const u32x4*>(grad_out + item * C + 16 * sk + 8 * kg);
+    if (writes) raw = *reinterpret_cast<const u32x4*>(grad_out + item * C + 16 * sk + 8 * kg);
     gof[sk] = __builtin_bit_cast(s16x8, raw);
   }
 
@@ -758,7 +759,7 @@
         dst[2] = o[4] | (o[5] << 16);
         stage[j * 32 + 24 + l * 2 + kg] = bf(a_in[l][0] * (res_a[l][0] - dot)) | (bf(a_in[l][1] * (res_a[l][1] - dot)) << 16);
       });
-      if (kg == 0) tok[j] = live ? static_cast<int>(b * S + s) : -1;
+      if (kg == 0) tok[j] = writes ? static_cast<int>(b * S + s) : -1;
       __syncthreads();
       const unsigned row_pieces = static_cast<unsigned>(M) * 8u;
 #pragma unroll
@@ -773,7 +774,7 @@
       return;
     }
   }
-  if (live) {
+  if (writes) {
     static_for<0, kMmaLevels>([&](auto lc) {
       constexpr int l = decltype(lc)::value;
       if (l >= L) return;
@@ -812,7 +813,7 @@
   const long t1 = u >> 2;
   const int m = static_cast<int>(t1 % M);
   const long t2 = t1 / M;
-  const int bricks = order.pad_start[order.L] >> 7;
+  const int bricks = order.q_bricks;
   const int brick = bricks - 1 - static_cast<int>(t2 % bricks);
   const long b = t2 / bricks;
   const int slot = (2 * (sb >> 1) + (j >> 4)) * 32 + ((j >> 2) & 3) * 8 + 4 * (sb & 1) + (j & 3);
diff --git a/transoar_amd/csrc/msda3d_pcm.hpp b/transoar_amd/csrc/msda3d_pcm.hpp
--- a/transoar_amd/csrc/msda3d_pcm.hpp
+++ b/transoar_amd/csrc/msda3d_pcm.hpp
@@ -110,7 +110,7 @@
   const unsigned t1 = u >> 4;
   const unsigned m = t1 % static_cast<unsigned>(M);
   const unsigned t2 = t1 / static_cast<unsigned>(M);
-  const unsigned bricks = static_cast<unsigned>(order.pad_start[order.L]) >> 7;
+  const unsigned bricks = static_cast<unsigned>(order.q_bricks);
   const int brick = static_cast<int>(bricks - 1u - t2 % bricks);
   const unsigned b = t2 / bricks;
 
diff --git a/transoar_amd/ms_deform_attn.py b/transoar_amd/ms_deform_attn.py
--- a/transoar_amd/ms_deform_attn.py
+++ b/transoar_amd/ms_deform_attn.py
@@ -54,26 +54,27 @@
 class _HeadGather(Function):
 
     @staticmethod
-    def forward(ctx, value, proj, reference_points, shapes, level_start, m, lv, pt, im2col_step):
+    def forward(ctx, value, proj, reference_points, shapes, level_start, m, lv, pt, im2col_step, query_levels=0):
         loc, attn = _head_raw(proj, reference_points, shapes, m, lv, pt)
-        out = MSDA.ms_deform_attn_forward(value, shapes, level_start, loc, attn, im2col_step)
+        out = MSDA.ms_deform_attn_forward(value, shapes, level_start, loc, attn, im2col_step, query_levels=query_levels)
         ctx.save_for_backward(value, shapes, level_start, loc, attn)
-        ctx.head = (m, lv, pt, tuple(proj.shape), im2col_step)
+        ctx.head = (m, lv, pt, tuple(proj.shape), im2col_step, query_levels)
         return out
 
     @staticmethod
     @once_differentiable
     def backward(ctx, grad_output):
         value, shapes, starts, loc, attn = ctx.saved_tensors
-        m, lv, pt, proj_shape, step = ctx.head
+        m, lv, pt, proj_shape, step, query_levels = ctx.head
         grad_output = grad_output.contiguous()
-        res = MSDA.ms_deform_attn_backward_proj(value, shapes, starts, loc, attn, grad_output, step)
+        res = MSDA.ms_deform_attn_backward_proj(value, shapes, starts, loc, attn, grad_output, step, query_levels=query_levels)
         if res is None:
-            g_value, g_loc, g_attn = MSDA.ms_deform_attn_backward(value, shapes, starts, loc, attn, grad_output, step)
+            g_value, g_loc, g_attn = MSDA.ms_deform_attn_backward(value, shapes, starts, loc, attn, grad_output, step,
+                                                                  query_levels=query_levels)
             g_proj = _head_bwd_raw(g_loc.contiguous(), g_attn.contiguous(), attn, shapes, m, lv, pt, proj_shape)
         else:
             g_value, g_proj = res
-        return g_value, g_proj, None, None, None, None, None, None, None
+        return g_value, g_proj, None, None, None, None, None, None, None, None
 
 
 HEAD_GATHER = __import__("os").environ.get("TRANSOAR_HEAD_GATHER", "1") != "0"
@@ -124,7 +125,7 @@
             self.output_proj.bias.zero_()
 
     def forward(self, query, reference_points, input_flatten, input_spatial_shapes,
-                input_level_start_index, input_padding_mask=None):
+                input_level_start_index, input_padding_mask=None, query_levels=0):
         n, lq, _ = query.shape
         s = input_flatten.shape[1]
         if reference_points.shape[-1] != 3:
@@ -149,7 +150,7 @@
                 and value.dtype in (torch.bfloat16, torch.float16)
                 and _sampling_head_usable(proj, reference_points, input_spatial_shapes, m, lv, pt)):
             sampled = _HeadGather.apply(value, proj, reference_points, input_spatial_shapes, input_level_start_index,
-                                        m, lv, pt, self.im2col_step)
+                                        m, lv, pt, self.im2col_step, query_levels if lq == s else 0)
             return token_linear(sampled, self.output_proj.weight, self.output_proj.bias)
         if self.use_cuda and _sampling_head_usable(proj, reference_points, input_spatial_shapes, m, lv, pt):
             locations, weights = _sampling_head(proj, reference_points, input_spatial_shapes, m, lv, pt)
diff --git a/transoar_amd/msda.py b/transoar_amd/msda.py
--- a/transoar_amd/msda.py
+++ b/transoar_amd/msda.py
@@ -11,6 +11,8 @@
 flags = int(os.environ.get("TRANSOAR_MSDA_FLAGS", "0"))
 DETERMINISTIC = 64
 ERR_MODE = -8
+QUERY_LEVELS_SHIFT = 8
+LAST_PATH = {"forward": None, "backward": None}
 deterministic = os.environ.get("TRANSOAR_MSDA_DETERMINISTIC", "0") == "1"
 
 
@@ -26,6 +28,12 @@
         hit = (spatial_shapes._version, (ctypes.c_int64 * len(vals))(*vals))
         spatial_shapes._transoar_host_shapes = hit
     return hit[1], ctypes.addressof(hit[1])
+
+
+def _query_rows(host, L, Lq, S, query_levels):
+    if not query_levels or not 0 < query_levels < L or host is None or Lq != S:
+        return None
+    return sum(host[3 * l] * host[3 * l + 1] * host[3 * l + 2] for l in range(query_levels))
 
 
 def _require(cond, msg):
@@ -74,7 +82,7 @@
 
 
 def ms_deform_attn_forward(value, spatial_shapes, level_start_index, sampling_loc, attn_weight,
-                           im2col_step):
+                           im2col_step, query_levels=0):
     _check_inputs([("value", value), ("spatial_shapes", spatial_shapes),
                    ("level_start_index", level_start_index), ("sampling_loc", sampling_loc),
                    ("attn_weight", attn_weight)])
@@ -82,11 +90,21 @@
                                  attn_weight, im2col_step)
     sampling_loc, attn_weight = _coerce_loc(value, sampling_loc, attn_weight)
     out = torch.empty((N, Lq, M * C), dtype=value.dtype, device=value.device)
-    _keep, host_ptr = _shapes_on_host(spatial_shapes)
-    _native.launch(_native.lib.transoar_msda3d_forward, value,
-                   value.data_ptr(), spatial_shapes.data_ptr(), level_start_index.data_ptr(),
-                   sampling_loc.data_ptr(), attn_weight.data_ptr(), out.data_ptr(),
-                   N, S, M, C, L, Lq, P, _DT[value.dtype], _DT[sampling_loc.dtype], host_ptr, flags)
+    host, host_ptr = _shapes_on_host(spatial_shapes)
+
+    def run(call_flags, ok=()):
+        return _native.launch(_native.lib.transoar_msda3d_forward, value,
+                              value.data_ptr(), spatial_shapes.data_ptr(), level_start_index.data_ptr(),
+                              sampling_loc.data_ptr(), attn_weight.data_ptr(), out.data_ptr(),
+                              N, S, M, C, L, Lq, P, _DT[value.dtype], _DT[sampling_loc.dtype], host_ptr, call_flags, ok=ok)
+
+    live = _query_rows(host, L, Lq, S, query_levels)
+    if live is not None and run(flags | (query_levels << QUERY_LEVELS_SHIFT), ok=(ERR_MODE,)) == 0:
+        out[:, live:].zero_()
+        LAST_PATH["forward"] = "query_levels"
+        return out
+    run(flags)
+    LAST_PATH["forward"] = "whole"
     return out
 
 
@@ -111,7 +129,7 @@
 
 
 def ms_deform_attn_backward(value, spatial_shapes, level_start_index, sampling_loc, attn_weight,
-                            grad_output, im2col_step):
+                            grad_output, im2col_step, query_levels=0):
     _check_inputs([("value", value), ("spatial_shapes", spatial_shapes),
                    ("level_start_index", level_start_index), ("sampling_loc", sampling_loc),
                    ("attn_weight", attn_weight), ("grad_output", grad_output)])
@@ -125,10 +143,11 @@
     grad_loc = torch.empty_like(sampling_loc)
     grad_attn = torch.empty_like(attn_weight)
     dims = (N, S, M, C, L, Lq, P, _DT[value.dtype], _DT[sampling_loc.dtype])
-    _keep, host_ptr = _shapes_on_host(spatial_shapes)
+    host, host_ptr = _shapes_on_host(spatial_shapes)
     torch_det = torch.are_deterministic_algorithms_enabled()
-
-    def run(call_flags, ok=()):
+    live = _query_rows(host, L, Lq, S, query_levels)
+
+    def run_once(call_flags, ok=()):
         ws_bytes = _native.lib.transoar_msda3d_backward_workspace_bytes(*dims, call_flags)
         workspace = torch.empty(max(ws_bytes, 16), dtype=torch.uint8, device=value.device)
         return _native.launch(_native.lib.transoar_msda3d_backward, value,
@@ -136,6 +155,15 @@
                               sampling_loc.data_ptr(), attn_weight.data_ptr(), grad_output.data_ptr(),
                               grad_value.data_ptr(), grad_loc.data_ptr(), grad_attn.data_ptr(),
                               workspace.data_ptr(), ws_bytes, *dims, host_ptr, call_flags, ok=ok)
+
+    def run(call_flags, ok=()):
+        LAST_PATH["backward"] = "whole"
+        if live is not None and run_once(call_flags | (query_levels << QUERY_LEVELS_SHIFT), ok=(ERR_MODE,)) == 0:
+            grad_loc[:, live:].zero_()
+            grad_attn[:, live:].zero_()
+            LAST_PATH["backward"] = "query_levels"
+            return 0
+        return run_once(call_flags, ok=ok)
 
     strict = deterministic or bool(flags & DETERMINISTIC)
     if strict or torch_det:
@@ -153,7 +181,8 @@
     return [grad_value, grad_loc.to(loc_in_dtype), grad_attn.to(attn_in_dtype)]
 
 
-def ms_deform_attn_backward_proj(value, spatial_shapes, level_start_index, sampling_loc, attn_weight, grad_output, im2col_step):
+def ms_deform_attn_backward_proj(value, spatial_shapes, level_start_index, sampling_loc, attn_weight, grad_output, im2col_step,
+                                 query_levels=0):
     _check_inputs([("value", value), ("spatial_shapes", spatial_shapes), ("level_start_index", level_start_index),
                    ("sampling_loc", sampling_loc), ("attn_weight", attn_weight), ("grad_output", grad_output)])
     N, S, M, C, L, Lq, P = _dims(value, spatial_shapes, level_start_index, sampling_loc, attn_weight, im2col_step)
@@ -165,11 +194,20 @@
     grad_value = torch.empty_like(value)
     grad_proj = torch.empty((N, Lq, 4 * M * L * P), dtype=torch.bfloat16, device=value.device)
     dims = (N, S, M, C, L, Lq, P, _DT[value.dtype], _DT[sampling_loc.dtype])
-    _keep, host_ptr = _shapes_on_host(spatial_shapes)
+    host, host_ptr = _shapes_on_host(spatial_shapes)
     ws_bytes = _native.lib.transoar_msda3d_backward_workspace_bytes(*dims, call_flags)
     workspace = torch.empty(max(ws_bytes, 16), dtype=torch.uint8, device=value.device)
-    rc = _native.launch(_native.lib.transoar_msda3d_backward_proj, value,
-                        value.data_ptr(), spatial_shapes.data_ptr(), level_start_index.data_ptr(), sampling_loc.data_ptr(),
-                        attn_weight.data_ptr(), grad_output.data_ptr(), grad_value.data_ptr(), grad_proj.data_ptr(),
-                        workspace.data_ptr(), ws_bytes, *dims, host_ptr, call_flags, ok=(ERR_MODE,))
-    return None if rc else [grad_value, grad_proj]
+
+    def run(run_flags):
+        return _native.launch(_native.lib.transoar_msda3d_backward_proj, value,
+                              value.data_ptr(), spatial_shapes.data_ptr(), level_start_index.data_ptr(), sampling_loc.data_ptr(),
+                              attn_weight.data_ptr(), grad_output.data_ptr(), grad_value.data_ptr(), grad_proj.data_ptr(),
+                              workspace.data_ptr(), ws_bytes, *dims, host_ptr, run_flags, ok=(ERR_MODE,))
+
+    live = _query_rows(host, L, Lq, S, query_levels)
+    if live is not None and run(call_flags | (query_levels << QUERY_LEVELS_SHIFT)) == 0:
+        grad_proj[:, live:].zero_()
+        LAST_PATH["backward"] = "query_levels"
+        return [grad_value, grad_proj]
+    LAST_PATH["backward"] = "whole"
+    return None if run(call_flags) else [grad_value, grad_proj]
diff --git a/transoar_amd/refine_block.py b/transoar_amd/refine_block.py
--- a/transoar_amd/refine_block.py
+++ b/transoar_amd/refine_block.py
@@ -5,6 +5,7 @@
 import torch.nn.functional as F
 from torch import nn
 
+from . import msda as MSDA
 from .ms_deform_attn import MSDeformAttn
 from .token_linear import fused_ffn, fused_ffn_usable, linear_relu_dropout, linear_relu_dropout_usable, token_linear
 
@@ -74,8 +75,8 @@
         ffn = token_linear(hidden, self.linear2.weight, self.linear2.bias)
         return self.norm2(src + self.dropout3(ffn))
 
-    def forward_fused(self, x, x16, q16, reference_points, spatial_shapes, level_start_index, pos_pack=()):
-        attn = self.self_attn(q16, reference_points, x16, spatial_shapes, level_start_index)
+    def forward_fused(self, x, x16, q16, reference_points, spatial_shapes, level_start_index, pos_pack=(), query_levels=0):
+        attn = self.self_attn(q16, reference_points, x16, spatial_shapes, level_start_index, query_levels=query_levels)
         y32, y16, _ = fused_tokens.add_layernorm(x, attn.contiguous(), self.norm1, dropout=self.dropout1)
         if (self.activation is F.relu and fused_tokens.SEEDED_DROPOUT and FUSED_FFN1
                 and fused_ffn_usable(y16, self.linear1.weight, self.linear2.weight)):
@@ -132,6 +133,7 @@
         self.refine_def_attn = DefAttnTransformer(layer, num_layers)
         self.level_embed = nn.Parameter(torch.empty(n_levels, d_model))
         self._geometry = {}
+        self.last_path = None
         self._reset_parameters()
 
     def _reset_parameters(self):
@@ -155,16 +157,25 @@
             self._geometry[key] = geo
         return geo
 
-    def forward(self, fmaps, pos_embeds):
+    def forward(self, fmaps, pos_embeds, read_levels=None):
         shapes = tuple(tuple(f.shape[2:]) for f in fmaps)
         spatial, starts, sizes, ref = self._level_geometry(shapes, fmaps[0].device)
         tokens = torch.cat([map_to_tokens(f) for f in fmaps], dim=1)
+        if read_levels is not None:
+            if not 0 < read_levels <= len(fmaps):
+                raise ValueError("read_levels must be in 1..%d, got %r" % (len(fmaps), read_levels))
+            sizes_out, shapes_out = sizes[:read_levels], shapes[:read_levels]
+        self.last_path = "whole"
         if self._fused_ok(tokens, pos_embeds):
-            memory = self._forward_fused(tokens, pos_embeds, shapes, spatial, starts, sizes, ref)
+            memory = self._forward_fused(tokens, pos_embeds, shapes, spatial, starts, sizes, ref,
+                                         query_levels=read_levels if read_levels is not None and read_levels < len(fmaps) else 0)
         else:
             pos = torch.cat([self._pos_tokens(p, lvl) + self.level_embed[lvl].view(1, 1, -1).to(p.dtype)
                              for lvl, p in enumerate(pos_embeds)], dim=1)
             memory = self.refine_def_attn(tokens, spatial, starts, pos, ref)
+        if read_levels is not None:
+            memory = memory[:, :sum(sizes_out)]
+            return [tokens_to_map(m, shape) for m, shape in zip(memory.split(sizes_out, dim=1), shapes_out)]
         return [tokens_to_map(m, shape) for m, shape in zip(memory.split(sizes, dim=1), shapes)]
 
     bf16_out = os.environ.get("TRANSOAR_REFINE_FP32_OUT", "0") != "1"
@@ -175,7 +186,7 @@
                 and all(is_constant(p) for p in pos_embeds)
                 and fused_tokens.usable(tokens, None, self.d_model))
 
-    def _forward_fused(self, tokens, pos_embeds, shapes, spatial, starts, sizes, ref):
+    def _forward_fused(self, tokens, pos_embeds, shapes, spatial, starts, sizes, ref, query_levels=0):
         key = ("pos_sine", shapes, tokens.device)
         const = self._geometry.get(key)
         if const is None:
@@ -188,7 +199,12 @@
         x, x16 = tokens, tokens
         for i, layer in enumerate(layers):
             last = i == len(layers) - 1
-            x, x16, q16 = layer.forward_fused(x, x16, q16, ref, spatial, starts, () if last else pos_pack)
+            if last:
+                MSDA.LAST_PATH["forward"] = None
+            x, x16, q16 = layer.forward_fused(x, x16, q16, ref, spatial, starts, () if last else pos_pack,
+                                              query_levels=query_levels if last else 0)
+            if last and MSDA.LAST_PATH["forward"] == "query_levels":
+                self.last_path = "read_levels"
         return x16 if DecoderDefAttnBlock.bf16_out else x
 
     def _pos_tokens(self, pos_map, lvl):
diff --git a/transoar_amd/transoarnet.py b/transoar_amd/transoarnet.py
--- a/transoar_amd/transoarnet.py
+++ b/transoar_amd/transoarnet.py
@@ -1,4 +1,5 @@
 import itertools
+import os
 
 import torch
 import torch.nn.functional as F
@@ -10,6 +11,9 @@
 from .focused_decoder import FocusedDecoder
 from .matcher import Matcher
 from .position_encoding import PositionEmbeddingLearned3D, PositionEmbeddingSine3D
+
+
+READ_LEVELS = os.environ.get("TRANSOAR_REFINE_READ_LEVELS", "1") != "0"
 
 
 def build_backbone(config):
@@ -94,6 +98,8 @@
         self._aux_loss = neck["aux_loss"]
 
         self._backbone = build_backbone(config["backbone"])
+        if READ_LEVELS:
+            self._backbone._decoder.read_levels = (self._input_levels,) + (("P0",) if config["backbone"]["use_seg_proxy_loss"] else ())
 
         anchors, restrictions = generate_anchors(neck, config["bbox_properties"])
         if not neck["anchor_gen_dynamic_offset"]:
```
